# TissueImageAnalytics/cerberus

Measured on AMD Instinct MI355X. Metric: Mpx/sec WSI tiled inference (all heads), higher is better.
Workload: dtype f32

## Files before the change

### cerberus_amd/csrc/cerb_api.hip

```cpp
#include "cerb_net.h"

static thread_local std::string g_err;
int cerb_set_error(const std::string& m) {
    g_err = m;
    return 1;
}
extern "C" int cerb_version(void) { return 1; }
extern "C" const char* cerb_last_error(void) { return g_err.c_str(); }
std::atomic<long long> g_devbuf_bytes{0};
extern "C" size_t cerb_device_bytes_held(void) { const long long v = g_devbuf_bytes.load(); return v > 0 ? (size_t)v : 0; }
thread_local hipStream_t g_call_stream = nullptr;

static int alloc_dev(cerb_net* net, size_t bytes, void** out) {
    if (net->reusing) {
        if (net->reuse_cursor >= net->n_finalize_allocs || net->dev_alloc_bytes[net->reuse_cursor] != bytes)
            return fail("reload: the tensors do not have the shapes the handle was finalized with");
        *out = net->dev_allocs[net->reuse_cursor++];
        return 0;
    }
    void* d = nullptr;
    HIP_OK(hipMalloc(&d, bytes));
    net->dev_allocs.push_back(d);
    net->dev_alloc_bytes.push_back(bytes);
    *out = d;
    return 0;
}
static int upload(cerb_net* net, const std::vector<float>& v, float** out) {
    void* d = nullptr;
    if (alloc_dev(net, v.size() * sizeof(float), &d)) return 1;
    HIP_OK(hipMemcpy(d, v.data(), v.size() * sizeof(float), hipMemcpyHostToDevice));
    *out = reinterpret_cast<float*>(d);
    return 0;
}

extern "C" int cerb_net_create(const char* const* decoder_names, const char* const* head_names, const int* out_ch,
                               int n_decoders, cerb_net** out_net) {
    if (!decoder_names || !head_names || !out_ch || !out_net || n_decoders <= 0) return fail("cerb_net_create: bad arguments");
    cerb_net* net = new cerb_net();
    for (int i = 0; i < n_decoders; ++i) {
        DecoderCfg d;
        d.name = decoder_names[i];
        d.head = head_names[i];
        d.out_ch = out_ch[i];
        if (d.name == "Patch-Class") {
            d.kind = 2;
            if (d.out_ch < 1 || d.out_ch > 16) { delete net; return fail("Patch-Class: out_ch must be 1..16"); }
            net->pc_idx = i;
        } else {
            if (d.head == "INST") d.kind = 0;
            else if (d.head == "TYPE") d.kind = 1;
            else { delete net; return fail("decoder " + d.name + ": head must be INST or TYPE, got " + d.head); }
            if (d.kind == 0 && d.out_ch != 2 && d.out_ch != 3) { delete net; return fail("INST heads must have 2 or 3 channels (infer_step keeps channels 1..out_ch-1), got " + std::to_string(d.out_ch)); }
            if (d.out_ch < 2 || d.out_ch > 8) { delete net; return fail("head out_ch must be 2..8"); }
            int trunk = -1;
            for (size_t t = 0; t < net->trunk_idx.size(); ++t)
                if (net->dec[net->trunk_idx[t]].name == d.name) trunk = (int)t;
            if (trunk < 0) {
                trunk = (int)net->trunk_idx.size();
                net->trunk_idx.push_back(i);
            } else {
                for (int e : net->dense_idx)
                    if (net->dec[e].name == d.name && net->dec[e].head == d.head) { delete net; return fail("decoder " + d.name + ": head " + d.head + " listed twice"); }
            }
            net->dense_idx.push_back(i);
            net->trunk_of.push_back(trunk);
        }
        net->dec.push_back(d);
    }
    *out_net = net;
    return 0;
}

extern "C" void cerb_net_destroy(cerb_net* net) { delete net; }

extern "C" int cerb_net_load_tensor(cerb_net* net, const char* key, const float* data, const int64_t* shape, int ndim) {
    if (!net || !key) return fail("cerb_net_load_tensor: bad arguments");
    if (net->finalized) return fail("cerb_net_load_tensor: network already finalized");
    std::string k(key);
    if (k.size() > 19 && k.compare(k.size() - 19, 19, "num_batches_tracked") == 0) return 0;
    if (k.rfind("backbone.fc.", 0) == 0) return 0;
    if (!data && ndim > 0) return fail("cerb_net_load_tensor: null data for " + k);
    HostTensor t;
    size_t n = 1;
    for (int i = 0; i < ndim; ++i) {
        t.shape.push_back(shape[i]);
        n *= (size_t)shape[i];
    }
    t.data.assign(data, data + n);
    net->host[k] = std::move(t);
    return 0;
}

struct Fold {
    std::vector<float> scale, shift;
};
static int get(cerb_net* net, const std::string& k, std::vector<int64_t> shape, const HostTensor** out) {
    auto it = net->host.find(k);
    if (it == net->host.end()) return fail("missing key in state dict: " + k);
    if (it->second.shape != shape) {
        std::string s = "shape mismatch for " + k + ": got [";
        for (auto v : it->second.shape) s += std::to_string(v) + ",";
        s += "] expected [";
        for (auto v : shape) s += std::to_string(v) + ",";
        return fail(s + "]");
    }
    *out = &it->second;
    return 0;
}
static int bn_fold(cerb_net* net, const std::string& p, int ch, Fold* f) {
    const HostTensor *w, *b, *m, *v;
    if (get(net, p + ".weight", {ch}, &w) || get(net, p + ".bias", {ch}, &b) || get(net, p + ".running_mean", {ch}, &m) ||
        get(net, p + ".running_var", {ch}, &v))
        return 1;
    f->scale.resize(ch);
    f->shift.resize(ch);
    for (int c = 0; c < ch; ++c) {
        const float s = w->data[c] / std::sqrt(v->data[c] + 1e-5f);
        f->scale[c] = s;
        f->shift[c] = b->data[c] - m->data[c] * s;
    }
    return 0;
}

static void pack_conv(const float* w, const float* scale, int cout, int cin, int ks, int CB, std::vector<float>* out) {
    const int T = ks * ks, NG = CB / 8, nchunk = cin / CB, ncb = cout / 64;
    const size_t base = out->size();
    out->resize(base + (size_t)cout * cin * T);
    float* o = out->data() + base;
    size_t idx = 0;
    for (int cb = 0; cb < ncb; ++cb)
        for (int ch = 0; ch < nchunk; ++ch)
            for (int tap = 0; tap < T; ++tap)
                for (int G = 0; G < NG; ++G)
                    for (int s = 0; s < 2; ++s)
                        for (int lane = 0; lane < 64; ++lane)
                            for (int t = 0; t < 4; ++t) {
                                const int co = cb * 64 + s * 32 + (lane & 31);
                                const int ci = ch * CB + G * 8 + 4 * (lane >> 5) + t;
                                o[idx++] = w[((size_t)co * cin + ci) * T + tap] * (scale ? scale[co] : 1.f);
                            }
}

static void pack_wino(const float* w, const float* scale, int cout, int cin, std::vector<float>* out) {
    static const double Gm[4][3] = {{1, 0, 0}, {0.5, 0.5, 0.5}, {0.5, -0.5, 0.5}, {0, 0, 1}};
    const int nchunk = cin / 32, ncb = cout / 64;
    const size_t base = out->size();
    out->resize(base + (size_t)cout * cin * 16);
    float* o = out->data() + base;
    std::vector<float> U((size_t)cout * cin * 16);
    for (int co = 0; co < cout; ++co)
        for (int ci = 0; ci < cin; ++ci) {
            double g[3][3], t[4][3];
            for (int y = 0; y < 3; ++y)
                for (int x = 0; x < 3; ++x) g[y][x] = (double)(w[((size_t)co * cin + ci) * 9 + y * 3 + x] * (scale ? scale[co] : 1.f));
            for (int a = 0; a < 4; ++a)
                for (int x = 0; x < 3; ++x) t[a][x] = Gm[a][0] * g[0][x] + Gm[a][1] * g[1][x] + Gm[a][2] * g[2][x];
            for (int a = 0; a < 4; ++a)
                for (int b = 0; b < 4; ++b)
                    U[((size_t)co * cin + ci) * 16 + a * 4 + b] = (float)(t[a][0] * Gm[b][0] + t[a][1] * Gm[b][1] + t[a][2] * Gm[b][2]);
        }
    size_t idx = 0;
    for (int cb = 0; cb < ncb; ++cb)
        for (int ch = 0; ch < nchunk; ++ch)
            for (int a = 0; a < 4; ++a)
                for (int b = 0; b < 4; ++b)
                    for (int G = 0; G < 4; ++G)
                        for (int s = 0; s < 2; ++s)
                            for (int lane = 0; lane < 64; ++lane)
                                for (int t = 0; t < 4; ++t) {
                                    const int co = cb * 64 + s * 32 + (lane & 31);
                                    const int ci = ch * 32 + G * 8 + 4 * (lane >> 5) + t;
                                    o[idx++] = U[((size_t)co * cin + ci) * 16 + a * 4 + b];
                                }
}

static void pack_wino4(const float* w, int cout, int cin, std::vector<float>* out, int layout = 0) {
    const bool chunk32 = layout == 1;
    static const double Gm[6][3] = {{1.0 / 4, 0, 0},          {-1.0 / 6, -1.0 / 6, -1.0 / 6}, {-1.0 / 6, 1.0 / 6, -1.0 / 6},
                                    {1.0 / 24, 1.0 / 12, 1.0 / 6}, {1.0 / 24, -1.0 / 12, 1.0 / 6},  {0, 0, 1}};
    const int nchunk = cin / 16, ncb = cout / 64;
    std::vector<float> U((size_t)cout * cin * 36);
    for (int co = 0; co < cout; ++co)
        for (int ci = 0; ci < cin; ++ci) {
            const float* g = w + ((size_t)co * cin + ci) * 9;
            double t[6][3];
            for (int a = 0; a < 6; ++a)
                for (int x = 0; x < 3; ++x) t[a][x] = Gm[a][0] * (double)g[x] + Gm[a][1] * (double)g[3 + x] + Gm[a][2] * (double)g[6 + x];
            for (int a = 0; a < 6; ++a)
                for (int b = 0; b < 6; ++b)
                    U[((size_t)co * cin + ci) * 36 + a * 6 + b] = (float)(t[a][0] * Gm[b][0] + t[a][1] * Gm[b][1] + t[a][2] * Gm[b][2]);
        }
    const size_t base = out->size();
    out->resize(base + (size_t)cout * cin * 36);
    float* o = out->data() + base;
    size_t idx = 0;
    if (chunk32) {
        for (int cb = 0; cb < ncb; ++cb)
            for (int ch = 0; ch < cin / 32; ++ch)
                for (int a = 0; a < 4; ++a)
                    for (int xi = 0; xi < 36; ++xi)
                        for (int G = 0; G < 2; ++G)
                            for (int lane = 0; lane < 64; ++lane)
                                for (int t = 0; t < 4; ++t) {
                                    const int co = cb * 64 + 16 * a + (lane & 15);
                                    const int ci = ch * 32 + 16 * G + 4 * (lane >> 4) + t;
                                    o[idx++] = U[((size_t)co * cin + ci) * 36 + xi];
                                }
        return;
    }
    for (int cb = 0; cb < ncb; ++cb)
        for (int ch = 0; ch < nchunk; ++ch)
            for (int a = 0; a < 4; ++a)
                for (int xi = 0; xi < 36; ++xi)
                    for (int lane = 0; lane < 64; ++lane)
                        for (int t = 0; t < 4; ++t) {
                            const int co = cb * 64 + 16 * a + (lane & 15);
                            const int ci = ch * 16 + 4 * (lane >> 4) + t;
                            o[idx++] = U[((size_t)co * cin + ci) * 36 + xi];
                        }
}

static int store_bn(cerb_net* net, const std::string& name, const std::vector<std::string>& bnkeys, int ch) {
    std::vector<float> ga, be;
    for (const std::string& k : bnkeys) {
        const HostTensor *w, *b;
        if (get(net, k + ".weight", {ch}, &w) || get(net, k + ".bias", {ch}, &b)) return 1;
        ga.insert(ga.end(), w->data.begin(), w->data.end());
        be.insert(be.end(), b->data.begin(), b->data.end());
    }
    cerb_net::BnDev d;
    d.C = ch;
    d.groups = (int)bnkeys.size();
    if (upload(net, ga, &d.gamma) || upload(net, be, &d.beta)) return 1;
    for (size_t g = 0; g < bnkeys.size(); ++g) {
        net->param_slots[bnkeys[g] + ".weight"].push_back({d.gamma + g * ch, ch});
        net->param_slots[bnkeys[g] + ".bias"].push_back({d.beta + g * ch, ch});
    }
    net->bn[name] = d;
    net->bn_keys[name] = bnkeys;
    return 0;
}

static int make_conv(cerb_net* net, const std::string& name, const std::vector<std::string>& wkeys,
                     const std::vector<std::string>& bkeys, const std::vector<std::string>& bnkeys, int cout, int cin, int ks,
                     int stride) {
    const int CB = cerb_conv_chunk(ks, stride);
    if (cout % 64 || cin % CB) return fail("conv " + name + ": unsupported channel counts");
    std::vector<float> wp, bp, wwino, hw;
    const bool wino = (ks == 3 && stride == 1 && cin % 32 == 0);
    for (size_t g = 0; g < wkeys.size(); ++g) {
        const HostTensor* w;
        if (get(net, wkeys[g], {cout, cin, ks, ks}, &w)) return 1;
        Fold f;
        bool have_bn = !bnkeys.empty() && net->fold_bn;
        if (have_bn && bn_fold(net, bnkeys[g], cout, &f)) return 1;
        if (net->fold_bn) {
            pack_conv(w->data.data(), have_bn ? f.scale.data() : nullptr, cout, cin, ks, CB, &wp);
            if (wino) {
                pack_wino(w->data.data(), have_bn ? f.scale.data() : nullptr, cout, cin, &wwino);
                const size_t b0 = hw.size();
                hw.insert(hw.end(), w->data.begin(), w->data.end());
                if (have_bn)
                    for (int co = 0; co < cout; ++co)
                        for (size_t e = 0; e < (size_t)cin * 9; ++e) hw[b0 + (size_t)co * cin * 9 + e] *= f.scale[co];
            }
        }
        const HostTensor* b = nullptr;
        if (!bkeys.empty() && get(net, bkeys[g], {cout}, &b)) return 1;
        for (int c = 0; c < cout; ++c) {
            float v = b ? b->data[c] : 0.f;
            if (have_bn) v = v * f.scale[c] + f.shift[c];
            bp.push_back(v);
        }
    }
    if (!net->fold_bn && !bnkeys.empty() && store_bn(net, name, bnkeys, cout)) return 1;
    if (!net->fold_bn) {
        std::vector<float> rw, rb;
        for (size_t g = 0; g < wkeys.size(); ++g) {
            const HostTensor* w;
            if (get(net, wkeys[g], {cout, cin, ks, ks}, &w)) return 1;
            rw.insert(rw.end(), w->data.begin(), w->data.end());
            if (!bkeys.empty()) {
                const HostTensor* b;
                if (get(net, bkeys[g], {cout}, &b)) return 1;
                rb.insert(rb.end(), b->data.begin(), b->data.end());
            }
        }
        cerb_net::RawW r;
        r.wkeys = wkeys; r.bkeys = bkeys; r.bnkeys = bnkeys;
        if (upload(net, rw, &r.w) || (!rb.empty() && upload(net, rb, &r.b))) return 1;
        for (size_t g = 0; g < wkeys.size(); ++g) {
            const long long nwg = (long long)cout * cin * ks * ks;
            net->param_slots[wkeys[g]].push_back({r.w + g * nwg, nwg});
            if (r.b) net->param_slots[bkeys[g]].push_back({r.b + g * cout, cout});
        }
        net->raw[name] = r;
    }
    PackedConv pc;
    pc.cin = cin; pc.cout = cout; pc.ks = ks; pc.stride = stride; pc.groups = (int)wkeys.size();
    if (upload(net, bp, &pc.b)) return 1;
    if (!net->fold_bn)
        for (size_t g = 0; g < bkeys.size(); ++g) net->param_slots[bkeys[g]].push_back({pc.b + g * cout, cout});
    if (net->fold_bn) {
        if (upload(net, wp, &pc.w)) return 1;
        if (wino && upload(net, wwino, &pc.wino)) return 1;
        pc.host_w.swap(hw);
    } else {
        const float* rawd = net->raw[name].w;
        const size_t G = wkeys.size(), nw = (size_t)cout * cin * ks * ks, nu = (size_t)cout * cin * 16;
        const bool dgrad = ks == 3 && cin % 64 == 0 && cout % 32 == 0;
        void *dwp = nullptr, *dwi = nullptr, *ddg = nullptr;
        if (alloc_dev(net, G * nw * 4, &dwp) || (wino && alloc_dev(net, G * nu * 4, &dwi)) || (dgrad && alloc_dev(net, G * nu * 4, &ddg))) return 1;
        pc.w = reinterpret_cast<float*>(dwp);
        pc.wino = reinterpret_cast<float*>(dwi);
        pc.wino_dgrad = reinterpret_cast<float*>(ddg);
        for (size_t g = 0; g < G; ++g) {
            HIP_OK(cerb_launch_pack_conv(rawd + g * nw, pc.w + g * nw, cout, cin, ks, CB, 0));
            if (wino) HIP_OK(cerb_launch_pack_wino(rawd + g * nw, pc.wino + g * nu, cout, cin, 0, 0));
            if (dgrad) HIP_OK(cerb_launch_pack_wino(rawd + g * nw, pc.wino_dgrad + g * nu, cin, cout, 1, 0));
        }
    }
    net->conv[name] = pc;
    return 0;
}


extern "C" int cerb_net_finalize(cerb_net* net) {
    if (!net) return fail("cerb_net_finalize: null handle");
    if (net->finalized) return 0;
    if (!net->fold_bn && net->trunk_idx.size() != net->dense_idx.size())
        return fail("cerb_net_finalize: a decoder with several output heads runs in inference only (the training tape sums one head's gradient per decoder)");
    {
        const HostTensor* w;
        if (get(net, "backbone.conv1.weight", {64, 3, 7, 7}, &w)) return 1;
        Fold f;
        if (bn_fold(net, "backbone.bn1", 64, &f)) return 1;
        if (!net->fold_bn) {
            f.scale.assign(64, 1.f);
            f.shift.assign(64, 0.f);
            if (store_bn(net, "stem", {"backbone.bn1"}, 64)) return 1;
        }
        std::vector<float> wp(7 * 12 * 2 * 64, 0.f);
        for (int ky = 0; ky < 7; ++ky)
            for (int t = 0; t < 12; ++t)
                for (int s = 0; s < 2; ++s)
                    for (int lane = 0; lane < 64; ++lane) {
                        const int co = s * 32 + (lane & 31), kk = 2 * t + (lane >> 5);
                        float v = 0.f;
                        if (kk < 21) {
                            const int kx = kk / 3, c = kk % 3;
                            v = w->data[(((size_t)co * 3 + c) * 7 + ky) * 7 + kx] * f.scale[co];
                        }
                        wp[((ky * 12 + t) * 2 + s) * 64 + lane] = v;
                    }
        if (upload(net, wp, &net->stem_w) || upload(net, f.shift, &net->stem_b)) return 1;
        if (!net->fold_bn) {
            if (upload(net, w->data, &net->stem_raw)) return 1;
            net->param_slots["backbone.conv1.weight"].push_back({net->stem_raw, 64 * 147});
        }
    }
    int inpl = 64;
    for (int li = 0; li < 4; ++li) {
        const int planes = kFilters[li + 1];
        for (int b = 0; b < kLayers[li]; ++b) {
            const std::string p = "backbone.layer" + std::to_string(li + 1) + "." + std::to_string(b);
            const int stride = (b == 0 && li > 0) ? 2 : 1;
            if (make_conv(net, p + ".conv1", {p + ".conv1.weight"}, {}, {p + ".bn1"}, planes, inpl, 3, stride)) return 1;
            if (make_conv(net, p + ".conv2", {p + ".conv2.weight"}, {}, {p + ".bn2"}, planes, planes, 3, 1)) return 1;
            if (stride != 1 || inpl != planes)
                if (make_conv(net, p + ".downsample", {p + ".downsample.0.weight"}, {}, {p + ".downsample.1"}, planes, inpl, 1, stride)) return 1;
            inpl = planes;
        }
    }
    if (make_conv(net, "conv_map", {"conv_map.weight"}, {}, {}, 256, 512, 1, 1)) return 1;
    const int dec_in[4] = {256, 128, 64, 64};
    const int dec_u[4][2] = {{256, 128}, {128, 64}, {64, 64}, {64, 64}};
    if (!net->dense_idx.empty()) {
        for (int u = 0; u < 4; ++u) {
            int c = dec_in[u];
            for (int j = 0; j < 2; ++j) {
                std::vector<std::string> wk, bk, bnk;
                for (int di : net->trunk_idx) {
                    const std::string p = "decoder_head." + net->dec[di].name + "." + std::to_string(u) + ".block." + std::to_string(j);
                    wk.push_back(p + ".conv.weight");
                    bk.push_back(p + ".conv.bias");
                    bnk.push_back(p + ".bn");
                }
                if (make_conv(net, "dec." + std::to_string(u) + "." + std::to_string(j), wk, bk, bnk, dec_u[u][j], c, 3, 1)) return 1;
                c = dec_u[u][j];
            }
        }
        for (int di : net->dense_idx) {
            const DecoderCfg& d = net->dec[di];
            const std::string p = "output_head." + d.name + "." + d.head + ".x";
            const HostTensor *w1, *b1, *w2, *b2;
            Fold f;
            if (get(net, p + ".0.block.0.conv.weight", {96, 64, 1, 1}, &w1) || get(net, p + ".0.block.0.conv.bias", {96}, &b1) ||
                bn_fold(net, p + ".0.block.0.bn", 96, &f) || get(net, p + ".1.conv.weight", {d.out_ch, 96, 1, 1}, &w2) ||
                get(net, p + ".1.conv.bias", {d.out_ch}, &b2))
                return 1;
            std::vector<float> w1p(6 * 4 * 64 * 4), b1p(96), w2p(6 * 64 * 4, 0.f), b2p(32, 0.f);
            for (int blk = 0; blk < 6; ++blk)
                for (int G = 0; G < 4; ++G)
                    for (int lane = 0; lane < 64; ++lane)
                        for (int t = 0; t < 4; ++t) {
                            const int hid = blk * 16 + (lane & 15), ci = G * 16 + 4 * (lane >> 4) + t;
                            w1p[((blk * 4 + G) * 64 + lane) * 4 + t] = w1->data[(size_t)hid * 64 + ci] * f.scale[hid];
                        }
            for (int c = 0; c < 96; ++c) b1p[c] = b1->data[c] * f.scale[c] + f.shift[c];
            for (int blk = 0; blk < 6; ++blk)
                for (int lane = 0; lane < 64; ++lane)
                    for (int r = 0; r < 4; ++r) {
                        const int o = lane & 15, hid = blk * 16 + 4 * (lane >> 4) + r;
                        w2p[(blk * 64 + lane) * 4 + r] = (o < d.out_ch) ? w2->data[(size_t)o * 96 + hid] : 0.f;
                    }
            for (int c = 0; c < d.out_ch; ++c) b2p[c] = b2->data[c];
            std::vector<float> w2q(2 * 24 * 64, 0.f);
            for (int set = 0; set < 2; ++set)
                for (int blk = 0; blk < 6; ++blk)
                    for (int r = 0; r < 4; ++r)
                        for (int lane = 0; lane < 64; ++lane) {
                            const int o = 4 * set + (lane & 3), hid = blk * 16 + 4 * (lane >> 4) + r;
                            if (o < d.out_ch) w2q[((set * 6 + blk) * 64 + lane) * 4 + r] = w2->data[(size_t)o * 96 + hid];
                        }
            if (!net->fold_bn) {
                float *r1, *rb1, *r2, *rb2;
                if (upload(net, w1->data, &r1) || upload(net, b1->data, &rb1) || upload(net, w2->data, &r2) || upload(net, b2->data, &rb2)) return 1;
                net->head_rw1.push_back(r1); net->head_rb1.push_back(rb1); net->head_rw2.push_back(r2); net->head_rb2.push_back(rb2);
                net->param_slots[p + ".0.block.0.conv.weight"].push_back({r1, 96 * 64});
                net->param_slots[p + ".0.block.0.conv.bias"].push_back({rb1, 96});
                net->param_slots[p + ".1.conv.weight"].push_back({r2, (long long)d.out_ch * 96});
                net->param_slots[p + ".1.conv.bias"].push_back({rb2, d.out_ch});
                if (store_bn(net, "head." + std::to_string(net->head_rw1.size() - 1), {p + ".0.block.0.bn"}, 96)) return 1;
            }
            float *dw1, *db1, *dw2, *db2;
            float* dw2q;
            if (upload(net, w1p, &dw1) || upload(net, b1p, &db1) || upload(net, w2p, &dw2) || upload(net, b2p, &db2) || upload(net, w2q, &dw2q)) return 1;
            net->head_w1.push_back(dw1); net->head_b1.push_back(db1); net->head_w2.push_back(dw2); net->head_b2.push_back(db2); net->head_w2q.push_back(dw2q);
        }
    }
    if (net->pc_idx >= 0) {
        const int oc = net->dec[net->pc_idx].out_ch;
        const std::string p = "decoder_head.Patch-Class";
        Fold f1, f2;
        const HostTensor *w1, *b1, *w2, *b2;
        if (bn_fold(net, p + ".bn1", 512, &f1) || bn_fold(net, p + ".bn2", 256, &f2) || get(net, p + ".conv1.weight", {256, 512, 1, 1}, &w1) ||
            get(net, p + ".conv1.bias", {256}, &b1) || get(net, p + ".conv2.weight", {oc, 256, 1, 1}, &w2) || get(net, p + ".conv2.bias", {oc}, &b2))
            return 1;
        if (!net->fold_bn) {
            if (upload(net, w1->data, &net->pc_rw1) || upload(net, b1->data, &net->pc_rb1) || upload(net, w2->data, &net->pc_rw2) ||
                upload(net, b2->data, &net->pc_rb2) || store_bn(net, "pc.bn1", {p + ".bn1"}, 512) || store_bn(net, "pc.bn2", {p + ".bn2"}, 256))
                return 1;
            net->param_slots[p + ".conv1.weight"].push_back({net->pc_rw1, 256 * 512});
            net->param_slots[p + ".conv1.bias"].push_back({net->pc_rb1, 256});
            net->param_slots[p + ".conv2.weight"].push_back({net->pc_rw2, (long long)oc * 256});
            net->param_slots[p + ".conv2.bias"].push_back({net->pc_rb2, oc});
        }
        std::vector<float> w1t(512 * 256), b1f(256), w2t(256 * 16, 0.f), b2f(16, 0.f);
        for (int o = 0; o < 256; ++o) {
            for (int c = 0; c < 512; ++c) w1t[(size_t)c * 256 + o] = w1->data[(size_t)o * 512 + c] * f2.scale[o];
            b1f[o] = b1->data[o] * f2.scale[o] + f2.shift[o];
        }
        for (int o = 0; o < oc; ++o) {
            for (int c = 0; c < 256; ++c) w2t[(size_t)c * 16 + o] = w2->data[(size_t)o * 256 + c];
            b2f[o] = b2->data[o];
        }
        if (upload(net, f1.scale, &net->pc_bn1s) || upload(net, f1.shift, &net->pc_bn1b) || upload(net, w1t, &net->pc_w1t) ||
            upload(net, b1f, &net->pc_b1) || upload(net, w2t, &net->pc_w2t) || upload(net, b2f, &net->pc_b2))
            return 1;
    }
    if (!net->fold_bn) {
        std::vector<float> z(512, 0.f);
        if (upload(net, z, &net->zero_bias)) return 1;
    }
    if (!net->fold_bn) HIP_OK(hipDeviceSynchronize());
    if (net->reusing && net->reuse_cursor != net->n_finalize_allocs) return fail("reload: fewer tensors than the handle was finalized with");
    if (!net->reusing) net->n_finalize_allocs = net->dev_allocs.size();
    net->reusing = false;
    net->host.clear();
    net->finalized = true;
    return 0;
}

int prof_begin(cerb_net* net, const std::string& name, const std::string& kernel, double flops, hipStream_t st) {
    if (!net->profiling) return 0;
    if (net->prof_n == net->prof.size()) {
        cerb_net::ProfRec r;
        HIP_OK(hipEventCreate(&r.e0));
        HIP_OK(hipEventCreate(&r.e1));
        net->prof.push_back(r);
    }
    cerb_net::ProfRec& r = net->prof[net->prof_n];
    r.name = name; r.kernel = kernel; r.flops = flops;
    HIP_OK(hipEventRecord(r.e0, st));
    net->prof_open = true;
    return 0;
}
int prof_end(cerb_net* net, hipStream_t st) {
    if (!net->profiling) return 0;
    HIP_OK(hipEventRecord(net->prof[net->prof_n].e1, st));
    net->prof_n++;
    net->prof_open = false;
    return 0;
}

int train_wino2_fresh(cerb_net* net, const std::string& name, PackedConv& cm, int dgrad, hipStream_t st) {
    if (net->fold_bn) return 0;
    bool& used = dgrad ? cm.wino_dgrad_used : cm.wino_used;
    bool& stale = dgrad ? cm.wino_dgrad_stale : cm.wino_stale;
    used = true;
    if (!stale) return 0;
    auto rit = net->raw.find(name);
    if (rit == net->raw.end()) return fail("conv " + name + ": no raw weights to re-pack");
    const size_t nw = (size_t)cm.cout * cm.cin * 9, nu = (size_t)cm.cout * cm.cin * 16;
    for (int g = 0; g < cm.groups; ++g)
        HIP_OK(cerb_launch_pack_wino(rit->second.w + g * nw, (dgrad ? cm.wino_dgrad : cm.wino) + g * nu, dgrad ? cm.cin : cm.cout, dgrad ? cm.cout : cm.cin, dgrad, st));
    stale = false;
    return 0;
}

int train_wino4_slot(cerb_net* net, const std::string& name, PackedConv& cm, int w4b, int dgrad, hipStream_t st, float** out) {
    float*& slot = cm.wino4_t[w4b][dgrad];
    if (!slot) {
        auto rit = net->raw.find(name);
        if (rit == net->raw.end()) return fail("conv " + name + ": no raw weights for the F(4x4) transform");
        const size_t nw = (size_t)cm.cout * cm.cin * 9, nu = (size_t)cm.cout * cm.cin * 36;
        void* d = nullptr;
        HIP_OK(hipMalloc(&d, (size_t)cm.groups * nu * 4));
        net->dev_allocs.push_back(d);
        net->dev_alloc_bytes.push_back((size_t)cm.groups * nu * 4);
        slot = (float*)d;
        (void)nw;
        HIP_OK(cerb_launch_pack_wino4(rit->second.w, slot, dgrad ? cm.cin : cm.cout, dgrad ? cm.cout : cm.cin, dgrad, w4b, cm.groups, st));
    }
    *out = slot;
    return 0;
}

static constexpr int kPlanarLowest = 0;
static const char* const kPlanarFamily[4] = {"conv_wino4_planar<f4x4,16x16x2,eighth-res>", "conv_wino4_planar<f4x4,16x16x2,quarter-res>",
                                             "conv_wino4p<f4x4,16x16x2,planar,half-res>", "conv_wino4p<f4x4,16x16x2,planar>"};
static const char* const kPlanarEntryFamily[4] = {"upsample2_add_planar<eighth-res>", "upsample2_add_planar<quarter-res>", "upsample2_add_planar", "upsample2_add_planar"};

int run_conv(cerb_net* net, const std::string& name, const float* in, const float* prev, const float* resid, float* out, int N,
             int H, int W, int relu, int mode, long long in_gs, long long prev_gs, hipStream_t st, double* macs,
             const int* roi, long long planar_out_gs) {
    auto it = net->conv.find(name);
    if (it == net->conv.end()) return fail("internal: conv " + name + " not packed");
    const PackedConv& c = it->second;
    struct BnReq {
        cerb_net* n;
        ~BnReq() { n->conv_bn_part = nullptr; }
    } bn_req{net};
    net->conv_bn_bpg = 0;
    ConvParams p;
    memset(&p, 0, sizeof(p));
    p.in = in; p.prev = prev; p.wpack = c.w; p.bias = c.b; p.resid = resid; p.out = out;
    p.N = N; p.H = H; p.W = W; p.Cin = c.cin; p.Cout = c.cout;
    p.Ho = (c.stride == 2) ? H / 2 : H;
    p.Wo = (c.stride == 2) ? W / 2 : W;
    p.relu = relu;
    p.groups = c.groups;
    p.in_gs = in_gs; p.prev_gs = prev_gs;
    p.w_gs = (long long)c.cout * c.cin * c.ks * c.ks;
    p.bias_gs = c.cout;
    p.resid_gs = 0;
    p.out_gs = (long long)N * p.Ho * p.Wo * c.cout;
    p.pk_off = net->packed_items ? 0 : 1;
    if (macs) {
        *macs += (double)c.groups * N * p.Ho * p.Wo * (double)c.cout * c.cin * c.ks * c.ks;
        if (!out) return 0;
    }
    const double fl = 2.0 * (double)c.groups * N * p.Ho * p.Wo * (double)c.cout * c.cin * c.ks * c.ks;
    const long long map_px = (long long)p.Ho * p.Wo;
    const bool use_w4 = net->conv_algo == 5 || net->conv_algo == 7 || (net->conv_algo == 6 && map_px >= 256);
    const bool planar = planar_out_gs > 0;
    static const long long w4b_max_px = [] {
        const char* e = cerb_dev_getenv("CERB_W4B_MAX_PX");
        return e ? atoll(e) : 4096ll;
    }();
    const bool w4b = !planar && (net->conv_algo == 7 || (net->conv_algo == 6 && map_px <= w4b_max_px)) && c.cin % 64 == 0;
    if (planar && !(use_w4 && c.wino && mode == 0 && net->fold_bn && !resid)) return fail("internal: conv " + name + " cannot take the planar path");
    if (use_w4 && c.wino && mode == 0 && (!it->second.host_w.empty() || !net->fold_bn)) {
        PackedConv& cm = it->second;
        float* train_slot = nullptr;
        if (!net->fold_bn && train_wino4_slot(net, name, cm, w4b ? 1 : 0, 0, st, &train_slot)) return 1;
        float*& slot4 = !net->fold_bn ? train_slot : (w4b ? cm.wino4b : cm.wino4);
        if (!slot4) {
            std::vector<float> w4;
            for (int g = 0; g < cm.groups; ++g) pack_wino4(cm.host_w.data() + (size_t)g * cm.cout * cm.cin * 9, cm.cout, cm.cin, &w4, w4b ? 1 : 0);
            void* d = nullptr;
            HIP_OK(hipMalloc(&d, w4.size() * 4));
            net->dev_allocs.push_back(d);
            net->dev_alloc_bytes.push_back(w4.size() * 4);
            HIP_OK(hipMemcpy(d, w4.data(), w4.size() * 4, hipMemcpyHostToDevice));
            slot4 = (float*)d;
        }
        p.wpack = slot4;
        p.w_gs = (long long)c.cout * c.cin * 36;
        double fl_done = fl;
        if (roi && roi[1] > roi[0] && roi[3] > roi[2]) {
            p.roi_y0 = roi[0]; p.roi_y1 = roi[1]; p.roi_x0 = roi[2]; p.roi_x1 = roi[3];
            const double ty = (roi[1] + 15) / 16 - roi[0] / 16, tx = (roi[3] + 15) / 16 - roi[2] / 16;
            fl_done = fl * (ty * 16.0 * tx * 16.0) / ((double)p.Ho * p.Wo);
        }
        if (planar) {
            p.out_gs = planar_out_gs;
            p.level_tag = net->planar_level == 3 ? 1 : net->planar_level == 2 ? 0 : 2;
            p.pl_byp = cerb_planar_blocks(p.Ho);
            p.pl_bxp = cerb_planar_blocks(p.Wo);
        }
        if (prof_begin(net, name, planar ? kPlanarFamily[net->planar_level & 3] : w4b ? (cerb_wino4b_packed(p) ? (resid ? "conv_wino4b<f4x4,16t,res>" : "conv_wino4b<f4x4,16t>") : (resid ? "conv_wino4b<f4x4,16x16,res>" : "conv_wino4b<f4x4,16x16>")) : (resid ? "conv_wino4<f4x4,16x16x2,res>" : "conv_wino4<f4x4,16x16x2>"), fl_done, st)) return 1;
        if (net->conv_bn_part && !planar && !resid && !(roi && roi[1] > roi[0] && roi[3] > roi[2])) {
            p.bn_part = net->conv_bn_part;
            net->conv_bn_bpg = w4b ? cerb_wino4b_bn_blocks(p) : N * ((p.Ho + 15) / 16) * ((p.Wo + 15) / 16);
        }
        HIP_OK(planar ? cerb_launch_wino4p(p, st) : w4b ? cerb_launch_wino4b(p, st) : cerb_launch_wino4(p, st));
        if (prof_end(net, st)) return 1;
        return 0;
    }
    if (net->conv_algo && c.wino && mode == 0) {
        if (train_wino2_fresh(net, name, it->second, 0, st)) return 1;
        p.wpack = c.wino;
        p.w_gs = (long long)c.cout * c.cin * 16;
        double fl_done = fl;
        if (roi && roi[1] > roi[0] && roi[3] > roi[2]) {
            p.roi_y0 = roi[0]; p.roi_y1 = roi[1]; p.roi_x0 = roi[2]; p.roi_x1 = roi[3];
            const double ty = (roi[1] + 7) / 8 - roi[0] / 8, tx = (roi[3] + 15) / 16 - roi[2] / 16;
            fl_done = fl * (ty * 8.0 * tx * 16.0) / ((double)p.Ho * p.Wo);
        }
        if (prof_begin(net, name, resid ? "conv_wino<f2x2,8x16,res>" : "conv_wino<f2x2,8x16>", fl_done, st)) return 1;
        HIP_OK(cerb_launch_wino(p, st));
        if (prof_end(net, st)) return 1;
        return 0;
    }
    const std::string kn = "conv_igemm<ks" + std::to_string(c.ks) + ",s" + std::to_string(c.stride) + ",mode" + std::to_string(mode) +
                           (p.Wo < 32 ? ",16x16>" : ",8x32>");
    if (prof_begin(net, name, kn, fl, st)) return 1;
    HIP_OK(cerb_launch_conv(p, c.ks, c.stride, mode, st));
    if (prof_end(net, st)) return 1;
    return 0;
}

static int forward_impl(cerb_net* net, const cerb_forward_io* io, hipStream_t st, double* macs) {
    g_call_stream = st;
    const bool dry = (macs != nullptr) && (io->tiles == nullptr) && (io->tiles_f32 == nullptr);
    const int N = io->n, H = io->h, W = io->w;
    if (N <= 0 || H <= 0 || W <= 0 || (H % 16) || (W % 16)) return fail("cerb_net_forward: tile H,W must be positive multiples of 16");
    const int out_h = io->out_h > 0 ? io->out_h : H, out_w = io->out_w > 0 ? io->out_w : W;
    if (out_h > H || out_w > W) return fail("cerb_net_forward: crop larger than tile");
    const int hs[5] = {H, H / 2, H / 4, H / 8, H / 16}, ws[5] = {W, W / 2, W / 4, W / 8, W / 16};
    const size_t D = net->trunk_idx.size();
    const size_t guard = cerb_conv_guard_bytes(W);
    const int planar_lowest = [] {
        const char* e = cerb_dev_getenv("CERB_PLANAR_LOWEST");
        return e ? atoi(e) : kPlanarLowest;
    }();
    auto level_is_planar = [&](int u) {
        if (dry || !net->planar || !net->fold_bn || net->conv_algo != 6 || net->head_algo < 1) return false;
        for (int v = 3; v >= u; --v) {
            if (v < planar_lowest) return false;
            auto c0 = net->conv.find("dec." + std::to_string(v) + ".0"), c1 = net->conv.find("dec." + std::to_string(v) + ".1");
            if (c0 == net->conv.end() || c1 == net->conv.end() || !c0->second.wino || !c1->second.wino) return false;
            const long long px = (long long)hs[3 - v] * ws[3 - v];
            if ((hs[3 - v] & 3) || (ws[3 - v] & 3)) return false;
            const bool ok = v >= 2 ? px >= 4096 && c0->second.cin == 64 && c0->second.cout == 64 && c1->second.cout == 64
                                   : px >= 256 && c0->second.cin % 16 == 0 && c0->second.cout % 64 == 0 && c1->second.cin == c0->second.cout && c1->second.cout % 64 == 0;
            if (!ok) return false;
        }
        return true;
    };
    if (!dry) {
        if (net->x0.ensure((size_t)N * H * W * 64 * 4, guard) || net->pool.ensure((size_t)N * hs[1] * ws[1] * 64 * 4, guard)) return fail_alloc();
        for (int i = 1; i < 5; ++i)
            if (net->x[i].ensure((size_t)N * hs[i] * ws[i] * kFilters[i] * 4, guard)) return fail_alloc();
        if (net->ta.ensure((size_t)N * hs[1] * ws[1] * 64 * 4, guard) || net->tb.ensure((size_t)N * hs[1] * ws[1] * 64 * 4, guard) ||
            net->cm.ensure((size_t)N * hs[4] * ws[4] * 256 * 4, guard))
            return fail_alloc();
        if (D) {
            static const bool exact_ws = cerb_dev_getenv("CERB_LEGACY_WS") == nullptr;
            size_t need_sum = 0, need_mid = 0;
            const int oc[4] = {128, 64, 64, 64};
            for (int u = 0; u < 4; ++u) {
                if (exact_ws && level_is_planar(u)) continue;
                const std::string n0 = "dec." + std::to_string(u) + ".0";
                auto c0 = net->conv.find(n0);
                const size_t px = (size_t)D * N * hs[3 - u] * ws[3 - u];
                need_sum = std::max(need_sum, px * (size_t)(c0 != net->conv.end() ? c0->second.cin : 256) * 4);
                need_mid = std::max(need_mid, px * (size_t)(c0 != net->conv.end() ? c0->second.cout : 256) * 4);
            }
            if (!exact_ws) need_sum = need_mid = D * (size_t)N * H * W * 64 * 4;
            if (net->dmid.ensure(need_mid, guard)) return fail_alloc();
            if (net->conv_algo && net->dsum.ensure(need_sum, guard)) return fail_alloc();
            for (int u = 0; u < 4; ++u) {
                if (exact_ws && level_is_planar(u)) continue;
                if (net->dout[u].ensure(D * (size_t)N * hs[3 - u] * ws[3 - u] * oc[u] * 4, guard)) return fail_alloc();
            }
        }
    }
    if (macs) *macs += (double)N * H * W * 64.0 * 147.0;
    if (!dry) {
        StemParams sp;
        sp.tiles = io->tiles; sp.tiles_f32 = io->tiles ? nullptr : io->tiles_f32; sp.wpack = net->stem_w; sp.bias = net->stem_b; sp.out = net->x0.p; sp.N = N; sp.H = H; sp.W = W; sp.relu = 1;
        sp.tiles_x = sp.tiles_y = 0;
        if (prof_begin(net, "stem", "stem_conv7x7", 2.0 * N * H * W * 64.0 * 147.0, st)) return 1;
        HIP_OK(cerb_launch_stem(sp, st));
        if (prof_end(net, st)) return 1;
        if (prof_begin(net, "maxpool", "maxpool3x3s2", 0.0, st)) return 1;
        HIP_OK(cerb_launch_maxpool(net->x0.p, net->pool.p, N, H, W, 64, st));
        if (prof_end(net, st)) return 1;
    }
    float* cur = dry ? nullptr : net->pool.p;
    int inpl = 64;
    for (int li = 0; li < 4; ++li) {
        const int planes = kFilters[li + 1];
        const int Hi = (li == 0) ? hs[1] : hs[li], Wi = (li == 0) ? ws[1] : ws[li];
        for (int b = 0; b < kLayers[li]; ++b) {
            const std::string p = "backbone.layer" + std::to_string(li + 1) + "." + std::to_string(b);
            const int stride = (b == 0 && li > 0) ? 2 : 1;
            const int hin = (b == 0) ? Hi : hs[li + 1], win = (b == 0) ? Wi : ws[li + 1];
            float* t1 = dry ? nullptr : net->ta.p;
            const bool last = (b == kLayers[li] - 1);
            float* outb = dry ? nullptr : (((kLayers[li] - 1 - b) % 2 == 0) ? net->x[li + 1].p : net->tb.p);
            (void)last;
            const float* idt = cur;
            if (run_conv(net, p + ".conv1", cur, nullptr, nullptr, t1, N, hin, win, 1, 0, 0, 0, st, macs)) return 1;
            if (stride != 1 || inpl != planes) {
                float* ds = dry ? nullptr : net->pool.p;
                if (run_conv(net, p + ".downsample", cur, nullptr, nullptr, ds, N, hin, win, 0, 0, 0, 0, st, macs)) return 1;
                idt = ds;
            }
            if (run_conv(net, p + ".conv2", t1, nullptr, idt, outb, N, hs[li + 1], ws[li + 1], 1, 0, 0, 0, st, macs)) return 1;
            cur = outb;
            inpl = planes;
        }
    }
    if (run_conv(net, "conv_map", dry ? nullptr : net->x[4].p, nullptr, nullptr, dry ? nullptr : net->cm.p, N, hs[4], ws[4], 0, 0, 0, 0, st, macs)) return 1;

    const long long tile_stride = io->tile_stride ? io->tile_stride : (long long)out_h * out_w;
    const long long row_stride = io->row_stride ? io->row_stride : out_w;
    if (net->pc_idx >= 0) {
        if (macs) *macs += (double)N * (512.0 * 256 + 256.0 * net->dec[net->pc_idx].out_ch);
        const bool want = io->out && io->out[net->pc_idx];
        const bool wantl = io->logits && io->logits[net->pc_idx];
        if (!dry && (want || wantl)) {
            PatchClassParams pp;
            memset(&pp, 0, sizeof(pp));
            pp.x4 = net->x[4].p; pp.bn1_s = net->pc_bn1s; pp.bn1_b = net->pc_bn1b; pp.w1t = net->pc_w1t; pp.b1 = net->pc_b1;
            pp.w2t = net->pc_w2t; pp.b2 = net->pc_b2;
            pp.N = N; pp.Hf = hs[4]; pp.Wf = ws[4]; pp.out_ch = net->dec[net->pc_idx].out_ch;
            pp.out_h = out_h; pp.out_w = out_w;
            pp.logits = wantl ? io->logits[net->pc_idx] : nullptr;
            pp.out = want ? (float*)io->out[net->pc_idx] : nullptr;
            pp.tile_off = io->tile_off; pp.tile_stride = tile_stride; pp.row_stride = row_stride;
            if (prof_begin(net, "patch_class", "patch_class", 2.0 * N * (512.0 * 256 + 256.0 * pp.out_ch), st)) return 1;
            HIP_OK(cerb_launch_patch_class(pp, st));
            if (prof_end(net, st)) return 1;
        }
    }
    if (D) {
        const float* skips[4] = {dry ? nullptr : net->x[3].p, dry ? nullptr : net->x[2].p, dry ? nullptr : net->x[1].p, dry ? nullptr : net->x0.p};
        const float* prev = dry ? nullptr : net->cm.p;
        long long prev_gs = 0;
        const int oc[4] = {128, 64, 64, 64};
        int roi_out[4][4], roi_mid[4][4], roi_sum[4][4];
        const bool any_logits = [&] {
            if (!io->logits) return false;
            for (size_t k = 0; k < net->dec.size(); ++k)
                if (io->logits[k]) return true;
            return false;
        }();
        const bool use_roi = !dry && net->crop_roi && (net->conv_algo == 1 || net->conv_algo >= 5) && !any_logits && (out_h < H || out_w < W);
        if (use_roi) {
            int y0 = (int)((H - out_h) * 0.5), x0 = (int)((W - out_w) * 0.5), y1 = y0 + out_h, x1 = x0 + out_w;
            for (int u = 3; u >= 0; --u) {
                const int hh = hs[3 - u], ww = ws[3 - u];
                auto widen = [&](int* r, const int* in, int d) {
                    r[0] = std::max(0, (in[0] - d) & ~3); r[1] = std::min(hh, (in[1] + d + 3) & ~3);
                    r[2] = std::max(0, (in[2] - d) & ~3); r[3] = std::min(ww, (in[3] + d + 3) & ~3);
                };
                const int win[4] = {y0, y1, x0, x1};
                widen(roi_out[u], win, 0);
                widen(roi_mid[u], roi_out[u], 1);
                widen(roi_sum[u], roi_mid[u], 1);
                y0 = std::max(0, roi_sum[u][0] / 2 - 1); y1 = std::min(hh / 2, (roi_sum[u][1] - 1) / 2 + 2);
                x0 = std::max(0, roi_sum[u][2] / 2 - 1); x1 = std::min(ww / 2, (roi_sum[u][3] - 1) / 2 + 2);
            }
        }
        bool feat_planar = false, prev_planar = false;
        for (int u = 0; u < 4; ++u) {
            const int hh = hs[3 - u], ww = ws[3 - u];
            const std::string n0 = "dec." + std::to_string(u) + ".0", n1 = "dec." + std::to_string(u) + ".1";
            const int cmid = net->conv[n0].cout;
            const int cin0 = net->conv[n0].cin;
            const bool lvl_planar = level_is_planar(u);
            if (lvl_planar) {
                PlanarBuf &bs = u == 3 ? net->psum : u == 2 ? net->psum2 : u == 1 ? net->psum1 : net->psum0;
                PlanarBuf &bm = u == 3 ? net->pmid : u == 2 ? net->pmid2 : u == 1 ? net->pmid1 : net->pmid0;
                const int cout1 = net->conv[n1].cout;
                PlanarBuf& bo = cout1 == cin0 ? bs : u == 1 ? net->pout1 : net->pout0;
                if (bs.ensure((int)D, N, hh, ww, cin0, st) || bm.ensure((int)D, N, hh, ww, cmid, st) || (&bo != &bs && bo.ensure((int)D, N, hh, ww, cout1, st)))
                    return fail_alloc();
                if (prof_begin(net, n0 + ".up", kPlanarEntryFamily[u], 0.0, st)) return 1;
                HIP_OK(cerb_launch_upsample2_add_planar(skips[u], prev, bs.b.p, (int)D, N, hh, ww, cin0, prev_gs, bs.gs(), use_roi ? roi_sum[u] : nullptr, prev_planar ? 1 : 0, st));
                if (prof_end(net, st)) return 1;
                net->planar_level = u;
                if (run_conv(net, n0, bs.b.p, nullptr, nullptr, bm.b.p, N, hh, ww, 1, 0, bs.gs(), 0, st, macs, use_roi ? roi_mid[u] : nullptr, bm.gs()))
                    return 1;
                if (run_conv(net, n1, bm.b.p, nullptr, nullptr, bo.b.p, N, hh, ww, 1, 0, bm.gs(), 0, st, macs, use_roi ? roi_out[u] : nullptr, bo.gs()))
                    return 1;
                if (u == 3) feat_planar = true;
                prev = bo.b.p;
                prev_gs = bo.gs();
                prev_planar = true;
                continue;
            }
            if (prev_planar) return fail("internal: a tile-planar decoder level feeds an NHWC one");
            if (net->conv_algo && net->conv[n0].wino && !dry) {
                if (prof_begin(net, n0 + ".up", "upsample2_add", 0.0, st)) return 1;
                HIP_OK(cerb_launch_upsample2_add(skips[u], prev, net->dsum.p, (int)D, N, hh, ww, cin0, prev_gs, use_roi ? roi_sum[u] : nullptr, st));
                if (prof_end(net, st)) return 1;
                if (run_conv(net, n0, net->dsum.p, nullptr, nullptr, net->dmid.p, N, hh, ww, 1, 0, (long long)N * hh * ww * cin0, 0, st, macs,
                             use_roi ? roi_mid[u] : nullptr))
                    return 1;
            } else if (run_conv(net, n0, skips[u], prev, nullptr, dry ? nullptr : net->dmid.p, N, hh, ww, 1, 1, 0, prev_gs, st, macs)) return 1;
            if (run_conv(net, n1, dry ? nullptr : net->dmid.p, nullptr, nullptr, dry ? nullptr : net->dout[u].p, N, hh, ww, 1, 0,
                         (long long)N * hh * ww * cmid, 0, st, macs, use_roi ? roi_out[u] : nullptr))
                return 1;
            prev = dry ? nullptr : net->dout[u].p;
            prev_gs = (long long)N * hh * ww * oc[u];
        }
        HeadParams hps[8];
        int n_hp = 0;
        double head_flops = 0.0;
        for (size_t k = 0; k < net->dense_idx.size(); ++k) {
            const int di = net->dense_idx[k];
            const size_t tk = (size_t)net->trunk_of[k];
            const DecoderCfg& d = net->dec[di];
            if (macs) *macs += (double)N * H * W * (64.0 * 96 + 96.0 * d.out_ch);
            const bool want = io->out && io->out[di];
            const bool wantl = io->logits && io->logits[di];
            if (dry || !(want || wantl)) continue;
            HeadParams hp;
            memset(&hp, 0, sizeof(hp));
            hp.feat = feat_planar ? net->psum.b.p + tk * net->psum.gs() : net->dout[3].p + tk * (size_t)N * H * W * 64;
            hp.feat_planar = feat_planar ? 1 : 0;
            hp.pl_byp = cerb_planar_blocks(H);
            hp.pl_bxp = cerb_planar_blocks(W);
            hp.w1p = net->head_w1[k]; hp.b1 = net->head_b1[k]; hp.w2p = net->head_w2[k]; hp.b2 = net->head_b2[k]; hp.w2q = net->head_w2q[k];
            hp.N = N; hp.H = H; hp.W = W; hp.out_ch = d.out_ch; hp.kind = d.kind;
            hp.crop_y0 = (int)((H - out_h) * 0.5); hp.crop_x0 = (int)((W - out_w) * 0.5);
            hp.out_h = want ? out_h : 0; hp.out_w = want ? out_w : 0;
            hp.roi = use_roi ? 1 : 0;
            hp.logits = wantl ? io->logits[di] : nullptr;
            hp.absmax_bits = io->logit_absmax ? io->logit_absmax + di : nullptr;
            if (want) {
                if (d.kind == 0) hp.out_inst = (float*)io->out[di];
                else if (io->type_is_u8) hp.out_type_u8 = (unsigned char*)io->out[di];
                else hp.out_type_i64 = (long long*)io->out[di];
            }
            hp.tile_off = io->tile_off; hp.tile_stride = tile_stride; hp.row_stride = row_stride;
            const double head_px = hp.roi ? (double)out_h * (((hp.crop_x0 + out_w + 15) / 16 - hp.crop_x0 / 16) * 16.0) : (double)H * W;
            const double fl = 2.0 * N * head_px * (64.0 * 96 + 96.0 * d.out_ch);
            if (net->head_algo == 0) {
                if (prof_begin(net, "head." + d.name, "head", fl, st)) return 1;
                HIP_OK(cerb_launch_head(hp, st));
                if (prof_end(net, st)) return 1;
            } else {
                if (n_hp == 8) {
                    if (prof_begin(net, "heads", "head_group", head_flops, st)) return 1;
                    HIP_OK(cerb_launch_head_group(hps, n_hp, st, net->head_algo == 1 ? 1 : 0));
                    if (prof_end(net, st)) return 1;
                    n_hp = 0;
                    head_flops = 0.0;
                }
                hps[n_hp++] = hp;
                head_flops += fl;
            }
        }
        if (n_hp > 0) {
            if (prof_begin(net, "heads", "head_group", head_flops, st)) return 1;
            HIP_OK(cerb_launch_head_group(hps, n_hp, st, net->head_algo == 1 ? 1 : 0));
            if (prof_end(net, st)) return 1;
        }
    }
    if (!dry && io->feats) {
        const float* src[6] = {net->x0.p, net->x[1].p, net->x[2].p, net->x[3].p, net->cm.p, net->x[4].p};
        const size_t nb[6] = {(size_t)N * H * W * 64, (size_t)N * hs[1] * ws[1] * 64, (size_t)N * hs[2] * ws[2] * 128,
                              (size_t)N * hs[3] * ws[3] * 256, (size_t)N * hs[4] * ws[4] * 256, (size_t)N * hs[4] * ws[4] * 512};
        for (int i = 0; i < 6; ++i)
            if (io->feats[i]) HIP_OK(hipMemcpyAsync(io->feats[i], src[i], nb[i] * 4, hipMemcpyDeviceToDevice, st));
    }
    return 0;
}

extern "C" int cerb_net_begin_reload(cerb_net* net) {
    if (!net) return fail("cerb_net_begin_reload: null handle");
    HIP_OK(hipDeviceSynchronize());
    while (net->dev_allocs.size() > net->n_finalize_allocs) {
        (void)hipFree(net->dev_allocs.back());
        net->dev_allocs.pop_back();
        net->dev_alloc_bytes.pop_back();
    }
    net->reusing = true;
    net->reuse_cursor = 0;
    net->param_slots.clear();
    net->conv.clear();
    net->bn.clear();
    net->raw.clear();
    net->grads.clear();
    net->head_w1.clear(); net->head_b1.clear(); net->head_w2.clear(); net->head_b2.clear(); net->head_w2q.clear();
    net->head_rw1.clear(); net->head_rb1.clear(); net->head_rw2.clear(); net->head_rb2.clear();
    net->host.clear();
    net->finalized = false;
    return 0;
}
extern "C" int cerb_net_update_params(cerb_net* net, int count, const char* const* keys, const float* const* dev_src, void* hip_stream) {
    if (!net || count < 0 || (count && (!keys || !dev_src))) return fail("cerb_net_update_params: bad arguments");
    if (!net->finalized || net->fold_bn) return fail("cerb_net_update_params: needs a finalized handle packed for training (cerb_net_set_fold_bn(net, 0))");
    hipStream_t st = (hipStream_t)hip_stream;
    std::vector<float*> cd;
    std::vector<const float*> cs;
    std::vector<long long> cn;
    for (int i = 0; i < count; ++i) {
        auto it = net->param_slots.find(keys[i]);
        if (it == net->param_slots.end()) continue;
        if (!dev_src[i]) return fail(std::string("cerb_net_update_params: null source for ") + keys[i]);
        for (const cerb_net::ParamSlot& sl : it->second) {
            cd.push_back(sl.dst); cs.push_back(dev_src[i]); cn.push_back(sl.n);
        }
    }
    HIP_OK(cerb_launch_copy_multi((int)cd.size(), cd.data(), cs.data(), cn.data(), &net->copy_tab, &net->copy_tab_bytes, &net->copy_tab_host, st));
    HIP_OK(cerb_launch_pack_stem(net->stem_raw, net->stem_w, st));
    static const bool per_conv = cerb_dev_getenv("CERB_PACK_PER_CONV") != nullptr;
    std::vector<PackJob> jobs;
    auto job = [&](const float* w, float* out, long long total, int cout, int cin, int kind, int a, int b) { jobs.push_back(PackJob{w, out, total, cout, cin, kind, a, b, 0}); };
    for (auto& kv : net->conv) {
        PackedConv& pc = kv.second;
        const float* rawd = net->raw[kv.first].w;
        if (pc.wino && !pc.wino_used) pc.wino_stale = true;
        if (pc.wino_dgrad && !pc.wino_dgrad_used) pc.wino_dgrad_stale = true;
        const size_t nw = (size_t)pc.cout * pc.cin * pc.ks * pc.ks, nu = (size_t)pc.cout * pc.cin * 16, nu4 = (size_t)pc.cout * pc.cin * 36;
        for (int g = 0; g < pc.groups; ++g) {
            if (per_conv) {
                HIP_OK(cerb_launch_pack_conv(rawd + g * nw, pc.w + g * nw, pc.cout, pc.cin, pc.ks, cerb_conv_chunk(pc.ks, pc.stride), st));
                if (pc.wino && pc.wino_used) HIP_OK(cerb_launch_pack_wino(rawd + g * nw, pc.wino + g * nu, pc.cout, pc.cin, 0, st));
                if (pc.wino_dgrad && pc.wino_dgrad_used) HIP_OK(cerb_launch_pack_wino(rawd + g * nw, pc.wino_dgrad + g * nu, pc.cin, pc.cout, 1, st));
                continue;
            }
            job(rawd + g * nw, pc.w + g * nw, (long long)nw, pc.cout, pc.cin, 0, pc.ks * pc.ks, cerb_conv_chunk(pc.ks, pc.stride));
            if (pc.wino && pc.wino_used) job(rawd + g * nw, pc.wino + g * nu, (long long)nu, pc.cout, pc.cin, 1, 0, 0);
            if (pc.wino_dgrad && pc.wino_dgrad_used) job(rawd + g * nw, pc.wino_dgrad + g * nu, (long long)nu, pc.cin, pc.cout, 1, 1, 0);
        }
        for (int l = 0; l < 2; ++l)
            for (int dg = 0; dg < 2; ++dg)
                if (pc.wino4_t[l][dg]) {
                    if (per_conv) {
                        HIP_OK(cerb_launch_pack_wino4(rawd, pc.wino4_t[l][dg], dg ? pc.cin : pc.cout, dg ? pc.cout : pc.cin, dg, l, pc.groups, st));
                        continue;
                    }
                    for (int g = 0; g < pc.groups; ++g)
                        job(rawd + g * nw, pc.wino4_t[l][dg] + g * nu4, (long long)nu4, dg ? pc.cin : pc.cout, dg ? pc.cout : pc.cin, 2, dg, l);
                }
    }
    if (!jobs.empty()) HIP_OK(cerb_launch_pack_multi(jobs.data(), (int)jobs.size(), &net->pack_tab, &net->pack_tab_bytes, &net->pack_tab_host, st));
    return 0;
}
extern "C" int cerb_net_set_fold_bn(cerb_net* net, int fold) {
    if (!net) return fail("cerb_net_set_fold_bn: null handle");
    if (net->finalized) return fail("cerb_net_set_fold_bn: must be called before cerb_net_finalize");
    net->fold_bn = fold ? 1 : 0;
    return 0;
}

extern "C" int cerb_net_forward(cerb_net* net, const cerb_forward_io* io, void* hip_stream) {
    if (!net || !io) return fail("cerb_net_forward: null argument");
    if (!net->finalized) return fail("cerb_net_forward: call cerb_net_finalize first");
    if (!io->tiles && !io->tiles_f32) return fail("cerb_net_forward: null tiles pointer (neither tiles nor tiles_f32)");
    if (!net->fold_bn) return fail("cerb_net_forward: the network was packed for training (cerb_net_set_fold_bn(net, 0)); use cerb_net_forward_train");
    net->prof_n = 0;
    return forward_impl(net, io, (hipStream_t)hip_stream, nullptr);
}

extern "C" double cerb_net_flops(const cerb_net* net, int n, int h, int w) {
    if (!net || !net->finalized) return -1.0;
    cerb_forward_io io;
    memset(&io, 0, sizeof(io));
    io.n = n; io.h = h; io.w = w;
    double macs = 0.0;
    if (forward_impl(const_cast<cerb_net*>(net), &io, nullptr, &macs)) return -1.0;
    return 2.0 * macs;
}

extern "C" int cerb_net_set_crop_roi(cerb_net* net, int enable) {
    if (!net) return fail("cerb_net_set_crop_roi: null handle");
    net->crop_roi = enable ? 1 : 0;
    return 0;
}
extern "C" int cerb_net_set_conv_algo(cerb_net* net, int algo) {
    if (!net) return fail("cerb_net_set_conv_algo: null handle");
    if (algo < 0 || algo > 7 || (algo >= 2 && algo <= 4))
        return fail("cerb_net_set_conv_algo: algo must be 0 (direct), 1 (Winograd F(2x2) fp32), 5 (Winograd F(4x4) fp32), 7 (F(4x4), one-block items with 32-channel chunks) or 6 (F(4x4) for maps of 16 x 16 pixels and more -- 7's kernel up to 64 x 64, 5's above --, else F(2x2): the default); 2-4 were experiments (scripts/experiments/)");
    net->conv_algo = algo;
    return 0;
}

extern "C" int cerb_net_set_bn_eval(cerb_net* net, const char* bn_prefix, const float* running_mean, const float* running_var, int channels) {
    if (!net || !bn_prefix) return fail("cerb_net_set_bn_eval: null argument");
    if (!net->finalized || net->fold_bn) return fail("cerb_net_set_bn_eval: needs a finalized network packed with cerb_net_set_fold_bn(net, 0)");
    for (auto& kv : net->bn_keys) {
        const std::vector<std::string>& keys = kv.second;
        for (size_t g = 0; g < keys.size(); ++g) {
            if (keys[g] != bn_prefix) continue;
            auto it = net->bn.find(kv.first);
            if (it == net->bn.end()) return fail(std::string("cerb_net_set_bn_eval: internal: no BatchNorm ") + kv.first);
            cerb_net::BnDev& b = it->second;
            if (!running_mean || !running_var) {
                if (g < b.eval.size()) b.eval[g] = 0;
                return 0;
// ... 81 lines not shown
```

### cerberus_amd/csrc/cerb_net.h

```cpp
#ifndef CERB_NET_H
#define CERB_NET_H
#include <hip/hip_runtime.h>

#include <algorithm>
#include <cmath>
#include <cstdio>
#include <cstdlib>
#include <cstring>
#include <map>
#include <atomic>
#include <string>
#include <vector>

#include "../../include/cerberus_hip.h"
#include "cerb_common.h"

hipError_t cerb_launch_conv(const ConvParams& p, int ks, int stride, int mode, hipStream_t st);
hipError_t cerb_launch_wino(ConvParams p, hipStream_t st);
hipError_t cerb_launch_wino4(ConvParams p, hipStream_t st);
hipError_t cerb_launch_wino4b(ConvParams p, hipStream_t st);
int cerb_wino4b_bn_blocks(const ConvParams& p);
bool cerb_wino4b_packed(const ConvParams& p);
hipError_t cerb_launch_wino4p(ConvParams p, hipStream_t st);
hipError_t cerb_launch_upsample2_add_planar(const float* skip, const float* prev, float* out, int groups, int N, int H, int W, int C, long long prev_gs,
                                            long long out_gs, const int* roi, int prev_planar, hipStream_t st);
hipError_t cerb_launch_upsample2_add(const float* skip, const float* prev, float* out, int groups, int N, int H, int W, int C,
                                     long long prev_gs, const int* roi, hipStream_t st);
extern "C" int cerb_conv_chunk(int ks, int stride);
struct StemParams {
    const unsigned char* tiles;
    const float* tiles_f32;
    const float* wpack;
    const float* bias;
    float* out;
    int N, H, W, tiles_x, tiles_y;
    int relu;
};
hipError_t cerb_launch_stem(StemParams p, hipStream_t st);
size_t cerb_bn_workspace_bytes(int groups, long long rows, int C);
hipError_t cerb_launch_bn_stats(const float* x, long long group_stride, long long rows, int C, int groups, float eps, float* mean, float* rstd,
                                float* var_unbiased, void* ws, hipStream_t st);
hipError_t cerb_launch_bn_apply(float* x, const float* src, const float* resid, long long group_stride, long long rows, int C, int groups, const float* mean,
                                const float* rstd, const float* gamma, const float* beta, int relu, hipStream_t st);
hipError_t cerb_launch_bn_finalize(const double* partial, int blocks, long long rows, int C, float eps, float* mean, float* rstd, float* var_unbiased, hipStream_t st,
                                   int groups = 1, void* fold_ws = nullptr);
size_t cerb_bn_fold_workspace_bytes(int groups, int C);
hipError_t cerb_launch_pointwise(const float* in, const float* w, const float* bias, float* out, long long rows, int cin, int cout, const float* in_scale,
                                 hipStream_t st, double* bn_part = nullptr, int* bn_blocks = nullptr);
hipError_t cerb_launch_crop_gap(const float* x, int N, int H, int W, int C, int y0, int ch, int x0, int cw, float* out, hipStream_t st);
hipError_t cerb_launch_copy_multi(int count, float* const* dst, const float* const* src, const long long* n, void** dev_tab, size_t* dev_bytes,
                                  std::vector<char>* host_prev, hipStream_t st);
hipError_t cerb_launch_bn_bwd(const float* dz, const float* z, const float* y, float* dy, float* dresid, long long group_stride, long long rows, int C, int groups,
                              const float* mean, const float* rstd, const float* gamma, const float* beta, float* dgamma, float* dbeta, int relu, int dy_assign, void* ws, hipStream_t st, unsigned long long eval_mask = 0, int dresid_assign = 0,
                              const double* pre_part = nullptr, int pre_bpg = 0);
int cerb_head_bwd2_blocks();
hipError_t cerb_launch_conv_bwd(const float* x, const float* dy, const float* w, float* dx, float* dw, float* db, int G, int N, int H, int W, int Cin, int Cout,
                                int ks, int stride, long long x_gs, hipStream_t st);
hipError_t cerb_launch_stem_wgrad(const unsigned char* tiles, const float* dy, float* dw, int N, int H, int W, hipStream_t st);
hipError_t cerb_launch_maxpool_bwd(const float* x, const float* ypool, const float* dy, float* dx, int N, int H, int W, int C, hipStream_t st);
hipError_t cerb_launch_maxpool_idx(const float* in, float* out, unsigned* idx, int N, int H, int W, int C, hipStream_t st);
hipError_t cerb_launch_maxpool_bwd_idx(const unsigned* idx, const float* dy, float* dx, int N, int H, int W, int C, hipStream_t st);
bool cerb_upadd_bwd_fused_ok(int H, int W, int C, int G);
hipError_t cerb_launch_upadd_bwd(const float* dout, float* dskip, float* dprev, int G, int N, int H, int W, int C, long long prev_gs, int shared_prev, hipStream_t st,
                                 unsigned group_mask = 0xffffffffu, int skip_assign = 0, int prev_assign = 0);
hipError_t cerb_launch_pointwise_bwd(const float* x, const float* dy, const float* w, float* dx, float* dw, float* db, long long rows, int cin, int cout,
                                     const float* in_scale, int dx_assign, hipStream_t st);
hipError_t cerb_launch_crop_gap_bwd(const float* dg, float* dx, int N, int H, int W, int C, int y0, int ch, int x0, int cw, hipStream_t st);
hipError_t cerb_launch_adam(float* p, const float* g, float* m, float* v, long long n, float lr, float b1, float b2, float eps, int step, hipStream_t st);
size_t cerb_wgrad_workspace_bytes(int G, int N, int Ho, int Wo, int Cin, int Cout, int ks, int* slices_out);
size_t cerb_stem_wgrad_workspace_bytes();
hipError_t cerb_launch_pack_stem(const float* w_raw, float* out, hipStream_t st);
struct PackJob {
    const float* w;
    float* out;
    long long total;
    int cout, cin, kind, a, b, pad;
};
hipError_t cerb_launch_pack_multi(const PackJob* jobs, int count, void** dev_tab, size_t* dev_bytes, std::vector<char>* host_prev, hipStream_t st);
hipError_t cerb_launch_adam_multi(int count, float* const* p, const float* const* g, float* const* m, float* const* v, const long long* n, float lr, float b1,
                                  float b2, float eps, int step, hipStream_t st);
hipError_t cerb_launch_pack_conv(const float* w_raw, float* out, int cout, int cin, int ks, int chunk, hipStream_t st);
hipError_t cerb_launch_pack_wino(const float* w_raw, float* out, int cout, int cin, int dgrad, hipStream_t st);
hipError_t cerb_launch_pack_wino4(const float* w_raw, float* out, int cout, int cin, int dgrad, int chunk32, int groups, hipStream_t st);
hipError_t cerb_launch_dilate2(const float* dy, float* d, long long n, int H, int W, int C, hipStream_t st);
size_t cerb_pw_wgrad_small_workspace_bytes(long long rows, int cin, int cout);
hipError_t cerb_launch_pw_wgrad_small(const float* x, const float* dy, float* dw, long long rows, int cin, int cout, void* ws, hipStream_t st);
size_t cerb_pw_bwd_small_workspace_bytes(long long rows, int cin, int cout);
hipError_t cerb_launch_pw_bwd_small(const float* x, const float* dy, const float* w, float* dx, float* dw, float* db, long long rows, int cin, int cout,
                                    int dx_assign, void* ws, hipStream_t st);
hipError_t cerb_launch_stem_wgrad_mfma(const unsigned char* tiles, const float* dy, float* dw, int N, int H, int W, void* ws, hipStream_t st);
hipError_t cerb_launch_colsum(const float* d, long long group_stride, long long rows, int C, int G, float* out, void* ws, hipStream_t st);
bool cerb_wgrad_wino_supported(int H, int W, int Cin, int Cout);
size_t cerb_wgrad_wino_workspace_bytes(int G, int N, int H, int W, int Cin, int Cout);
hipError_t cerb_launch_wgrad_wino(const float* x, const float* dy, float* dw, int G, int N, int H, int W, int Cin, int Cout, long long x_gs, void* ws, hipStream_t st,
                                  float* db);
hipError_t cerb_launch_wgrad(const float* x, const float* dy, float* dw, int G, int N, int H, int W, int Cin, int Cout, int ks, int stride, long long x_gs, void* ws,
                             hipStream_t st, float* db = nullptr);
bool cerb_head_train_supported(long long rows, int cin, int chid, int out);
hipError_t cerb_launch_head_fwd1(const float* prev, const float* w1, const float* b1, float* hid, long long rows, double* bn_part, int* bn_blocks, hipStream_t st,
                                 const float* const* in_bn = nullptr);
hipError_t cerb_launch_head_fwd2(const float* hid, const float* mean, const float* rstd, const float* gamma, const float* beta, const float* w2, const float* b2,
                                 float* logits, long long rows, int out, hipStream_t st);
size_t cerb_head_bwd_workspace_bytes(long long rows, int out);
hipError_t cerb_launch_head_bwd1(const float* hid, const float* dlog, const float* mean, const float* rstd, const float* gamma, const float* beta, const float* w2,
                                 float* dw2, float* db2, float* dgamma, float* dbeta, long long rows, int out, void* ws, hipStream_t st);
hipError_t cerb_launch_head_bwd2(const float* hid, const float* dlog, const float* prev, const float* mean, const float* rstd, const float* gamma, const float* beta,
                                 const float* dgamma, const float* dbeta, const float* w1, const float* w2, float* dprev, float* dw1, float* db1, long long rows, int out,
                                 int eval_mode, int assign, void* ws, hipStream_t st, const float* const* in_bn = nullptr, double* in_part = nullptr);
hipError_t cerb_launch_maxpool(const float* in, float* out, int N, int H, int W, int C, hipStream_t st);
hipError_t cerb_launch_head(const HeadParams& p, hipStream_t st);
hipError_t cerb_launch_head_group(const HeadParams* heads, int n_heads, hipStream_t st, int w2_44);
struct PatchClassParams {
    const float* x4;
    const float* bn1_s;
    const float* bn1_b;
    const float* w1t;
    const float* b1;
    const float* w2t;
    const float* b2;
    int N, Hf, Wf, out_ch;
    int out_h, out_w;
    float* logits;
    float* out;
    const long long* tile_off;
    long long tile_stride, row_stride;
};
hipError_t cerb_launch_patch_class(const PatchClassParams& p, hipStream_t st);

int cerb_set_error(const std::string& m);
static inline int fail(const std::string& m) { return cerb_set_error(m); }
static inline int fail_alloc() { return cerb_set_error("workspace allocation failed") + 1; }
#define HIP_OK(expr)                                                                              \
    do {                                                                                          \
        hipError_t e_ = (expr);                                                                   \
        if (e_ != hipSuccess) return fail(std::string(#expr) + ": " + hipGetErrorString(e_));     \
    } while (0)

struct HostTensor {
    std::vector<int64_t> shape;
    std::vector<float> data;
};

extern "C" size_t cerb_conv_guard_bytes(int tile_w);
extern thread_local hipStream_t g_call_stream;
extern std::atomic<long long> g_devbuf_bytes;
struct DevBuf {
    float* p = nullptr;
    char* raw = nullptr;
    size_t bytes = 0, guard = 0, held = 0;
    int ensure(size_t need, size_t g) {
        if (need <= bytes && g <= guard) return 0;
        release();
        if (hipMalloc(&raw, need + 2 * g) != hipSuccess) {
            raw = nullptr;
            return 1;
        }
        g_devbuf_bytes += (long long)(need + 2 * g);
        held = need + 2 * g;
        if (hipMemsetAsync(raw, 0, need + 2 * g, g_call_stream) != hipSuccess) return 1;
        p = reinterpret_cast<float*>(raw + g);
        bytes = need;
        guard = g;
        return 0;
    }
    void release() {
        if (raw) {
            (void)hipFree(raw);
            g_devbuf_bytes -= (long long)held;
        }
        held = 0;
        raw = nullptr;
        p = nullptr;
        bytes = guard = 0;
    }
};

struct PlanarBuf {
    DevBuf b;
    int h = 0, w = 0, c = 0, groups = 0;
    long long cap_n = 0;
    long long per_image() const { return cerb_planar_elems(1, h, w, c); }
    long long gs() const { return cap_n * per_image(); }
    int ensure(int G, int N, int H, int W, int C, hipStream_t st) {
        if (H == h && W == w && C == c && G == groups && N <= cap_n) return 0;
        const size_t need = (size_t)G * (size_t)N * (size_t)cerb_planar_elems(1, H, W, C) * 4;
        if (need > b.bytes) {
            if (b.ensure(need, 0)) return 1;
        } else if (hipMemsetAsync(b.raw, 0, b.bytes + 2 * b.guard, st) != hipSuccess) {
            return 1;
        }
        h = H; w = W; c = C; groups = G;
        cap_n = (long long)(b.bytes / ((size_t)G * (size_t)cerb_planar_elems(1, H, W, C) * 4));
        return 0;
    }
    void release() { b.release(); h = w = c = groups = 0; cap_n = 0; }
};

struct PackedConv {
    int cin = 0, cout = 0, ks = 0, stride = 1, groups = 1;
    float* w = nullptr;
    float* wino = nullptr;
    float* wino_dgrad = nullptr;
    bool wino_used = false, wino_dgrad_used = false, wino_stale = false, wino_dgrad_stale = false;
    float* wino4_t[2][2] = {{nullptr, nullptr}, {nullptr, nullptr}};
    float* wino4b = nullptr;
    float* wino4 = nullptr;
    std::vector<float> host_w;
    float* b = nullptr;
};

struct DecoderCfg {
    std::string name, head;
    int out_ch = 0;
    int kind = 0;
};

struct cerb_net {
    std::vector<DecoderCfg> dec;
    std::vector<int> dense_idx;
    std::vector<int> trunk_idx;
    std::vector<int> trunk_of;
    int pc_idx = -1;
    std::map<std::string, HostTensor> host;
    bool finalized = false;
    float *stem_w = nullptr, *stem_b = nullptr;
    std::map<std::string, PackedConv> conv;
    std::vector<float*> head_w1, head_b1, head_w2, head_b2, head_w2q;
    float *pc_bn1s = nullptr, *pc_bn1b = nullptr, *pc_w1t = nullptr, *pc_b1 = nullptr, *pc_w2t = nullptr, *pc_b2 = nullptr;
    std::vector<void*> dev_allocs;
    std::vector<size_t> dev_alloc_bytes;
    size_t n_finalize_allocs = 0, reuse_cursor = 0;
    bool reusing = false;
    int fold_bn = 1;
    struct BnDev {
        float *gamma = nullptr, *beta = nullptr;
        int C = 0, groups = 1;
        float *run_mean = nullptr, *run_rstd = nullptr;
        std::vector<char> eval;
    };
    std::map<std::string, BnDev> bn;
    std::vector<float*> head_rw1, head_rb1, head_rw2, head_rb2;
    float *pc_rw1 = nullptr, *pc_rb1 = nullptr, *pc_rw2 = nullptr, *pc_rb2 = nullptr;
    DevBuf t_mean, t_rstd, t_ws, t_hid, t_gap, t_pc1, t_idn, t_dil;
    struct RawW { float* w = nullptr; float* b = nullptr; std::vector<std::string> wkeys, bkeys, bnkeys; };
    std::map<std::string, RawW> raw;
    struct ParamSlot { float* dst; long long n; };
    std::map<std::string, std::vector<ParamSlot>> param_slots;
    float* stem_raw = nullptr;
    std::vector<DevBuf> tape;
    size_t tape_pos = 0;
    void* copy_tab = nullptr;
    size_t copy_tab_bytes = 0;
    std::vector<char> copy_tab_host;
    void* pack_tab = nullptr;
    size_t pack_tab_bytes = 0;
    std::vector<char> pack_tab_host;
    float* zero_bias = nullptr;
    std::map<std::string, std::pair<float*, long long>> grads;
    std::map<std::string, std::vector<std::string>> bn_keys;
    DevBuf x0, pool, x[5], ta, tb, cm, dmid, dsum, dout[4];
    PlanarBuf psum, pmid, pout;
    int planar_level = 3;
    PlanarBuf psum2, pmid2, pout2;
    PlanarBuf psum1, pmid1, pout1, psum0, pmid0, pout0;
    int packed_items = 1;
    int planar = 1;
    bool profiling = false;
    int crop_roi = 1;
    int head_algo = 1;
    int conv_algo = 6;
    struct ProfRec { std::string name, kernel; double flops; hipEvent_t e0, e1; };
    std::vector<ProfRec> prof;
    size_t prof_n = 0;
    bool prof_open = false;
    double* conv_bn_part = nullptr;
    int conv_bn_bpg = 0;
    hipStream_t side = nullptr;
    hipEvent_t ev_fork = nullptr, ev_join = nullptr;
    DevBuf t_ws2;
    ~cerb_net() {
        if (side) { (void)hipStreamSynchronize(side); (void)hipStreamDestroy(side); }
        if (ev_fork) (void)hipEventDestroy(ev_fork);
        if (ev_join) (void)hipEventDestroy(ev_join);
        t_ws2.release();
        for (auto& r : prof) { (void)hipEventDestroy(r.e0); (void)hipEventDestroy(r.e1); }
        for (void* p : dev_allocs) (void)hipFree(p);
        if (copy_tab) (void)hipFree(copy_tab);
        if (pack_tab) (void)hipFree(pack_tab);
        x0.release(); pool.release(); ta.release(); tb.release(); cm.release(); dmid.release(); dsum.release(); psum.release(); pmid.release(); pout.release(); psum2.release(); pmid2.release(); pout2.release(); psum1.release(); pmid1.release(); pout1.release(); psum0.release(); pmid0.release(); pout0.release();
        t_mean.release(); t_rstd.release(); t_ws.release(); t_hid.release(); t_gap.release(); t_pc1.release(); t_idn.release(); t_dil.release();
        for (auto& b : tape) b.release();
        for (auto& b : x) b.release();
        for (auto& b : dout) b.release();
    }
};


static const int kLayers[4] = {3, 4, 6, 3};
static const int kFilters[5] = {64, 64, 128, 256, 512};
int prof_begin(cerb_net* net, const std::string& name, const std::string& kernel, double flops, hipStream_t st);
int prof_end(cerb_net* net, hipStream_t st);
int train_wino2_fresh(cerb_net* net, const std::string& name, PackedConv& cm, int dgrad, hipStream_t st);
int train_wino4_slot(cerb_net* net, const std::string& name, PackedConv& cm, int w4b, int dgrad, hipStream_t st, float** out);
int run_conv(cerb_net* net, const std::string& name, const float* in, const float* prev, const float* resid, float* out, int N, int H, int W, int relu, int mode,
             long long in_gs, long long prev_gs, hipStream_t st, double* macs, const int* roi = nullptr, long long planar_out_gs = 0);
#endif
```

### cerberus_amd/csrc/conv_igemm.hip

```cpp
#include "wino_common.h"

__device__ __forceinline__ f32x4 splat4(float x) {
    f32x4 r = {x, x, x, x};
    return r;
}

template <int KS, int STRIDE, int TH, int TW, int CB, int MODE>
struct ConvCfg {
    static constexpr int PAD = KS / 2;
    static constexpr int GSTEP = (KS == 1) ? STRIDE : 1;
    static constexpr int LSTEP = (KS == 1) ? 1 : STRIDE;
    static constexpr int IH = (KS == 1) ? TH : (TH - 1) * STRIDE + KS;
    static constexpr int IW = (KS == 1) ? TW : (TW - 1) * STRIDE + KS;
    static constexpr int PS = CB + 4;
    static constexpr int NG = CB / 8;
    static constexpr int T = KS * KS;
    static constexpr int NQ = T * NG;
    static constexpr int PARTS = CB / 4;
    static constexpr int PPS = 256 / PARTS;
    static constexpr int NF = IH * IW * PARTS;
    static constexpr int RPS = 32 / TW;
    static constexpr int NM = (IH + RPS - 1) / RPS;
    static constexpr int NE = (2 * IH * 8 + 255) / 256;
    static constexpr int ITER = (MODE == 1) ? NM + NE : (NF + 255) / 256;
    static constexpr int MAIN_FLOATS = IH * IW * PS;
    static constexpr int AR = TH / 2 + 2, AC = TW / 2 + 2;
    static constexpr int NA = AR * AC * PARTS;
    static constexpr int AITER = (NA + 255) / 256;
    static constexpr int AUX_FLOATS = (MODE == 1) ? AR * AC * PS : 0;
    static constexpr int LDS_FLOATS = MAIN_FLOATS + AUX_FLOATS;
    static constexpr int LDS_BYTES = LDS_FLOATS * 4;
    static constexpr int S_PREV = ITER;
    static constexpr int S_BAR = ITER + AITER + 6;
    static constexpr int S_COMB = S_BAR + 1;
    static constexpr int WD = (MODE == 0 && STRIDE == 1) ? 3 : 2;
};

struct Item {
    int g, cb, n, oy0, ox0, tx, ty;
};

template <int KS, int STRIDE, int TH, int TW, int CB, int MODE>
__global__ __launch_bounds__(256, 2) void conv_igemm_kernel(ConvParams p) {
    using C = ConvCfg<KS, STRIDE, TH, TW, CB, MODE>;
    constexpr int WD = C::WD;
    static_assert(TH * TW == 256, "tile must hold 256 pixels (4 waves x 2 x 32)");
    static_assert(MODE == 0 || (KS == 3 && STRIDE == 1 && CB == 32 && C::IH % C::RPS == 0 && C::S_COMB + C::ITER <= C::NQ),
                  "MODE 1 schedule must fit in one chunk");
    static_assert(C::ITER <= 2 * C::NQ || KS == 1, "every staging slice needs a step");
    extern __shared__ __attribute__((aligned(16))) float lds[];

    const int tid = threadIdx.x;
    const int lane = tid & 63;
    const int wave = tid >> 6;
    const int j = lane & 31;
    const int h = lane >> 5;

    const int ncb = p.Cout >> 6;
    const int ntile = p.N * p.tiles_y * p.tiles_x;
    const int per_group = ntile * ncb;
    const int total = per_group * p.groups;
    const int nchunk = p.Cin / CB;
    const int lb = xcd_remap(blockIdx.x, gridDim.x);
    const int base_cnt = total / (int)gridDim.x, rem_cnt = total % (int)gridDim.x;
    int item = lb * base_cnt + min(lb, rem_cnt);
    const int item_end = item + base_cnt + (lb < rem_cnt ? 1 : 0);
    if (item >= item_end) return;

    auto decode = [&](int it) {
        Item w;
        w.g = it / per_group;
        int L = it - w.g * per_group;
        w.cb = L % ncb;
        int t_ = L / ncb;
        w.tx = t_ % p.tiles_x;
        t_ /= p.tiles_x;
        w.ty = t_ % p.tiles_y;
        w.n = t_ / p.tiles_y;
        w.oy0 = w.ty * TH;
        w.ox0 = w.tx * TW;
        return w;
    };
    auto advance = [&](Item w) {
        if (++w.cb == ncb) {
            w.cb = 0;
            if (++w.tx == p.tiles_x) {
                w.tx = 0;
                if (++w.ty == p.tiles_y) {
                    w.ty = 0;
                    if (++w.n == p.N) {
                        w.n = 0;
                        ++w.g;
                    }
                }
            }
        }
        w.oy0 = w.ty * TH;
        w.ox0 = w.tx * TW;
        return w;
    };
    auto in_base = [&](const Item& w) {
        return reinterpret_cast<const char*>(p.in + w.g * p.in_gs) +
               ((((long long)w.n * p.H + (w.oy0 * STRIDE - C::PAD)) * p.W + (w.ox0 * STRIDE - C::PAD)) * p.Cin) * 4;
    };
    auto w_base = [&](const Item& w) {
        return reinterpret_cast<const char*>(p.wpack + w.g * p.w_gs + (long long)w.cb * nchunk * C::NQ * 2 * 256);
    };
    auto touches_border = [&](const Item& w) {
        const int y0 = w.oy0 * STRIDE - C::PAD, x0 = w.ox0 * STRIDE - C::PAD;
        return y0 < 0 || x0 < 0 || y0 + (C::IH - 1) * C::GSTEP + 1 > p.H || x0 + (C::IW - 1) * C::GSTEP + 1 > p.W;
    };

    constexpr int RPS = C::RPS, NM = C::NM, NE = C::NE;
    unsigned soff[MODE == 1 ? 1 + NE : C::ITER];
    int ldsw0, ldswE = 0;
    bool e_last_ok = true;
    const int rowb = p.W * p.Cin * 4;
    if (MODE == 1) {
        const int mrow = (tid >> 3) / TW, mcol = (tid >> 3) % TW, part = tid & 7;
        soff[0] = (unsigned)(((mrow * p.W + mcol) * p.Cin + part * 4) * 4);
        ldsw0 = (mrow * C::IW + mcol) * C::PS + part * 4;
        const int e_iy = tid >> 4, e_ix = TW + ((tid >> 3) & 1);
#pragma unroll
        for (int k = 0; k < NE; ++k) {
            const int iy = min(e_iy + 16 * k, C::IH - 1);
            soff[1 + k] = (unsigned)(((iy * p.W + e_ix) * p.Cin + part * 4) * 4);
        }
        ldswE = (e_iy * C::IW + e_ix) * C::PS + part * 4;
        e_last_ok = e_iy + 16 * (NE - 1) < C::IH;
    } else {
#pragma unroll
        for (int s = 0; s < C::ITER; ++s) {
            const int f = min(tid + s * 256, C::NF - 1);
            const int pix = f / C::PARTS, part = f % C::PARTS;
            soff[s] = (unsigned)((((pix / C::IW) * C::GSTEP * p.W + (pix % C::IW) * C::GSTEP) * p.Cin + part * 4) * 4);
        }
        ldsw0 = (tid / C::PARTS) * C::PS + (tid % C::PARTS) * 4;
    }
    const unsigned wlane = (unsigned)lane * 16u;
    int ldsb[2];
    unsigned ooff[2];
#pragma unroll
    for (int q = 0; q < 2; ++q) {
        const int pl = (wave * 2 + q) * 32 + j;
        const int py = pl / TW, px = pl % TW;
        ldsb[q] = ((py * C::LSTEP) * C::IW + px * C::LSTEP) * C::PS + 4 * h;
        ooff[q] = (unsigned)(((py * p.Wo + px) * p.Cout + 4 * h) * 4);
    }
    float* aux = lds + C::MAIN_FLOATS;
    int aoffM = 0, aoffE[NE];
    float wM[4] = {0.f, 0.f, 0.f, 0.f}, wE[4] = {0.f, 0.f, 0.f, 0.f};
    int auxw0 = 0;
    if (MODE == 1) {
        const int mrow = (tid >> 3) / TW, mcol = (tid >> 3) % TW, part = tid & 7;
        aoffM = (mcol >> 1) * C::PS + part * 4;
        const float lxM = (mcol & 1) ? 0.75f : 0.25f;
        const float lyM = (RPS == 2 && (mrow & 1)) ? 0.75f : 0.25f;
        wM[0] = (1.f - lyM) * (1.f - lxM), wM[1] = (1.f - lyM) * lxM, wM[2] = lyM * (1.f - lxM), wM[3] = lyM * lxM;
        const int e_iy = tid >> 4, e_b = (tid >> 3) & 1;
#pragma unroll
        for (int k = 0; k < NE; ++k) aoffE[k] = ((min(e_iy + 16 * k, C::IH - 1) >> 1) * C::AC + TW / 2) * C::PS + part * 4;
        const float lxE = e_b ? 0.75f : 0.25f, lyE = (e_iy & 1) ? 0.75f : 0.25f;
        wE[0] = (1.f - lyE) * (1.f - lxE), wE[1] = (1.f - lyE) * lxE, wE[2] = lyE * (1.f - lxE), wE[3] = lyE * lxE;
        auxw0 = (tid / C::PARTS) * C::PS + (tid % C::PARTS) * 4;
    }

    f32x4 v[C::ITER];
    f32x4 pvv[C::AITER > 0 ? C::AITER : 1];
    unsigned poff[MODE == 1 ? C::AITER : 1];

    auto issue = [&](__amdgpu_buffer_rsrc_t r, int chunk_off, int s) {
        if (MODE == 1) {
            if (s < NM) v[s] = buf_load(r, soff[0], chunk_off + s * RPS * rowb);
            else v[s] = buf_load(r, soff[1 + s - NM], chunk_off);
        } else {
            v[s] = buf_load(r, soff[s], chunk_off);
        }
    };
    auto prev_offsets = [&](const Item& w) {
        const int Hp = p.H >> 1, Wp = p.W >> 1;
#pragma unroll
        for (int k = 0; k < C::AITER; ++k) {
            const int f = min(tid + k * 256, C::NA - 1);
            const int apix = f / C::PARTS, part = f % C::PARTS;
            const int py = min(max((w.oy0 >> 1) - 1 + apix / C::AC, 0), Hp - 1), px = min(max((w.ox0 >> 1) - 1 + apix % C::AC, 0), Wp - 1);
            poff[k] = (unsigned)(((py * Wp + px) * p.Cin + part * 4) * 4);
        }
    };
    auto prev_base = [&](const Item& w) {
        return reinterpret_cast<const char*>(p.prev + w.g * p.prev_gs + (long long)w.n * (p.H >> 1) * (p.W >> 1) * p.Cin);
    };
    auto write_prev = [&]() {
#pragma unroll
        for (int k = 0; k < C::AITER; ++k)
            if (tid + k * 256 < C::NA) *reinterpret_cast<f32x4*>(aux + auxw0 + k * C::PPS * C::PS) = pvv[k];
    };
    auto combine = [&](int s) {
        const bool main = s < NM;
        const float* a = main ? aux + aoffM + ((s * RPS) >> 1) * C::AC * C::PS : aux + aoffE[main ? 0 : s - NM];
        const f32x4 p00 = *reinterpret_cast<const f32x4*>(a);
        const f32x4 p01 = *reinterpret_cast<const f32x4*>(a + C::PS);
        const f32x4 p10 = *reinterpret_cast<const f32x4*>(a + C::AC * C::PS);
        const f32x4 p11 = *reinterpret_cast<const f32x4*>(a + C::AC * C::PS + C::PS);
        const bool swap = main && RPS == 1 && (s & 1);
        const float* wt = main ? wM : wE;
        f32x4 r = v[s];
        r = __builtin_elementwise_fma(splat4(wt[swap ? 2 : 0]), p00, r);
        r = __builtin_elementwise_fma(splat4(wt[swap ? 3 : 1]), p01, r);
        r = __builtin_elementwise_fma(splat4(wt[swap ? 0 : 2]), p10, r);
        r = __builtin_elementwise_fma(splat4(wt[swap ? 1 : 3]), p11, r);
        v[s] = r;
    };
    auto slice_iy = [&](int s) { return MODE == 1 ? (s < NM ? s * RPS + (tid >> 3) / TW : (tid >> 4) + 16 * (s - NM)) : ((tid + s * 256) / C::PARTS) / C::IW; };
    auto slice_ix = [&](int s) { return MODE == 1 ? (s < NM ? (tid >> 3) % TW : TW + ((tid >> 3) & 1)) : ((tid + s * 256) / C::PARTS) % C::IW; };
    auto slice_ptr = [&](int s) { return MODE == 1 ? (s < NM ? lds + ldsw0 + s * RPS * C::IW * C::PS : lds + ldswE + (s - NM) * 16 * C::IW * C::PS) : lds + ldsw0 + s * C::PPS * C::PS; };
    auto slice_live = [&](int s) { return MODE == 1 ? (s < C::ITER - 1 || e_last_ok) : (tid + s * 256 < C::NF); };
    auto write_tile = [&](const Item& w, bool masked) {
        if (!masked) {
#pragma unroll
            for (int s = 0; s < C::ITER; ++s)
                if (slice_live(s)) *reinterpret_cast<f32x4*>(slice_ptr(s)) = v[s];
        } else {
#pragma unroll
            for (int s = 0; s < C::ITER; ++s) {
                const int gy = w.oy0 * STRIDE - C::PAD + slice_iy(s) * C::GSTEP, gx = w.ox0 * STRIDE - C::PAD + slice_ix(s) * C::GSTEP;
                const bool ok = gy >= 0 && gy < p.H && gx >= 0 && gx < p.W;
                const f32x4 z = {0.f, 0.f, 0.f, 0.f};
                if (slice_live(s)) *reinterpret_cast<f32x4*>(slice_ptr(s)) = ok ? v[s] : z;
            }
        }
    };

    Item w = decode(item);
    {
        const __amdgpu_buffer_rsrc_t r0 = make_rsrc(in_base(w));
#pragma unroll
        for (int s = 0; s < C::ITER; ++s) issue(r0, 0, s);
    }
    if (MODE == 1) {
        prev_offsets(w);
        const __amdgpu_buffer_rsrc_t rp = make_rsrc(prev_base(w));
#pragma unroll
        for (int k = 0; k < C::AITER; ++k) pvv[k] = buf_load(rp, poff[k], 0);
        write_prev();
        __syncthreads();
#pragma unroll
        for (int s = 0; s < C::ITER; ++s) combine(s);
    }
    __amdgpu_buffer_rsrc_t rw = make_rsrc(w_base(w));
    f32x4 wq[WD + 1][2];
#pragma unroll
    for (int d = 0; d < WD; ++d)
#pragma unroll
        for (int s = 0; s < 2; ++s) wq[d][s] = buf_load(rw, wlane, (d * 2 + s) * 1024);

    for (;;) {
        f32x16 acc[2][2];
#pragma unroll
        for (int s = 0; s < 2; ++s)
#pragma unroll
            for (int q = 0; q < 2; ++q)
#pragma unroll
                for (int r = 0; r < 16; ++r) acc[s][q][r] = 0.f;

        const bool more_items = item + 1 < item_end;
        const Item wnx = more_items ? advance(w) : w;
        const __amdgpu_buffer_rsrc_t rw_nx = more_items ? make_rsrc(w_base(wnx)) : rw;
        const bool mask_cur = touches_border(w);

        for (int ch = 0; ch < nchunk; ++ch) {
            __syncthreads();
            write_tile(w, mask_cur);
            __syncthreads();

            const bool last_ch = (ch == nchunk - 1);
            const Item wp_ = last_ch ? wnx : w;
            const int chp = last_ch ? 0 : ch + 1;
            const __amdgpu_buffer_rsrc_t r_stage = make_rsrc(in_base(wp_));
            const int stage_off = chp * (CB * 4);
            __amdgpu_buffer_rsrc_t r_prev = r_stage;
            if (MODE == 1) {
                r_prev = make_rsrc(prev_base(wp_));
                if (last_ch) prev_offsets(wp_);
            }
            const int wcur_off = ch * (C::NQ * 2048);
            const __amdgpu_buffer_rsrc_t rw_over = last_ch ? rw_nx : rw;
            const int wover_off = last_ch ? 0 : (ch + 1) * (C::NQ * 2048);

            f32x4 b0 = *reinterpret_cast<const f32x4*>(lds + ldsb[0]), b1 = *reinterpret_cast<const f32x4*>(lds + ldsb[1]);
            f32x4 bn0 = b0, bn1 = b1;
#pragma unroll
            for (int tap = 0; tap < C::T; ++tap) {
#pragma unroll
                for (int G = 0; G < C::NG; ++G) {
                    const int q = tap * C::NG + G;
                    {
                        if (q + WD < C::NQ) {
                            wq[WD][0] = buf_load(rw, wlane, wcur_off + ((q + WD) * 2 + 0) * 1024);
                            wq[WD][1] = buf_load(rw, wlane, wcur_off + ((q + WD) * 2 + 1) * 1024);
                        } else {
                            wq[WD][0] = buf_load(rw_over, wlane, wover_off + ((q + WD - C::NQ) * 2 + 0) * 1024);
                            wq[WD][1] = buf_load(rw_over, wlane, wover_off + ((q + WD - C::NQ) * 2 + 1) * 1024);
                        }
                        if (q + 1 < C::NQ) {
                            const int tap1 = (q + 1) / C::NG, G1 = (q + 1) % C::NG;
                            const int toff1 = ((tap1 / KS) * C::IW + (tap1 % KS)) * C::PS + G1 * 8;
                            bn0 = *reinterpret_cast<const f32x4*>(lds + ldsb[0] + toff1);
                            bn1 = *reinterpret_cast<const f32x4*>(lds + ldsb[1] + toff1);
                        }
                    }
#pragma unroll
                    for (int s = q; s < C::ITER; s += C::NQ) issue(r_stage, stage_off, s);
                    if (MODE == 1) {
                        if (q >= C::S_PREV && q < C::S_PREV + C::AITER) pvv[q - C::S_PREV] = buf_load(r_prev, poff[q - C::S_PREV], stage_off);
                        if (q == C::S_BAR) {
                            write_prev();
                            __syncthreads();
                        }
                        if (q >= C::S_COMB && q - C::S_COMB < C::ITER) combine(q - C::S_COMB);
                    }
                    __builtin_amdgcn_sched_barrier(0);
#pragma unroll
                    for (int t = 0; t < 4; ++t) {
                        acc[0][0] = __builtin_amdgcn_mfma_f32_32x32x2f32(wq[0][0][t], b0[t], acc[0][0], 0, 0, 0);
                        acc[1][0] = __builtin_amdgcn_mfma_f32_32x32x2f32(wq[0][1][t], b0[t], acc[1][0], 0, 0, 0);
                        acc[0][1] = __builtin_amdgcn_mfma_f32_32x32x2f32(wq[0][0][t], b1[t], acc[0][1], 0, 0, 0);
                        acc[1][1] = __builtin_amdgcn_mfma_f32_32x32x2f32(wq[0][1][t], b1[t], acc[1][1], 0, 0, 0);
                    }
#pragma unroll
                    for (int d = 0; d < WD; ++d) {
                        wq[d][0] = wq[d + 1][0];
                        wq[d][1] = wq[d + 1][1];
                    }
                    b0 = bn0;
                    b1 = bn1;
                }
            }
        }

        {
            const float* bias = p.bias + w.g * p.bias_gs + w.cb * 64 + h * 4;
            const long long origin = (((long long)w.n * p.Ho + w.oy0) * p.Wo + w.ox0) * p.Cout + w.cb * 64;
            const __amdgpu_buffer_rsrc_t r_out = make_rsrc(p.out + w.g * p.out_gs + origin);
            const __amdgpu_buffer_rsrc_t r_res = make_rsrc(p.resid ? p.resid + w.g * p.resid_gs + origin : p.out);
            const bool has_res = p.resid != nullptr;
            const bool partial = (w.oy0 + TH > p.Ho) || (w.ox0 + TW > p.Wo);
#pragma unroll
            for (int q = 0; q < 2; ++q) {
                if (partial) {
                    const int pl = (wave * 2 + q) * 32 + j;
                    if (w.oy0 + pl / TW >= p.Ho || w.ox0 + pl % TW >= p.Wo) continue;
                }
#pragma unroll
                for (int s = 0; s < 2; ++s) {
#pragma unroll
                    for (int rq = 0; rq < 4; ++rq) {
                        const int co = s * 32 + rq * 8;
                        f32x4 o = {acc[s][q][rq * 4 + 0], acc[s][q][rq * 4 + 1], acc[s][q][rq * 4 + 2], acc[s][q][rq * 4 + 3]};
                        o = o + *reinterpret_cast<const f32x4*>(bias + co);
                        if (has_res) o = o + buf_load(r_res, ooff[q], co * 4);
                        if (p.relu) {
                            o[0] = fmaxf(o[0], 0.f);
                            o[1] = fmaxf(o[1], 0.f);
                            o[2] = fmaxf(o[2], 0.f);
                            o[3] = fmaxf(o[3], 0.f);
                        }
                        buf_store(o, r_out, ooff[q], co * 4);
                    }
                }
            }
        }
        if (!more_items) break;
        ++item;
        w = wnx;
        rw = rw_nx;
    }
}

template <int KS, int STRIDE, int TH, int TW, int CB, int MODE>
static hipError_t launch_cfg(ConvParams p, hipStream_t st) {
    using C = ConvCfg<KS, STRIDE, TH, TW, CB, MODE>;
    p.tiles_x = (p.Wo + TW - 1) / TW;
    p.tiles_y = (p.Ho + TH - 1) / TH;
    const long long items = (long long)p.groups * p.N * p.tiles_x * p.tiles_y * (p.Cout / 64);
    auto kern = conv_igemm_kernel<KS, STRIDE, TH, TW, CB, MODE>;
    static bool attr_done[64] = {};
    if (cerb_attr_needed(attr_done)) {
        hipError_t e = hipFuncSetAttribute(reinterpret_cast<const void*>(kern), hipFuncAttributeMaxDynamicSharedMemorySize, C::LDS_BYTES);
        if (e != hipSuccess) return e;
    }
    const int blocks_per_cu = (C::LDS_BYTES * 2 <= 160 * 1024) ? 2 : 1;
    long long grid = 256ll * blocks_per_cu;
    if (grid > items) grid = items;
    hipLaunchKernelGGL(kern, dim3((unsigned)grid), dim3(256), C::LDS_BYTES, st, p);
    return hipGetLastError();
}

extern "C" int cerb_conv_chunk(int ks, int stride) { return (stride == 2) ? 16 : 32; }

extern "C" size_t cerb_conv_guard_bytes(int tile_w) { return (size_t)17 * (size_t)tile_w * 64 * 4 + (64u << 10); }

hipError_t cerb_launch_conv(const ConvParams& p, int ks, int stride, int mode, hipStream_t st) {
    const bool small = p.Wo < 32;
    if (ks == 3 && stride == 1 && mode == 0) return small ? launch_cfg<3, 1, 16, 16, 32, 0>(p, st) : launch_cfg<3, 1, 8, 32, 32, 0>(p, st);
    if (ks == 3 && stride == 1 && mode == 1) return small ? launch_cfg<3, 1, 16, 16, 32, 1>(p, st) : launch_cfg<3, 1, 8, 32, 32, 1>(p, st);
    if (ks == 3 && stride == 2 && mode == 0) return small ? launch_cfg<3, 2, 16, 16, 16, 0>(p, st) : launch_cfg<3, 2, 8, 32, 16, 0>(p, st);
    if (ks == 1 && stride == 1 && mode == 0) return small ? launch_cfg<1, 1, 16, 16, 32, 0>(p, st) : launch_cfg<1, 1, 8, 32, 32, 0>(p, st);
    if (ks == 1 && stride == 2 && mode == 0) return small ? launch_cfg<1, 2, 16, 16, 16, 0>(p, st) : launch_cfg<1, 2, 8, 32, 16, 0>(p, st);
    return hipErrorInvalidValue;
}
```

### cerberus_amd/csrc/conv_wino4p.hip

```cpp
#include <type_traits>

#include "wino_common.h"

namespace {
constexpr int NPOS = 36;
constexpr int NT = 32;
constexpr int CB = 16;
constexpr int V_FLOATS = NPOS * NT * CB;
constexpr int LDS_BYTES = 2 * V_FLOATS * 4;
constexpr int PLANE_BYTES = 16 * 16 * 16 * 4;
constexpr int NS = NPOS;
constexpr int NPOS_A = 32;
#ifndef P4_RING
#define P4_RING 12
#endif
constexpr int RING = P4_RING;
#ifndef P4_WD
#define P4_WD 8
#endif
constexpr int WD = P4_WD;
#ifndef P4_PRE
#define P4_PRE P4_WD
#endif
constexpr int PRE = P4_PRE;
#ifndef P4_WB
#define P4_WB 1
#endif
constexpr int WB = P4_WB;
#ifndef P4_TQ
#define P4_TQ 22
#endif
constexpr int TQ = P4_TQ;
#ifndef P4_HQ
#define P4_HQ 8
#endif
constexpr int HQ = P4_HQ;
constexpr int halo_r(int k) { return k < 6 ? k : k < 14 ? ((k - 6) & 1 ? 5 : 0) : k - 14; }
constexpr int halo_q(int k) { return k < 6 ? 0 : k < 14 ? 1 + (k - 6) / 2 : 5; }
static_assert(NS % RING == 0 && WD + WB <= RING && NS % WB == 0 && PRE == WD && PRE <= RING, "weight ring");
static_assert(HQ + 10 <= TQ && TQ + 13 < NS && TQ + 8 + 4 <= NS, "the halo must be requested before the transform starts, the interior after its registers are free");
constexpr int BIAS_XI = 7;
constexpr int CHUNK_W_BYTES = NPOS * 4 * 1024;
constexpr int WAVE_W_BYTES = NPOS * 1024;

#ifdef P4_PROF
constexpr int PROF_BYTES = 16 * 40 * 8;
__device__ unsigned long long p4_prof_buf[16 * 40];
#ifndef P4_PROF_WAVE
#define P4_PROF_WAVE 0
#endif
#else
#ifdef P4_ABL_LDSPATCH
constexpr int PROF_BYTES = 16 * 1024;
#else
constexpr int PROF_BYTES = 0;
#endif
#endif

template <int I>
using IC = std::integral_constant<int, I>;
template <int B, int E, class F>
__device__ __forceinline__ void static_for(F&& f) {
    if constexpr (B < E) {
        f(IC<B>{});
        static_for<B + 1, E>(f);
    }
}

#ifndef P4_WAUX
#define P4_WAUX 0
#endif
#ifndef P4_PAUX
#define P4_PAUX 0
#endif

template <bool AGPR, bool ZERO>
__device__ __forceinline__ void mfma_step(f32x4& c0, f32x4& c1, const f32x4& av, const f32x4& b0, const f32x4& b1) {
#define P4_STEP_BODY(FIRST0, FIRST1)                               \
    "v_mfma_f32_16x16x4_f32 %0, %2, %6, " FIRST0 "\n\t"             \
    "v_mfma_f32_16x16x4_f32 %1, %2, %10, " FIRST1 "\n\t"            \
    "v_mfma_f32_16x16x4_f32 %0, %3, %7, %0\n\t"                     \
    "v_mfma_f32_16x16x4_f32 %1, %3, %11, %1\n\t"                    \
    "v_mfma_f32_16x16x4_f32 %0, %4, %8, %0\n\t"                     \
    "v_mfma_f32_16x16x4_f32 %1, %4, %12, %1\n\t"                    \
    "v_mfma_f32_16x16x4_f32 %0, %5, %9, %0\n\t"                     \
    "v_mfma_f32_16x16x4_f32 %1, %5, %13, %1"
#define P4_STEP_IN "v"(av[0]), "v"(av[1]), "v"(av[2]), "v"(av[3]), "v"(b0[0]), "v"(b0[1]), "v"(b0[2]), "v"(b0[3]), "v"(b1[0]), "v"(b1[1]), "v"(b1[2]), "v"(b1[3])
    if constexpr (ZERO) {
        if constexpr (AGPR) asm volatile(P4_STEP_BODY("0", "0") : "=&a"(c0), "=&a"(c1) : P4_STEP_IN);
        else asm volatile(P4_STEP_BODY("0", "0") : "=&v"(c0), "=&v"(c1) : P4_STEP_IN);
    } else {
        if constexpr (AGPR) asm volatile(P4_STEP_BODY("%0", "%1") : "+a"(c0), "+a"(c1) : P4_STEP_IN);
        else asm volatile(P4_STEP_BODY("%0", "%1") : "+v"(c0), "+v"(c1) : P4_STEP_IN);
    }
#undef P4_STEP_BODY
#undef P4_STEP_IN
}
#ifndef P4_ILV
#define P4_ILV 0
#endif
template <bool AGPR, bool ZERO>
__device__ __forceinline__ void mfma_pair(f32x4& c0, f32x4& c1, float a, float b0, float b1) {
    if constexpr (ZERO) {
        if constexpr (AGPR) asm volatile("v_mfma_f32_16x16x4_f32 %0, %2, %3, 0\n\tv_mfma_f32_16x16x4_f32 %1, %2, %4, 0" : "=&a"(c0), "=&a"(c1) : "v"(a), "v"(b0), "v"(b1));
        else asm volatile("v_mfma_f32_16x16x4_f32 %0, %2, %3, 0\n\tv_mfma_f32_16x16x4_f32 %1, %2, %4, 0" : "=&v"(c0), "=&v"(c1) : "v"(a), "v"(b0), "v"(b1));
    } else {
        if constexpr (AGPR) asm volatile("v_mfma_f32_16x16x4_f32 %0, %2, %3, %0\n\tv_mfma_f32_16x16x4_f32 %1, %2, %4, %1" : "+a"(c0), "+a"(c1) : "v"(a), "v"(b0), "v"(b1));
        else asm volatile("v_mfma_f32_16x16x4_f32 %0, %2, %3, %0\n\tv_mfma_f32_16x16x4_f32 %1, %2, %4, %1" : "+v"(c0), "+v"(c1) : "v"(a), "v"(b0), "v"(b1));
    }
}
__device__ __forceinline__ void wait_mfma_results() { asm volatile("s_nop 15\n\ts_nop 3"); }

__device__ __forceinline__ int fresh_lane() {
    int l;
    asm volatile("v_mbcnt_lo_u32_b32 %0, -1, 0\n\tv_mbcnt_hi_u32_b32 %0, -1, %0" : "=v"(l));
    return l;
}

__device__ __forceinline__ f32x4 sub4(const f32x4& x, const f32x4& y) {
    f32x2 lo, hi;
    const f32x2 xl = {x[0], x[1]}, xh = {x[2], x[3]}, yl = {y[0], y[1]}, yh = {y[2], y[3]};
    asm("v_pk_add_f32 %0, %1, %2 neg_lo:[0,1] neg_hi:[0,1]" : "=v"(lo) : "v"(xl), "v"(yl));
    asm("v_pk_add_f32 %0, %1, %2 neg_lo:[0,1] neg_hi:[0,1]" : "=v"(hi) : "v"(xh), "v"(yh));
    return f32x4{lo[0], lo[1], hi[0], hi[1]};
}

struct Blk {
    int n, by, bx;
};
struct Item {
    int g, cb;
    Blk b0, b1;
    int nvalid;
};
}

template <int LEVEL>
__global__ __launch_bounds__(256) __attribute__((amdgpu_waves_per_eu(1, 1))) void conv_wino4p_kernel(ConvParams p) {
    extern __shared__ __attribute__((aligned(16))) float lds[];
    const int tid = threadIdx.x;
    const int lane = tid & 63;
    const int a = __builtin_amdgcn_readfirstlane(tid >> 6);
    const int m = lane & 15;
    const int ks = lane >> 4;

    const int ncb = p.Cout >> 6;
    const int nblk = p.N * p.tiles_y * p.tiles_x;
    const int npair = (nblk + 1) >> 1;
    const int per_group = npair * ncb;
    const int total = per_group * p.groups;
    const int nchunk = p.Cin / CB;
    const int nplane_o = p.Cout / CB;
    const int lb = xcd_remap(blockIdx.x, gridDim.x);
    const int ISTEP = (int)gridDim.x;
    int item = lb;
    const int item_end = total;
    if (item >= item_end) return;
#ifdef P4_PROF
    const int prof_item = item + 2 * ISTEP;
#endif

    auto decode_blk = [&](int id) {
        Blk b;
        b.bx = id % p.tiles_x;
        const int r = id / p.tiles_x;
        b.by = r % p.tiles_y;
        b.n = r / p.tiles_y;
        return b;
    };
    auto decode = [&](int it) {
        Item w;
        w.g = it / per_group;
        const int L = it - w.g * per_group;
        w.cb = L % ncb;
        const int pr = L / ncb;
        w.nvalid = (2 * pr + 1 < nblk) ? 2 : 1;
        w.b0 = decode_blk(2 * pr);
        w.b1 = w.nvalid == 2 ? decode_blk(2 * pr + 1) : w.b0;
        return w;
    };
    auto in_base = [&](int g, const Blk& b) {
#ifdef P4_ABL_PATCHL2
        return reinterpret_cast<const char*>(p.in) + (((long long)(b.by & 1)) * p.pl_bxp + (b.bx & 3)) * (long long)nchunk * PLANE_BYTES;
#endif
        return reinterpret_cast<const char*>(p.in + g * p.in_gs) +
               (((long long)b.n * p.pl_byp + (b.by + p.ty_off)) * p.pl_bxp + (b.bx + p.tx_off)) * (long long)nchunk * PLANE_BYTES;
    };
    auto w_base = [&](const Item& w) {
        return reinterpret_cast<const char*>(p.wpack + w.g * p.w_gs) + (long long)w.cb * nchunk * CHUNK_W_BYTES + a * WAVE_W_BYTES;
    };

    const int t = tid >> 3, c = tid & 7, tm = t & 15, tty = tm >> 2, ttx = tm & 3;
    const bool second = (a >> 1) != 0;
    auto mine = [&](const Item& wi) {
        Blk b;
        b.n = second ? wi.b1.n : wi.b0.n;
        b.by = second ? wi.b1.by : wi.b0.by;
        b.bx = second ? wi.b1.bx : wi.b0.bx;
        return b;
    };
    unsigned poff[3][3];
    {
        const unsigned rowblk = (unsigned)p.pl_bxp * (unsigned)nchunk * PLANE_BYTES, colblk = (unsigned)nchunk * PLANE_BYTES;
#pragma unroll
        for (int rc = 0; rc < 3; ++rc)
#pragma unroll
            for (int qc = 0; qc < 3; ++qc) {
                const int dby = (rc == 0 && tty == 0) ? 0 : (rc == 2 && tty == 3) ? 2 : 1;
                const int dbx = (qc == 0 && ttx == 0) ? 0 : (qc == 2 && ttx == 3) ? 2 : 1;
                const int ty2 = rc == 0 ? ((tty + 3) & 3) : rc == 2 ? ((tty + 1) & 3) : tty;
                const int tx2 = qc == 0 ? ((ttx + 3) & 3) : qc == 2 ? ((ttx + 1) & 3) : ttx;
                poff[rc][qc] = (unsigned)dby * rowblk + (unsigned)dbx * colblk + (unsigned)((4 * ty2 + tx2) * 64 + c * 8);
                asm volatile("" : "+v"(poff[rc][qc]));
            }
    }
    const int vw = t * CB + (((c >> 1) ^ ((tm & 8) ? 3 : 0)) << 2) + 2 * (c & 1);
    const int vr = m * CB + ((ks ^ ((m & 8) ? 3 : 0)) << 2);
    const unsigned wlane = (unsigned)lane * 16u;

    f32x2 d[6][6];
#ifdef P4_ABL_PREVADD
    f32x2 pv[4][4];
#endif
    auto issue = [&](__amdgpu_buffer_rsrc_t r, int chunk_off, int rr, int qq) __attribute__((always_inline)) {
        const int ii = rr == 0 ? 3 : rr == 5 ? 0 : rr - 1, jj = qq == 0 ? 3 : qq == 5 ? 0 : qq - 1;
#ifdef P4_ABL_PREVADD
        if ((rr == 0 || rr == 1 || rr == 3 || rr == 5) && (qq == 0 || qq == 1 || qq == 3 || qq == 5))
            pv[rr == 0 ? 0 : rr == 1 ? 1 : rr == 3 ? 2 : 3][qq == 0 ? 0 : qq == 1 ? 1 : qq == 3 ? 2 : 3] =
                buf_load2<P4_PAUX>(r, poff[rr == 0 ? 0 : rr == 5 ? 2 : 1][qq == 0 ? 0 : qq == 5 ? 2 : 1], chunk_off + ((ii ^ 1) * 4 + (jj ^ 2)) * 1024);
#endif
#ifdef P4_ABL_LDSPATCH
        d[rr][qq] = *reinterpret_cast<const f32x2*>(lds + (rr * 6 + qq) * NT * CB + vw);
        return;
#endif
#ifdef P4_ABL_NOCORNER
        if ((rr == 0 || rr == 5) && (qq == 0 || qq == 5)) return;
#endif
#ifdef P4_ABL_NOEDGE
        if (rr == 0 || rr == 5 || qq == 0 || qq == 5) return;
#endif
#ifdef P4_ABL_HALOOWN
        d[rr][qq] = buf_load2<P4_PAUX>(r, poff[1][1], chunk_off + (ii * 4 + jj) * 1024);
        return;
#endif
#ifdef P4_ABL_CORNEROWN
        if ((rr == 0 || rr == 5) && (qq == 0 || qq == 5)) { d[rr][qq] = buf_load2<P4_PAUX>(r, poff[1][1], chunk_off + (ii * 4 + jj) * 1024); return; }
#endif
        d[rr][qq] = buf_load2<P4_PAUX>(r, poff[rr == 0 ? 0 : rr == 5 ? 2 : 1][qq == 0 ? 0 : qq == 5 ? 2 : 1], chunk_off + (ii * 4 + jj) * 1024);
    };
    f32x2 k2 = {2.f, 2.f}, k4 = {4.f, 4.f}, k5 = {5.f, 5.f};
    asm volatile("" : "+v"(k2), "+v"(k4), "+v"(k5));
#if defined(P4_ABL_PREVADD) && P4_ABL_PREVADD + 0 == 2
    f32x2 k75 = {0.75f, 0.75f}, k25 = {0.25f, 0.25f};
    asm volatile("" : "+v"(k75), "+v"(k25));
    auto blend = [&](const f32x2& wa, const f32x2& x, const f32x2& wb, const f32x2& y) __attribute__((always_inline)) {
        f32x2 t, r;
        asm("v_pk_mul_f32 %0, %1, %2" : "=v"(t) : "v"(wb), "v"(y));
        asm("v_pk_fma_f32 %0, %1, %2, %3" : "=v"(r) : "v"(wa), "v"(x), "v"(t));
        return r;
    };
    auto pass_v = [&](int q) __attribute__((always_inline)) {
        const int qa = q <= 1 ? 0 : q <= 3 ? 1 : 2, qb = qa + 1;
        const bool odd = (q & 1) != 0;
        f32x2 h[4];
#pragma unroll
        for (int r = 0; r < 4; ++r) h[r] = odd ? blend(k75, pv[r][qa], k25, pv[r][qb]) : blend(k25, pv[r][qa], k75, pv[r][qb]);
        const f32x2 v0 = blend(k25, h[0], k75, h[1]), v1 = blend(k75, h[1], k25, h[2]), v2 = blend(k25, h[1], k75, h[2]);
        const f32x2 v3 = blend(k75, h[2], k25, h[3]), v4 = blend(k25, h[2], k75, h[3]), v5 = blend(k75, h[2], k25, h[3]);
        asm("v_pk_add_f32 %0, %0, %1" : "+v"(d[0][q]) : "v"(v0));
        asm("v_pk_add_f32 %0, %0, %1" : "+v"(d[1][q]) : "v"(v1));
        asm("v_pk_add_f32 %0, %0, %1" : "+v"(d[2][q]) : "v"(v2));
        asm("v_pk_add_f32 %0, %0, %1" : "+v"(d[3][q]) : "v"(v3));
        asm("v_pk_add_f32 %0, %0, %1" : "+v"(d[4][q]) : "v"(v4));
        asm("v_pk_add_f32 %0, %0, %1" : "+v"(d[5][q]) : "v"(v5));
        wino4_bt6(d[0][q], d[1][q], d[2][q], d[3][q], d[4][q], d[5][q], k2, k4, k5);
    };
#elif defined(P4_ABL_PREVADD)
    auto pass_v = [&](int q) __attribute__((always_inline)) {
        const int qi = q == 0 ? 0 : q <= 2 ? 1 : q <= 4 ? 2 : 3;
        asm("v_pk_add_f32 %0, %0, %1" : "+v"(d[0][q]) : "v"(pv[0][qi]));
        asm("v_pk_add_f32 %0, %0, %1" : "+v"(d[1][q]) : "v"(pv[1][qi]));
        asm("v_pk_add_f32 %0, %0, %1" : "+v"(d[2][q]) : "v"(pv[1][qi]));
        asm("v_pk_add_f32 %0, %0, %1" : "+v"(d[3][q]) : "v"(pv[2][qi]));
        asm("v_pk_add_f32 %0, %0, %1" : "+v"(d[4][q]) : "v"(pv[2][qi]));
        asm("v_pk_add_f32 %0, %0, %1" : "+v"(d[5][q]) : "v"(pv[3][qi]));
        wino4_bt6(d[0][q], d[1][q], d[2][q], d[3][q], d[4][q], d[5][q], k2, k4, k5);
    };
#else
    auto pass_v = [&](int q) __attribute__((always_inline)) { wino4_bt6(d[0][q], d[1][q], d[2][q], d[3][q], d[4][q], d[5][q], k2, k4, k5); };
#endif
    auto pass_h = [&](int r) __attribute__((always_inline)) { wino4_bt6(d[r][0], d[r][1], d[r][2], d[r][3], d[r][4], d[r][5], k2, k4, k5); };
    auto write_row = [&](int buf, int r) __attribute__((always_inline)) {
#pragma unroll
        for (int b = 0; b < 6; ++b) *reinterpret_cast<f32x2*>(lds + buf * V_FLOATS + (r * 6 + b) * NT * CB + vw) = d[r][b];
    };

    Item w = decode(item);
    {
        const __amdgpu_buffer_rsrc_t r0 = make_rsrc(in_base(w.g, mine(w)));
#pragma unroll
        for (int k = 0; k < 36; ++k) issue(r0, 0, k / 6, k % 6);
    }
#pragma unroll
    for (int q = 0; q < 6; ++q) pass_v(q);
#pragma unroll
    for (int r = 0; r < 6; ++r) {
        pass_h(r);
        write_row(0, r);
    }
    {
        const bool one = (nchunk == 1);
        const Item w1 = (one && item + ISTEP < item_end) ? decode(item + ISTEP) : w;
        const __amdgpu_buffer_rsrc_t r1 = make_rsrc(in_base(w1.g, mine(w1)));
#pragma unroll
        for (int k = 0; k < 16; ++k) issue(r1, one ? 0 : PLANE_BYTES, 1 + k / 4, 1 + k % 4);
    }
    int vbuf = 0;
    __syncthreads();
    __amdgpu_buffer_rsrc_t rw = make_rsrc(w_base(w));
    f32x4 wq[RING];
#pragma unroll
    for (int dd = 0; dd < PRE; ++dd) wq[dd] = buf_load<P4_WAUX>(rw, wlane, dd * 1024);
    f32x4 bnext;
    auto load_bias = [&](const Item& wi) {
        const float* bias = p.bias + wi.g * p.bias_gs + wi.cb * 64 + 16 * a;
        const __amdgpu_buffer_rsrc_t rb = __builtin_amdgcn_make_buffer_rsrc(const_cast<float*>(bias), 0, 64, 0x00020000);
        bnext = buf_load<P4_WAUX>(rb, (unsigned)(fresh_lane() >> 4) * 16u, 0);
    };
    load_bias(w);

    for (;;) {
        f32x4 acc[NPOS][2];
        const bool more_items = item + ISTEP < item_end;
        const Item wnx = more_items ? decode(item + ISTEP) : w;
        const __amdgpu_buffer_rsrc_t rw_nx = more_items ? make_rsrc(w_base(wnx)) : rw;
        const char* in_cur = in_base(w.g, mine(w));
        const char* in_nx = in_base(wnx.g, mine(wnx));
        const bool more2 = item + 2 * ISTEP < item_end;
        const Item wn2 = (nchunk == 1 && more2) ? decode(item + 2 * ISTEP) : wnx;
        const char* in_n2 = in_base(wn2.g, mine(wn2));
        auto in_nx2 = [&](int over) { return (nchunk == 1 && over >= 1) ? in_n2 : in_nx; };
        acc[BIAS_XI][0] = bnext;
        acc[BIAS_XI][1] = bnext;
#ifdef P4_PROF
        const bool prof_on = (blockIdx.x == P4_PROF) && a == P4_PROF_WAVE && (item == prof_item);
#define P4_STAMP(row, col) do { if (prof_on && lane == 0) reinterpret_cast<unsigned long long*>(lds + 2 * V_FLOATS)[(row) * 40 + (col)] = __builtin_readcyclecounter(); } while (0)
#else
#define P4_STAMP(row, col) do { } while (0)
#endif

        auto chunk = [&](auto first_tag, int ch) __attribute__((always_inline)) {
            constexpr bool FIRST = decltype(first_tag)::value;
            const bool last_ch = (ch == nchunk - 1);
            const __amdgpu_buffer_rsrc_t r_stage = make_rsrc(last_ch ? in_nx : in_cur);
            const int stage_off = (last_ch ? 0 : ch + 1) * PLANE_BYTES;
            const bool wrap2 = ch + 2 >= nchunk;
            const __amdgpu_buffer_rsrc_t r_stage2 = make_rsrc(wrap2 ? in_nx2(ch + 2 - nchunk) : in_cur);
            const int stage_off2 = (wrap2 ? (ch + 2 - nchunk) % nchunk : ch + 2) * PLANE_BYTES;
            const int wcur_off = ch * CHUNK_W_BYTES;
            const __amdgpu_buffer_rsrc_t rw_over = last_ch ? rw_nx : rw;
            const int wover_off = last_ch ? 0 : (ch + 1) * CHUNK_W_BYTES;
            const float* vsrc = lds + vbuf * V_FLOATS + vr;
            const int wbuf = vbuf ^ 1;

            f32x4 bb[2][2];
            bb[0][0] = *reinterpret_cast<const f32x4*>(vsrc);
            bb[0][1] = *reinterpret_cast<const f32x4*>(vsrc + 16 * CB);
            static_for<0, NS>([&](auto Q) __attribute__((always_inline)) {
                constexpr int q = decltype(Q)::value;
                constexpr int xi = q;
                constexpr bool AG = xi < NPOS_A;
#ifdef P4_PROF
                if (ch < 15) P4_STAMP(ch, q);
#endif
#if P4_ILV
                {
                    const f32x4 av = wq[q % RING];
                    const f32x4 b0 = bb[q & 1][0], b1 = bb[q & 1][1];
                    constexpr bool ZR = FIRST && xi != BIAS_XI;
                    __builtin_amdgcn_sched_barrier(0);
                    mfma_pair<AG, ZR>(acc[xi][0], acc[xi][1], av[0], b0[0], b1[0]);
                    __builtin_amdgcn_sched_barrier(0);
#ifndef P4_ABL_NOWLOAD
                if constexpr (q % WB == 0) {
#pragma unroll
                    for (int dd = q + WD; dd < q + WD + WB; ++dd) {
                        if (FIRST && dd < PRE) continue;
                        if (dd < NS) wq[dd % RING] = buf_load<P4_WAUX>(rw, wlane, wcur_off + dd * 1024);
                        else wq[(dd - NS) % RING] = buf_load<P4_WAUX>(rw_over, wlane, wover_off + (dd - NS) * 1024);
                    }
                }
#endif
                    __builtin_amdgcn_sched_barrier(0);
                    mfma_pair<AG, false>(acc[xi][0], acc[xi][1], av[1], b0[1], b1[1]);
                    __builtin_amdgcn_sched_barrier(0);
                if constexpr (q + 1 < NS) {
                    bb[(q + 1) & 1][0] = *reinterpret_cast<const f32x4*>(vsrc + (q + 1) * NT * CB);
                    bb[(q + 1) & 1][1] = *reinterpret_cast<const f32x4*>(vsrc + (q + 1) * NT * CB + 16 * CB);
                }
                    __builtin_amdgcn_sched_barrier(0);
                    mfma_pair<AG, false>(acc[xi][0], acc[xi][1], av[2], b0[2], b1[2]);
                    __builtin_amdgcn_sched_barrier(0);
#if P4_ILV == 3
                if constexpr (q > TQ + 7 && q <= TQ + 13) write_row(wbuf, q - TQ - 8);
#endif
#ifndef P4_ABL_NOPATCH
                if constexpr (q >= HQ && q < HQ + 10) {
                    issue(r_stage, stage_off, halo_r(2 * (q - HQ)), halo_q(2 * (q - HQ)));
                    issue(r_stage, stage_off, halo_r(2 * (q - HQ) + 1), halo_q(2 * (q - HQ) + 1));
                }
#endif
#ifndef P4_ABL_NOPATCH
                if constexpr (q >= TQ + 9 && q <= TQ + 12) {
#pragma unroll
                    for (int u = 1; u <= 4; ++u) issue(r_stage2, stage_off2, q - TQ - 8, u);
                }
#endif
                    __builtin_amdgcn_sched_barrier(0);
                    mfma_pair<AG, false>(acc[xi][0], acc[xi][1], av[3], b0[3], b1[3]);
                    __builtin_amdgcn_sched_barrier(0);
#ifndef P4_ABL_NOXF
                if constexpr (q > TQ && q <= TQ + 6) pass_v(q - TQ - 1);
                if constexpr (q > TQ + 6 && q <= TQ + 12) pass_h(q - TQ - 7);
#endif
#if defined(P4_ABL_VWRITE_FAKE)
                if constexpr (q > TQ + 6 && q <= TQ + 12) { if (p.N < 0) write_row(wbuf, q - TQ - 7); }
#elif !defined(P4_ABL_NOVWRITE)
                if constexpr (P4_ILV != 3 && q > TQ + 6 && q <= TQ + 12) write_row(wbuf, q - TQ - 7);
#endif
                }
#else
#ifndef P4_ABL_NOWLOAD
                if constexpr (q % WB == 0) {
#pragma unroll
                    for (int dd = q + WD; dd < q + WD + WB; ++dd) {
                        if (FIRST && dd < PRE) continue;
                        if (dd < NS) wq[dd % RING] = buf_load<P4_WAUX>(rw, wlane, wcur_off + dd * 1024);
                        else wq[(dd - NS) % RING] = buf_load<P4_WAUX>(rw_over, wlane, wover_off + (dd - NS) * 1024);
                    }
                }
#endif
                if constexpr (q + 1 < NS) {
                    bb[(q + 1) & 1][0] = *reinterpret_cast<const f32x4*>(vsrc + (q + 1) * NT * CB);
                    bb[(q + 1) & 1][1] = *reinterpret_cast<const f32x4*>(vsrc + (q + 1) * NT * CB + 16 * CB);
                }
#ifdef P4_ABL_LDSPATCH
                if constexpr (q < P4_ABL_LDSPATCH) {
                    const unsigned voff = (unsigned)(q * 4096 + tid * 16);
                    asm volatile("s_mov_b32 m0, %2\n\tbuffer_load_dwordx4 %0, %1, 0 offen lds" ::"v"(voff), "s"(r_stage), "s"((unsigned)(LDS_BYTES + ((q & 3) * 4 + a) * 1024)) : "memory");
                }
#endif
#ifndef P4_ABL_NOPATCH
                if constexpr (q >= HQ && q < HQ + 10) {
                    issue(r_stage, stage_off, halo_r(2 * (q - HQ)), halo_q(2 * (q - HQ)));
                    issue(r_stage, stage_off, halo_r(2 * (q - HQ) + 1), halo_q(2 * (q - HQ) + 1));
                }
#endif
#ifndef P4_ABL_NOXF
                if constexpr (q > TQ && q <= TQ + 6) pass_v(q - TQ - 1);
                if constexpr (q > TQ + 6 && q <= TQ + 12) pass_h(q - TQ - 7);
#endif
#if defined(P4_ABL_VWRITE_FAKE)
                if constexpr (q > TQ + 6 && q <= TQ + 12) { if (p.N < 0) write_row(wbuf, q - TQ - 7); }
#elif !defined(P4_ABL_NOVWRITE)
                if constexpr (q > TQ + 6 && q <= TQ + 12) write_row(wbuf, q - TQ - 7);
#endif
#ifndef P4_ABL_NOPATCH
                if constexpr (q >= TQ + 9 && q <= TQ + 12) {
#pragma unroll
                    for (int u = 1; u <= 4; ++u) issue(r_stage2, stage_off2, q - TQ - 8, u);
                }
#endif
                __builtin_amdgcn_sched_barrier(0);
                const f32x4 av = wq[q % RING];
                const f32x4 b0 = bb[q & 1][0], b1 = bb[q & 1][1];
                mfma_step<AG, FIRST && xi != BIAS_XI>(acc[xi][0], acc[xi][1], av, b0, b1);
#endif
                __builtin_amdgcn_sched_barrier(0);
            });
#ifndef P4_ABL_NOBAR
            __syncthreads();
#endif
            vbuf ^= 1;
        };
        chunk(std::true_type{}, 0);
        for (int ch = 1; ch < nchunk; ++ch) chunk(std::false_type{}, ch);

#pragma unroll
        for (int dd = WD; dd < PRE; ++dd) wq[dd % RING] = buf_load<P4_WAUX>(rw_nx, wlane, dd * 1024);
        load_bias(wnx);
        P4_STAMP(15, 0);
        wait_mfma_results();
#ifdef P4_ABL_NOOUT
        if (acc[0][0][0] == 1.2345e-30f)
#endif
        {
            int relu_s = p.relu;
            asm volatile("" : "+s"(relu_s));
            const float floor_ = __builtin_bit_cast(float, __builtin_amdgcn_readfirstlane(relu_s ? 0 : (int)0xff7fffff));
            const int lane_o = fresh_lane();
            const int m_o = lane_o & 15;
            const unsigned olane = (unsigned)(m_o * 64 + (lane_o >> 4) * 16);
#pragma unroll
            for (int tb = 0; tb < 2; ++tb) {
                const Blk bo = tb ? w.b1 : w.b0;
                if (tb == 1 && w.nvalid == 1) continue;
                const int by_abs = bo.by + p.ty_off, bx_abs = bo.bx + p.tx_off;
                const long long origin = p.out_gs * w.g + ((((long long)bo.n * p.pl_byp + by_abs + 1) * p.pl_bxp + bx_abs + 1) * nplane_o + w.cb * 4 + a) * (long long)(PLANE_BYTES / 4);
                const __amdgpu_buffer_rsrc_t r_out = __builtin_amdgcn_make_buffer_rsrc(p.out + origin, 0, PLANE_BYTES, 0x00020000);
                const bool partial = (by_abs * BLK + BLK > p.Ho) || (bx_abs * BLK + BLK > p.Wo);
                f32x4 T[4][6];
#pragma unroll
                for (int b = 0; b < 6; ++b) {
                    const f32x4 m0 = acc[0 * 6 + b][tb], m1 = acc[1 * 6 + b][tb], m2 = acc[2 * 6 + b][tb], m3 = acc[3 * 6 + b][tb],
                                m4 = acc[4 * 6 + b][tb], m5 = acc[5 * 6 + b][tb];
#ifdef P4_ABL_NOVPASS
                    T[0][b] = m0; T[1][b] = m1 + m5; T[2][b] = m2 + m3; T[3][b] = m4;
#else
                    const f32x4 s1 = m1 + m2, d1 = sub4(m1, m2), s2 = m3 + m4, d2 = sub4(m3, m4);
                    T[0][b] = m0 + s1 + s2;
                    T[1][b] = d1 + 2.f * d2;
                    T[2][b] = s1 + 4.f * s2;
                    T[3][b] = (d1 + 8.f * d2) + m5;
#endif
                }
                const int rem_y = p.Ho - by_abs * BLK - 4 * (m_o >> 2), rem_x = p.Wo - bx_abs * BLK - 4 * (m_o & 3);
#pragma unroll
                for (int i = 0; i < 4; ++i) {
                    const f32x4 s1 = T[i][1] + T[i][2], d1 = sub4(T[i][1], T[i][2]), s2 = T[i][3] + T[i][4], d2 = sub4(T[i][3], T[i][4]);
                    f32x4 y[4];
                    y[0] = T[i][0] + s1 + s2;
                    y[1] = d1 + 2.f * d2;
                    y[2] = s1 + 4.f * s2;
                    y[3] = (d1 + 8.f * d2) + T[i][5];
#pragma unroll
                    for (int j = 0; j < 4; ++j) {
                        f32x4 o = y[j];
                        o[0] = fmaxf(o[0], floor_);
                        o[1] = fmaxf(o[1], floor_);
                        o[2] = fmaxf(o[2], floor_);
                        o[3] = fmaxf(o[3], floor_);
#ifdef P4_ABL_STOREOOB
                        const unsigned vo = 0x80000000u | olane;
#else
                        const unsigned vo = (!partial || (i < rem_y && j < rem_x)) ? olane : 0x80000000u;
#endif
#ifndef P4_ABL_NOSTORE
                        buf_store(o, r_out, vo, (i * 4 + j) * 1024);
#else
                        if (o[0] == 1.2345e-30f) buf_store(o, r_out, vo, (i * 4 + j) * 1024);
#endif
                    }
                }
            }
        }
#ifdef P4_PROF
        P4_STAMP(15, 1);
        if (prof_on) {
            __builtin_amdgcn_s_waitcnt(0);
            P4_STAMP(15, 2);
            __builtin_amdgcn_s_waitcnt(0);
            for (int i = lane; i < 16 * 40; i += 64) p4_prof_buf[i] = reinterpret_cast<unsigned long long*>(lds + 2 * V_FLOATS)[i];
        }
#endif
        if (!more_items) break;
        item += ISTEP;
        w = wnx;
        rw = rw_nx;
    }
}

hipError_t cerb_launch_wino4p(ConvParams p, hipStream_t st) {
    if (p.Cin % CB || p.Cout % 64 || p.resid || p.pl_byp < 3 || p.pl_bxp < 3 || p.H != p.Ho || p.W != p.Wo) return hipErrorInvalidValue;
    const long long nblk = wino4_block_grid(p);
    if (p.pl_byp != (p.Ho + BLK - 1) / BLK + 2 || p.pl_bxp != (p.Wo + BLK - 1) / BLK + 2) return hipErrorInvalidValue;
    const long long items = (long long)p.groups * ((nblk + 1) / 2) * (p.Cout / 64);
    const int tag = p.level_tag == 2 ? 2 : p.level_tag ? 1 : 0;
    auto kern = tag == 2 ? conv_wino4p_kernel<2> : tag ? conv_wino4p_kernel<1> : conv_wino4p_kernel<0>;
    static bool attr_done[3][64] = {};
    return wino4_launch(kern, attr_done[tag], items, LDS_BYTES + PROF_BYTES, p, st);
}

#ifdef P4_PROF
extern "C" int cerb_w4p_prof_read(unsigned long long* dst) { return (int)hipMemcpyFromSymbol(dst, HIP_SYMBOL(p4_prof_buf), sizeof(unsigned long long) * 16 * 40); }
#endif
```

### cerberus_amd/csrc/dev_entry.hip

```cpp
#include "cerb_net.h"

#define DEV_NEED(cond) \
    do {               \
        if (!(cond)) return (int)hipErrorInvalidValue; \
    } while (0)

extern "C" {

int cerb_dev_wgrad_wino_supported(int H, int W, int Cin, int Cout) { return cerb_wgrad_wino_supported(H, W, Cin, Cout) ? 1 : 0; }
size_t cerb_dev_wgrad_wino_workspace_bytes(int G, int N, int H, int W, int Cin, int Cout) {
    return cerb_wgrad_wino_supported(H, W, Cin, Cout) ? cerb_wgrad_wino_workspace_bytes(G, N, H, W, Cin, Cout) : 0;
}
int cerb_dev_wgrad_wino(const float* x, const float* dy, float* dw, float* db, int G, int N, int H, int W, int Cin, int Cout, long long x_gs, void* ws, void* st) {
    DEV_NEED(x && dy && dw && ws && G > 0 && N > 0);
    return (int)cerb_launch_wgrad_wino(x, dy, dw, G, N, H, W, Cin, Cout, x_gs, ws, (hipStream_t)st, db);
}

size_t cerb_dev_wgrad_workspace_bytes(int G, int N, int Ho, int Wo, int Cin, int Cout, int ks, int* slices_out) {
    return cerb_wgrad_workspace_bytes(G, N, Ho, Wo, Cin, Cout, ks, slices_out);
}
int cerb_dev_wgrad(const float* x, const float* dy, float* dw, float* db, int G, int N, int H, int W, int Cin, int Cout, int ks, int stride, long long x_gs, void* ws,
                   void* st) {
    DEV_NEED(x && dy && dw && ws && G > 0 && N > 0 && H > 0 && W > 0);
    return (int)cerb_launch_wgrad(x, dy, dw, G, N, H, W, Cin, Cout, ks, stride, x_gs, ws, (hipStream_t)st, db);
}

size_t cerb_dev_stem_wgrad_mfma_workspace_bytes() { return cerb_stem_wgrad_workspace_bytes(); }
int cerb_dev_stem_wgrad_mfma(const unsigned char* tiles, const float* dy, float* dw, int N, int H, int W, void* ws, void* st) {
    DEV_NEED(tiles && dy && dw && ws && N > 0 && H > 0 && W > 0);
    return (int)cerb_launch_stem_wgrad_mfma(tiles, dy, dw, N, H, W, ws, (hipStream_t)st);
}
int cerb_dev_stem_wgrad(const unsigned char* tiles, const float* dy, float* dw, int N, int H, int W, void* st) {
    DEV_NEED(tiles && dy && dw && N > 0 && H > 0 && W > 0);
    return (int)cerb_launch_stem_wgrad(tiles, dy, dw, N, H, W, (hipStream_t)st);
}

int cerb_dev_conv_bwd(const float* x, const float* dy, const float* w, float* dx, float* dw, float* db, int G, int N, int H, int W, int Cin, int Cout, int ks, int stride,
                      long long x_gs, void* st) {
    DEV_NEED(dy && (dx || dw || db) && (!dx || w) && (!dw || x) && G > 0 && N > 0 && (ks == 1 || ks == 3) && (stride == 1 || stride == 2));
    return (int)cerb_launch_conv_bwd(x, dy, w, dx, dw, db, G, N, H, W, Cin, Cout, ks, stride, x_gs, (hipStream_t)st);
}

size_t cerb_dev_bn_workspace_bytes(int groups, long long rows, int C) { return cerb_bn_workspace_bytes(groups, rows, C); }
size_t cerb_dev_bn_fold_workspace_bytes(int groups, int C) { return cerb_bn_fold_workspace_bytes(groups, C); }
int cerb_dev_bn_stats(const float* x, long long group_stride, long long rows, int C, int groups, float eps, float* mean, float* rstd, float* var_unbiased, void* ws,
                      void* st) {
    DEV_NEED(x && mean && rstd && ws && rows > 0 && groups > 0);
    return (int)cerb_launch_bn_stats(x, group_stride, rows, C, groups, eps, mean, rstd, var_unbiased, ws, (hipStream_t)st);
}
int cerb_dev_bn_finalize(const double* partial, int blocks, long long rows, int C, float eps, float* mean, float* rstd, float* var_unbiased, int groups, void* fold_ws,
                         void* st) {
    DEV_NEED(partial && mean && rstd && blocks > 0 && rows > 0 && groups > 0);
    return (int)cerb_launch_bn_finalize(partial, blocks, rows, C, eps, mean, rstd, var_unbiased, (hipStream_t)st, groups, fold_ws);
}
int cerb_dev_bn_bwd(const float* dz, const float* z, const float* y, float* dy, float* dresid, long long group_stride, long long rows, int C, int groups, const float* mean,
                    const float* rstd, const float* gamma, const float* beta, float* dgamma, float* dbeta, int relu, int dy_assign, int dresid_assign,
                    unsigned long long eval_mask, void* ws, void* st) {
    DEV_NEED(dz && y && dy && mean && rstd && gamma && dgamma && dbeta && ws && rows > 0 && groups > 0 && (!relu || z || (beta && !dresid)));
    return (int)cerb_launch_bn_bwd(dz, z, y, dy, dresid, group_stride, rows, C, groups, mean, rstd, gamma, beta, dgamma, dbeta, relu, dy_assign, ws, (hipStream_t)st, eval_mask,
                                   dresid_assign);
}

int cerb_dev_upadd_bwd_fused_ok(int H, int W, int C, int G) { return cerb_upadd_bwd_fused_ok(H, W, C, G) ? 1 : 0; }
int cerb_dev_upadd_bwd(const float* dout, float* dskip, float* dprev, int G, int N, int H, int W, int C, long long prev_gs, int shared_prev, unsigned group_mask,
                       int skip_assign, int prev_assign, void* st) {
    DEV_NEED(dout && dskip && dprev && G > 0 && N > 0 && H > 0 && W > 0 && H % 2 == 0 && W % 2 == 0 && C % 4 == 0);
    return (int)cerb_launch_upadd_bwd(dout, dskip, dprev, G, N, H, W, C, prev_gs, shared_prev, (hipStream_t)st, group_mask, skip_assign, prev_assign);
}

int cerb_dev_maxpool_idx(const float* in, float* out, unsigned* idx, int N, int H, int W, int C, void* st) {
    DEV_NEED(in && out && idx && N > 0 && H > 0 && W > 0 && C % 4 == 0);
    return (int)cerb_launch_maxpool_idx(in, out, idx, N, H, W, C, (hipStream_t)st);
}
int cerb_dev_maxpool_bwd_idx(const unsigned* idx, const float* dy, float* dx, int N, int H, int W, int C, void* st) {
    DEV_NEED(idx && dy && dx && N > 0 && H > 0 && W > 0 && H % 2 == 0 && W % 2 == 0 && C % 4 == 0);
    return (int)cerb_launch_maxpool_bwd_idx(idx, dy, dx, N, H, W, C, (hipStream_t)st);
}
int cerb_dev_maxpool_bwd(const float* x, const float* ypool, const float* dy, float* dx, int N, int H, int W, int C, void* st) {
    DEV_NEED(x && ypool && dy && dx && N > 0 && H > 0 && W > 0 && H % 2 == 0 && W % 2 == 0 && C % 4 == 0);
    return (int)cerb_launch_maxpool_bwd(x, ypool, dy, dx, N, H, W, C, (hipStream_t)st);
}

int cerb_dev_pointwise_bwd(const float* x, const float* dy, const float* w, float* dx, float* dw, float* db, long long rows, int cin, int cout, const float* in_scale,
                           int dx_assign, void* st) {
    DEV_NEED(dy && (dx || dw || db) && (!dx || w) && (!dw || x) && rows > 0 && cin > 0 && cout > 0);
    return (int)cerb_launch_pointwise_bwd(x, dy, w, dx, dw, db, rows, cin, cout, in_scale, dx_assign, (hipStream_t)st);
}
size_t cerb_dev_pw_bwd_small_workspace_bytes(long long rows, int cin, int cout) { return cerb_pw_bwd_small_workspace_bytes(rows, cin, cout); }
int cerb_dev_pw_bwd_small(const float* x, const float* dy, const float* w, float* dx, float* dw, float* db, long long rows, int cin, int cout, int dx_assign, void* ws,
                          void* st) {
    DEV_NEED(x && dy && w && ws && rows > 0 && cin > 0 && cout > 0);
    return (int)cerb_launch_pw_bwd_small(x, dy, w, dx, dw, db, rows, cin, cout, dx_assign, ws, (hipStream_t)st);
}
size_t cerb_dev_pw_wgrad_small_workspace_bytes(long long rows, int cin, int cout) { return cerb_pw_wgrad_small_workspace_bytes(rows, cin, cout); }
int cerb_dev_pw_wgrad_small(const float* x, const float* dy, float* dw, long long rows, int cin, int cout, void* ws, void* st) {
    DEV_NEED(x && dy && dw && ws && rows > 0 && cin > 0 && cout > 0);
    return (int)cerb_launch_pw_wgrad_small(x, dy, dw, rows, cin, cout, ws, (hipStream_t)st);
}

size_t cerb_dev_colsum_workspace_bytes(int C, int G) { return (size_t)G * 2048 * C * 4; }
int cerb_dev_colsum(const float* d, long long group_stride, long long rows, int C, int G, float* out, void* ws, void* st) {
    DEV_NEED(d && out && ws && rows > 0 && C > 0 && G > 0);
    return (int)cerb_launch_colsum(d, group_stride, rows, C, G, out, ws, (hipStream_t)st);
}
int cerb_dev_crop_gap(const float* x, int N, int H, int W, int C, int y0, int ch, int x0, int cw, float* out, void* st) {
    DEV_NEED(x && out && N > 0 && C > 0 && y0 >= 0 && x0 >= 0 && ch > 0 && cw > 0 && y0 + ch <= H && x0 + cw <= W);
    return (int)cerb_launch_crop_gap(x, N, H, W, C, y0, ch, x0, cw, out, (hipStream_t)st);
}
int cerb_dev_crop_gap_bwd(const float* dg, float* dx, int N, int H, int W, int C, int y0, int ch, int x0, int cw, void* st) {
    DEV_NEED(dg && dx && N > 0 && C > 0 && y0 >= 0 && x0 >= 0 && ch > 0 && cw > 0 && y0 + ch <= H && x0 + cw <= W);
    return (int)cerb_launch_crop_gap_bwd(dg, dx, N, H, W, C, y0, ch, x0, cw, (hipStream_t)st);
}
int cerb_dev_dilate2(const float* dy, float* d, long long n, int H, int W, int C, void* st) {
    DEV_NEED(dy && d && n > 0 && H > 0 && W > 0);
    return (int)cerb_launch_dilate2(dy, d, n, H, W, C, (hipStream_t)st);
}

long long cerb_devfwd_planar_elems(int N, int H, int W, int C) { return cerb_planar_elems(N, H, W, C); }
int cerb_devfwd_upsample2_add(const float* skip, const float* prev, float* out, int G, int N, int H, int W, int C, long long prev_gs, void* st) {
    DEV_NEED(skip && prev && out && G > 0 && N > 0 && H > 0 && W > 0 && H % 2 == 0 && W % 2 == 0 && C % 4 == 0);
    return (int)cerb_launch_upsample2_add(skip, prev, out, G, N, H, W, C, prev_gs, nullptr, (hipStream_t)st);
}
int cerb_devfwd_upsample2_add_planar(const float* skip, const float* prev, float* out, int G, int N, int H, int W, int C, long long prev_gs, long long out_gs,
                                     int prev_planar, void* st) {
    DEV_NEED(skip && prev && out && G > 0 && N > 0 && H > 0 && W > 0 && out_gs >= cerb_planar_elems(N, H, W, C));
    return (int)cerb_launch_upsample2_add_planar(skip, prev, out, G, N, H, W, C, prev_gs, out_gs, nullptr, prev_planar, (hipStream_t)st);
}

}
```

### cerberus_amd/csrc/net_kernels.hip

```cpp
#include "cerb_common.h"

struct StemParams {
    const unsigned char* tiles;
    const float* tiles_f32;
    const float* wpack;
    const float* bias;
    float* out;
    int N, H, W, tiles_x, tiles_y;
    int relu;
};

template <bool F32IN>
__global__ __launch_bounds__(256, 2) void stem_conv7x7_kernel(StemParams p) {
    constexpr int TH = 8, TW = 32, IH = TH + 6, IW = TW + 6, ROW = 120;
    __shared__ __attribute__((aligned(16))) float wl[7 * 12 * 2 * 64];
    __shared__ __attribute__((aligned(16))) float xl[IH * ROW];
    const int tid = threadIdx.x, lane = tid & 63, wave = tid >> 6, j = lane & 31, h = lane >> 5;
    for (int i = tid; i < 7 * 12 * 2 * 64; i += 256) wl[i] = p.wpack[i];
    const int ntile = p.N * p.tiles_y * p.tiles_x;
    for (int tile = blockIdx.x; tile < ntile; tile += gridDim.x) {
        int t_ = tile;
        const int tx = t_ % p.tiles_x;
        t_ /= p.tiles_x;
        const int ty = t_ % p.tiles_y;
        const int n = t_ / p.tiles_y;
        const int oy0 = ty * TH, ox0 = tx * TW;
        __syncthreads();
        const unsigned char* img = F32IN ? nullptr : p.tiles + (long long)n * p.H * p.W * 3;
        const float* imgf = F32IN ? p.tiles_f32 + (long long)n * p.H * p.W * 3 : nullptr;
        for (int i = tid; i < IH * ROW; i += 256) {
            const int iy = i / ROW, c = i % ROW;
            const int gy = oy0 - 3 + iy, gx = ox0 - 3 + c / 3;
            float v = 0.f;
            if (c < IW * 3 && gy >= 0 && gy < p.H && gx >= 0 && gx < p.W) {
                const long long at = ((long long)gy * p.W + gx) * 3 + c % 3;
                v = (F32IN ? imgf[at] : (float)img[at]) / 255.0f;
            }
            xl[i] = v;
        }
        __syncthreads();
        f32x16 acc[2][2];
#pragma unroll
        for (int s = 0; s < 2; ++s)
#pragma unroll
            for (int q = 0; q < 2; ++q)
#pragma unroll
                for (int r = 0; r < 16; ++r) acc[s][q][r] = 0.f;
        const int b0 = (wave * 2 + 0) * ROW + j * 3 + h;
        const int b1 = (wave * 2 + 1) * ROW + j * 3 + h;
#pragma unroll
        for (int ky = 0; ky < 7; ++ky) {
#pragma unroll
            for (int t = 0; t < 12; ++t) {
                const float a0 = wl[((ky * 12 + t) * 2 + 0) * 64 + lane];
                const float a1 = wl[((ky * 12 + t) * 2 + 1) * 64 + lane];
                const float x0 = xl[b0 + ky * ROW + 2 * t];
                const float x1 = xl[b1 + ky * ROW + 2 * t];
                acc[0][0] = __builtin_amdgcn_mfma_f32_32x32x2f32(a0, x0, acc[0][0], 0, 0, 0);
                acc[1][0] = __builtin_amdgcn_mfma_f32_32x32x2f32(a1, x0, acc[1][0], 0, 0, 0);
                acc[0][1] = __builtin_amdgcn_mfma_f32_32x32x2f32(a0, x1, acc[0][1], 0, 0, 0);
                acc[1][1] = __builtin_amdgcn_mfma_f32_32x32x2f32(a1, x1, acc[1][1], 0, 0, 0);
            }
        }
#pragma unroll
        for (int q = 0; q < 2; ++q) {
            const int oy = oy0 + wave * 2 + q, ox = ox0 + j;
            if (oy >= p.H || ox >= p.W) continue;
            float* o = p.out + (((long long)n * p.H + oy) * p.W + ox) * 64;
#pragma unroll
            for (int s = 0; s < 2; ++s)
#pragma unroll
                for (int rq = 0; rq < 4; ++rq) {
                    const int co = s * 32 + rq * 8 + h * 4;
                    f32x4 v = {acc[s][q][rq * 4 + 0], acc[s][q][rq * 4 + 1], acc[s][q][rq * 4 + 2], acc[s][q][rq * 4 + 3]};
                    v = v + *reinterpret_cast<const f32x4*>(p.bias + co);
                    const float floor_ = p.relu ? 0.f : -3.402823466e38f;
                    v[0] = fmaxf(v[0], floor_);
                    v[1] = fmaxf(v[1], floor_);
                    v[2] = fmaxf(v[2], floor_);
                    v[3] = fmaxf(v[3], floor_);
                    *reinterpret_cast<f32x4*>(o + co) = v;
                }
        }
    }
}

hipError_t cerb_launch_stem(StemParams p, hipStream_t st) {
    p.tiles_x = (p.W + 31) / 32;
    p.tiles_y = (p.H + 7) / 8;
    const long long ntile = (long long)p.N * p.tiles_x * p.tiles_y;
    const unsigned grid = (unsigned)(ntile < 256 * 6 ? ntile : 256 * 6);
    if (p.tiles) hipLaunchKernelGGL(stem_conv7x7_kernel<false>, dim3(grid), dim3(256), 0, st, p);
    else hipLaunchKernelGGL(stem_conv7x7_kernel<true>, dim3(grid), dim3(256), 0, st, p);
    return hipGetLastError();
}

__global__ void maxpool3x3s2_kernel(const float* __restrict__ in, float* __restrict__ out, int N, int H, int W, int C, int Ho, int Wo) {
    const long long total = (long long)N * Ho * Wo * (C / 4);
    const long long per_xcd = gridDim.x / 8, vb = (long long)(blockIdx.x & 7) * per_xcd + (blockIdx.x >> 3);
    for (long long i = vb * (long long)blockDim.x + threadIdx.x; i < total; i += (long long)gridDim.x * blockDim.x) {
        const int c4 = (int)(i % (C / 4));
        long long r = i / (C / 4);
        const int ox = (int)(r % Wo);
        r /= Wo;
        const int oy = (int)(r % Ho);
        const int n = (int)(r / Ho);
        f32x4 m = {-INFINITY, -INFINITY, -INFINITY, -INFINITY};
#pragma unroll
        for (int ky = 0; ky < 3; ++ky) {
            const int y = oy * 2 - 1 + ky;
            if (y < 0 || y >= H) continue;
#pragma unroll
            for (int kx = 0; kx < 3; ++kx) {
                const int x = ox * 2 - 1 + kx;
                if (x < 0 || x >= W) continue;
                const f32x4 v = *reinterpret_cast<const f32x4*>(in + (((long long)n * H + y) * W + x) * C + c4 * 4);
                m[0] = fmaxf(m[0], v[0]);
                m[1] = fmaxf(m[1], v[1]);
                m[2] = fmaxf(m[2], v[2]);
                m[3] = fmaxf(m[3], v[3]);
            }
        }
        *reinterpret_cast<f32x4*>(out + i * 4) = m;
    }
}

__global__ void maxpool3x3s2_idx_kernel(const float* __restrict__ in, float* __restrict__ out, unsigned* __restrict__ idx, int N, int H, int W, int C, int Ho, int Wo) {
    const long long total = (long long)N * Ho * Wo * (C / 4);
    const long long per_xcd = gridDim.x / 8, vb = (long long)(blockIdx.x & 7) * per_xcd + (blockIdx.x >> 3);
    for (long long i = vb * (long long)blockDim.x + threadIdx.x; i < total; i += (long long)gridDim.x * blockDim.x) {
        const int c4 = (int)(i % (C / 4));
        long long r = i / (C / 4);
        const int ox = (int)(r % Wo);
        r /= Wo;
        const int oy = (int)(r % Ho);
        const int n = (int)(r / Ho);
        f32x4 m = {-INFINITY, -INFINITY, -INFINITY, -INFINITY};
        unsigned w0 = 0, w1 = 0, w2 = 0, w3 = 0;
        bool first = true;
#pragma unroll
        for (int ky = 0; ky < 3; ++ky) {
            const int y = oy * 2 - 1 + ky;
            if (y < 0 || y >= H) continue;
#pragma unroll
            for (int kx = 0; kx < 3; ++kx) {
                const int x = ox * 2 - 1 + kx;
                if (x < 0 || x >= W) continue;
                const f32x4 v = *reinterpret_cast<const f32x4*>(in + (((long long)n * H + y) * W + x) * C + c4 * 4);
                const unsigned k = (unsigned)(ky * 3 + kx);
                if (first || v[0] > m[0]) w0 = k;
                if (first || v[1] > m[1]) w1 = k;
                if (first || v[2] > m[2]) w2 = k;
                if (first || v[3] > m[3]) w3 = k;
                first = false;
                m[0] = fmaxf(m[0], v[0]);
                m[1] = fmaxf(m[1], v[1]);
                m[2] = fmaxf(m[2], v[2]);
                m[3] = fmaxf(m[3], v[3]);
            }
        }
        *reinterpret_cast<f32x4*>(out + i * 4) = m;
        idx[i] = w0 | (w1 << 8) | (w2 << 16) | (w3 << 24);
    }
}

hipError_t cerb_launch_maxpool_idx(const float* in, float* out, unsigned* idx, int N, int H, int W, int C, hipStream_t st) {
    const int Ho = (H + 2 - 3) / 2 + 1, Wo = (W + 2 - 3) / 2 + 1;
    const long long total = (long long)N * Ho * Wo * (C / 4);
    long long blocks = ((total + 255) / 256 + 7) / 8 * 8;
    if (blocks > 256 * 64) blocks = 256 * 64;
    hipLaunchKernelGGL(maxpool3x3s2_idx_kernel, dim3((unsigned)blocks), dim3(256), 0, st, in, out, idx, N, H, W, C, Ho, Wo);
    return hipGetLastError();
}

hipError_t cerb_launch_maxpool(const float* in, float* out, int N, int H, int W, int C, hipStream_t st) {
    const int Ho = (H + 2 - 3) / 2 + 1, Wo = (W + 2 - 3) / 2 + 1;
    const long long total = (long long)N * Ho * Wo * (C / 4);
    long long blocks = ((total + 255) / 256 + 7) / 8 * 8;
    if (blocks > 256 * 64) blocks = 256 * 64;
    hipLaunchKernelGGL(maxpool3x3s2_kernel, dim3((unsigned)blocks), dim3(256), 0, st, in, out, N, H, W, C, Ho, Wo);
    return hipGetLastError();
}

__device__ __forceinline__ f32x4 blend2(float a, const f32x4& x, float b, const f32x4& y) {
    f32x4 r;
#pragma unroll
    for (int e = 0; e < 4; ++e) r[e] = __builtin_fmaf(a, x[e], b * y[e]);
    return r;
}
__global__ void upsample2_add_kernel(const float* __restrict__ skip, const float* __restrict__ prev, float* __restrict__ out, int groups,
                                     int N, int H, int W, int C, long long prev_gs, int bm_lo, int bm_cnt, int bn_lo, int bn_cnt) {
    const int Hp = H >> 1, Wp = W >> 1, C4 = C >> 2;
    const long long total = (long long)N * bm_cnt * bn_cnt * C4;
    const long long out_gs = (long long)N * H * W * C;
    for (long long i = blockIdx.x * (long long)blockDim.x + threadIdx.x; i < total; i += (long long)gridDim.x * blockDim.x) {
        const int c4 = (int)(i % C4);
        long long r = i / C4;
        const int bn = (int)(r % bn_cnt) + bn_lo;
        r /= bn_cnt;
        const int bm = (int)(r % bm_cnt) + bm_lo;
        const int n = (int)(r / bm_cnt);
        const int m0 = max(bm, 0), m1 = min(bm + 1, Hp - 1), n0 = max(bn, 0), n1 = min(bn + 1, Wp - 1);
        f32x4 sk[2][2];
        bool ok[2][2];
        long long o[2][2];
#pragma unroll
        for (int dy = 0; dy < 2; ++dy)
#pragma unroll
            for (int dx = 0; dx < 2; ++dx) {
                const int y = 2 * bm + 1 + dy, x = 2 * bn + 1 + dx;
                ok[dy][dx] = y >= 0 && y < H && x >= 0 && x < W;
                o[dy][dx] = (((long long)n * H + y) * W + x) * C + c4 * 4;
                if (ok[dy][dx]) sk[dy][dx] = *reinterpret_cast<const f32x4*>(skip + o[dy][dx]);
            }
        const long long pb = (long long)n * Hp * Wp * C + c4 * 4;
        for (int g = 0; g < groups; ++g) {
            const float* pg = prev + g * prev_gs + pb;
            const f32x4 p00 = *reinterpret_cast<const f32x4*>(pg + ((long long)m0 * Wp + n0) * C);
            const f32x4 p01 = *reinterpret_cast<const f32x4*>(pg + ((long long)m0 * Wp + n1) * C);
            const f32x4 p10 = *reinterpret_cast<const f32x4*>(pg + ((long long)m1 * Wp + n0) * C);
            const f32x4 p11 = *reinterpret_cast<const f32x4*>(pg + ((long long)m1 * Wp + n1) * C);
            const f32x4 top_l = blend2(0.75f, p00, 0.25f, p01), top_r = blend2(0.25f, p00, 0.75f, p01);
            const f32x4 bot_l = blend2(0.75f, p10, 0.25f, p11), bot_r = blend2(0.25f, p10, 0.75f, p11);
            const f32x4 u[2][2] = {{blend2(0.75f, top_l, 0.25f, bot_l), blend2(0.75f, top_r, 0.25f, bot_r)},
                                   {blend2(0.25f, top_l, 0.75f, bot_l), blend2(0.25f, top_r, 0.75f, bot_r)}};
#pragma unroll
            for (int dy = 0; dy < 2; ++dy)
#pragma unroll
                for (int dx = 0; dx < 2; ++dx)
                    if (ok[dy][dx]) __builtin_nontemporal_store(sk[dy][dx] + u[dy][dx], reinterpret_cast<f32x4*>(out + g * out_gs + o[dy][dx]));
        }
    }
}

hipError_t cerb_launch_upsample2_add(const float* skip, const float* prev, float* out, int groups, int N, int H, int W, int C,
                                     long long prev_gs, const int* roi, hipStream_t st) {
    int bm_lo = -1, bm_hi = H / 2 - 1, bn_lo = -1, bn_hi = W / 2 - 1;
    if (roi && roi[1] > roi[0] && roi[3] > roi[2]) {
        auto lo = [](int v) { return (v - 2 >= 0 ? (v - 2) / 2 : -1); };
        bm_lo = lo(roi[0]);
        bn_lo = lo(roi[2]);
        if ((roi[1] - 1) / 2 < bm_hi) bm_hi = (roi[1] - 1) / 2;
        if ((roi[3] - 1) / 2 < bn_hi) bn_hi = (roi[3] - 1) / 2;
    }
    const int bm_cnt = bm_hi - bm_lo + 1, bn_cnt = bn_hi - bn_lo + 1;
    const long long total = (long long)N * bm_cnt * bn_cnt * (C / 4);
    long long blocks = (total + 255) / 256;
    if (blocks > 256 * 32) blocks = 256 * 32;
    if (blocks < 1) blocks = 1;
    hipLaunchKernelGGL(upsample2_add_kernel, dim3((unsigned)blocks), dim3(256), 0, st, skip, prev, out, groups, N, H, W, C, prev_gs, bm_lo, bm_cnt, bn_lo,
                       bn_cnt);
    return hipGetLastError();
}

template <bool PREV_PLANAR, int C>
__global__ __launch_bounds__(256) void upsample2_add_planar_kernel(const float* __restrict__ skip, const float* __restrict__ prev, float* __restrict__ out,
                                                                   int groups, int N, int H, int W, long long prev_gs, long long out_gs, int byp, int bxp,
                                                                   int by_lo, int by_cnt, int bx_lo, int bx_cnt) {
    static_assert(C % 64 == 0, "four 16-channel planes per pass");
    constexpr int NCC = C / 16, NPASS = NCC / 4;
    const int Hp = H >> 1, Wp = W >> 1;
    const int lane = threadIdx.x & 63, m = lane >> 2, cq = lane & 3, ty = m >> 2, tx = m & 3;
    const int nwork = N * by_cnt * bx_cnt * NPASS;
    for (int wk = blockIdx.x; wk < nwork; wk += gridDim.x) {
        const int blk = wk / NPASS, cc = (wk % NPASS) * 4 + (int)(threadIdx.x >> 6);
        const int bx = blk % bx_cnt + bx_lo;
        const int r_ = blk / bx_cnt;
        const int by = r_ % by_cnt + by_lo, n = r_ / by_cnt;
        const int y0 = 16 * by + 4 * ty, x0 = 16 * bx + 4 * tx;
        if (y0 >= H || x0 >= W) continue;
        const int ch = cc * 16 + cq * 4;
        f32x4 sk[4][4];
#pragma unroll
        for (int i = 0; i < 4; ++i)
#pragma unroll
            for (int j = 0; j < 4; ++j) sk[i][j] = *reinterpret_cast<const f32x4*>(skip + (((long long)n * H + y0 + i) * W + x0 + j) * C + ch);
        int rr[4], qq[4];
#pragma unroll
        for (int k = 0; k < 4; ++k) {
            rr[k] = min(max((y0 >> 1) - 1 + k, 0), Hp - 1);
            qq[k] = min(max((x0 >> 1) - 1 + k, 0), Wp - 1);
        }
        float* ob = out + ((((long long)n * byp + by + 1) * bxp + bx + 1) * NCC + cc) * 4096 + lane * 4;
        long long pcol[4];
        if constexpr (PREV_PLANAR) {
#pragma unroll
            for (int k = 0; k < 4; ++k) pcol[k] = (long long)((qq[k] >> 4) + 1) * NCC * 4096 + ((qq[k] & 3) * 16 + ((qq[k] >> 2) & 3)) * 16;
        }
        const int pbyp = cerb_planar_blocks(Hp), pbxp = cerb_planar_blocks(Wp);
        for (int g = 0; g < groups; ++g) {
            const float* pg = PREV_PLANAR ? prev + g * prev_gs + (long long)cc * 4096 + cq * 4 : prev + g * prev_gs + (long long)n * Hp * Wp * C + ch;
            f32x4 h[4][4];
#pragma unroll
            for (int k = 0; k < 4; ++k) {
                f32x4 p0, p1, p2, p3;
                if constexpr (PREV_PLANAR) {
                    const float* pr = pg + (((long long)n * pbyp + (rr[k] >> 4) + 1) * pbxp) * NCC * 4096 + (((rr[k] & 3) << 2) * 16 + (((rr[k] >> 2) & 3) << 2)) * 16;
                    p0 = *reinterpret_cast<const f32x4*>(pr + pcol[0]); p1 = *reinterpret_cast<const f32x4*>(pr + pcol[1]);
                    p2 = *reinterpret_cast<const f32x4*>(pr + pcol[2]); p3 = *reinterpret_cast<const f32x4*>(pr + pcol[3]);
                } else {
                    const float* pr = pg + (long long)rr[k] * Wp * C;
                    p0 = *reinterpret_cast<const f32x4*>(pr + (long long)qq[0] * C); p1 = *reinterpret_cast<const f32x4*>(pr + (long long)qq[1] * C);
                    p2 = *reinterpret_cast<const f32x4*>(pr + (long long)qq[2] * C); p3 = *reinterpret_cast<const f32x4*>(pr + (long long)qq[3] * C);
                }
                h[k][0] = blend2(0.25f, p0, 0.75f, p1);
                h[k][1] = blend2(0.75f, p1, 0.25f, p2);
                h[k][2] = blend2(0.25f, p1, 0.75f, p2);
                h[k][3] = blend2(0.75f, p2, 0.25f, p3);
            }
            float* og = ob + g * out_gs;
#pragma unroll
            for (int j = 0; j < 4; ++j) {
                const f32x4 u0 = blend2(0.25f, h[0][j], 0.75f, h[1][j]), u1 = blend2(0.75f, h[1][j], 0.25f, h[2][j]), u2 = blend2(0.25f, h[1][j], 0.75f, h[2][j]),
                            u3 = blend2(0.75f, h[2][j], 0.25f, h[3][j]);
#ifndef UPP_PLAIN_STORE
                __builtin_nontemporal_store(sk[0][j] + u0, reinterpret_cast<f32x4*>(og + (0 * 4 + j) * 256));
                __builtin_nontemporal_store(sk[1][j] + u1, reinterpret_cast<f32x4*>(og + (1 * 4 + j) * 256));
                __builtin_nontemporal_store(sk[2][j] + u2, reinterpret_cast<f32x4*>(og + (2 * 4 + j) * 256));
                __builtin_nontemporal_store(sk[3][j] + u3, reinterpret_cast<f32x4*>(og + (3 * 4 + j) * 256));
#else
                *reinterpret_cast<f32x4*>(og + (0 * 4 + j) * 256) = sk[0][j] + u0;
                *reinterpret_cast<f32x4*>(og + (1 * 4 + j) * 256) = sk[1][j] + u1;
                *reinterpret_cast<f32x4*>(og + (2 * 4 + j) * 256) = sk[2][j] + u2;
                *reinterpret_cast<f32x4*>(og + (3 * 4 + j) * 256) = sk[3][j] + u3;
#endif
            }
        }
    }
}

hipError_t cerb_launch_upsample2_add_planar(const float* skip, const float* prev, float* out, int groups, int N, int H, int W, int C, long long prev_gs,
                                            long long out_gs, const int* roi, int prev_planar, hipStream_t st) {
    if ((C != 64 && C != 128 && C != 256) || (H & 3) || (W & 3)) return hipErrorInvalidValue;
    int by_lo = 0, by_hi = (H + 15) / 16, bx_lo = 0, bx_hi = (W + 15) / 16;
    if (roi && roi[1] > roi[0] && roi[3] > roi[2]) {
        by_lo = roi[0] / 16; by_hi = (roi[1] + 15) / 16;
        bx_lo = roi[2] / 16; bx_hi = (roi[3] + 15) / 16;
    }
    const long long nblk = (long long)N * (by_hi - by_lo) * (bx_hi - bx_lo);
    if (nblk <= 0 || nblk >= (1ll << 31)) return hipErrorInvalidValue;
#ifndef UPP_GRID
#define UPP_GRID 16
#endif
    const long long nwork = nblk * (C / 64);
    if (nwork >= (1ll << 31)) return hipErrorInvalidValue;
    long long blocks = nwork < 256 * UPP_GRID ? nwork : 256 * UPP_GRID;
    auto kern = C == 64    ? (prev_planar ? upsample2_add_planar_kernel<true, 64> : upsample2_add_planar_kernel<false, 64>)
                : C == 128 ? (prev_planar ? upsample2_add_planar_kernel<true, 128> : upsample2_add_planar_kernel<false, 128>)
                           : (prev_planar ? upsample2_add_planar_kernel<true, 256> : upsample2_add_planar_kernel<false, 256>);
    hipLaunchKernelGGL(kern, dim3((unsigned)blocks), dim3(256), 0, st, skip, prev, out, groups, N, H, W, prev_gs, out_gs,
                       cerb_planar_blocks(H), cerb_planar_blocks(W), by_lo, by_hi - by_lo, bx_lo, bx_hi - bx_lo);
    return hipGetLastError();
}

#ifndef HEAD_TPW
#define HEAD_TPW 2
#endif
typedef float f32x4h __attribute__((ext_vector_type(4)));
__device__ __forceinline__ void head_absmax_commit(unsigned int* word, float m) {
#pragma unroll
    for (int o = 32; o >= 1; o >>= 1) m = fmaxf(m, __shfl_xor(m, o));
    if ((threadIdx.x & 63) == 0) {
        const unsigned int b = __float_as_uint(m);
        if (b > __atomic_load_n(word, __ATOMIC_RELAXED)) atomicMax(word, b);
    }
}

template <bool ROI>
__global__ __launch_bounds__(256, 2) void head_kernel(HeadParams p) {
    const int tid = threadIdx.x, lane = tid & 63, px = lane & 15, ks = lane >> 4;
    const f32x4h* w1v = reinterpret_cast<const f32x4h*>(p.w1p) + lane;
    const f32x4h* w2v = reinterpret_cast<const f32x4h*>(p.w2p) + lane;
    struct BPos {
        int n, row, xb;
    };
    auto inc = [&](BPos b) {
        if (++b.xb == p.nxb) {
            b.xb = 0;
            if (++b.row == p.rows) {
                b.row = 0;
                ++b.n;
            }
        }
        return b;
    };
    const long long npix = (long long)p.N * p.H * p.W;
    long long pbase = ((long long)blockIdx.x * 4 + (tid >> 6)) * (64 * HEAD_TPW);
    BPos cur[4], nxt[4];
    if constexpr (ROI) {
        const int wave = __builtin_amdgcn_readfirstlane(tid >> 6);
        const unsigned nblk = (unsigned)p.N * (unsigned)p.rows * (unsigned)p.nxb;
        const unsigned b0 = ((unsigned)blockIdx.x * 4u + (unsigned)wave) * (4u * HEAD_TPW);
        const unsigned bc = b0 < nblk ? b0 : nblk;
        const unsigned r = bc / (unsigned)p.nxb;
        cur[0].xb = (int)(bc - r * (unsigned)p.nxb);
        cur[0].n = (int)(r / (unsigned)p.rows);
        cur[0].row = (int)(r - (unsigned)cur[0].n * (unsigned)p.rows);
#pragma unroll
        for (int pb = 1; pb < 4; ++pb) cur[pb] = inc(cur[pb - 1]);
        nxt[0] = inc(cur[3]);
#pragma unroll
        for (int pb = 1; pb < 4; ++pb) nxt[pb] = inc(nxt[pb - 1]);
    }
    auto ptr_of = [&](const BPos& b) {
        const int n = min(b.n, p.N - 1), x = min(p.xa0 + 16 * b.xb + px, p.W - 1);
        return p.feat + (((long long)n * p.H + p.row0 + b.row) * p.W + x) * 64 + 4 * ks;
    };
    auto feat_ptr = [&](int pb, bool next) {
        if constexpr (ROI) return ptr_of(next ? nxt[pb] : cur[pb]);
        const long long P = pbase + (next ? 64 : 0) + pb * 16 + px;
        return p.feat + (P < npix ? P : npix - 1) * 64 + 4 * ks;
    };
    f32x4h x[4];
#pragma unroll
    for (int pb = 0; pb < 4; ++pb) x[pb] = *reinterpret_cast<const f32x4h*>(feat_ptr(pb, false));
    float amax = 0.f;
#pragma unroll 1
    for (int task = 0; task < HEAD_TPW; ++task, pbase += 64) {
    f32x4h acc1[6][4];
#pragma unroll
    for (int blk = 0; blk < 6; ++blk) {
        const f32x4h bb = *reinterpret_cast<const f32x4h*>(p.b1 + blk * 16 + ks * 4);
#pragma unroll
        for (int pb = 0; pb < 4; ++pb) acc1[blk][pb] = bb;
    }
    const float* xp[4];
#pragma unroll
    for (int pb = 0; pb < 4; ++pb) xp[pb] = feat_ptr(pb, false);
#pragma unroll
    for (int g = 0; g < 4; ++g) {
        f32x4h xn[4];
        if (g + 1 < 4) {
#pragma unroll
            for (int pb = 0; pb < 4; ++pb) xn[pb] = *reinterpret_cast<const f32x4h*>(xp[pb] + (g + 1) * 16);
        } else if (task + 1 < HEAD_TPW) {
#pragma unroll
            for (int pb = 0; pb < 4; ++pb) xn[pb] = *reinterpret_cast<const f32x4h*>(feat_ptr(pb, true));
        }
#pragma unroll
        for (int blk = 0; blk < 6; ++blk) {
            const f32x4h a = w1v[(blk * 4 + g) * 64];
#pragma unroll
            for (int t = 0; t < 4; ++t)
#pragma unroll
                for (int pb = 0; pb < 4; ++pb) acc1[blk][pb] = __builtin_amdgcn_mfma_f32_16x16x4f32(a[t], x[pb][t], acc1[blk][pb], 0, 0, 0);
        }
        if (g + 1 < 4 || task + 1 < HEAD_TPW) {
#pragma unroll
            for (int pb = 0; pb < 4; ++pb) x[pb] = xn[pb];
        }
    }
#pragma unroll
    for (int blk = 0; blk < 6; ++blk)
#pragma unroll
        for (int pb = 0; pb < 4; ++pb)
#pragma unroll
            for (int r = 0; r < 4; ++r) acc1[blk][pb][r] = fmaxf(acc1[blk][pb][r], 0.f);
    f32x4h acc2[4];
    {
        const f32x4h b2 = *reinterpret_cast<const f32x4h*>(p.b2 + 4 * ks);
#pragma unroll
        for (int pb = 0; pb < 4; ++pb) acc2[pb] = b2;
    }
#pragma unroll
    for (int blk = 0; blk < 6; ++blk) {
        const f32x4h a = w2v[blk * 64];
#pragma unroll
        for (int r = 0; r < 4; ++r)
#pragma unroll
            for (int pb = 0; pb < 4; ++pb) acc2[pb] = __builtin_amdgcn_mfma_f32_16x16x4f32(a[r], acc1[blk][pb][r], acc2[pb], 0, 0, 0);
    }
    float lg[8];
#pragma unroll
    for (int e = 0; e < 4; ++e) {
        float lo = 0.f, hi = 0.f;
#pragma unroll
        for (int pb = 0; pb < 4; ++pb) {
            const float t0 = __shfl(acc2[pb][e], px), t1 = __shfl(acc2[pb][e], 16 + px);
            lo = (ks == pb) ? t0 : lo;
            hi = (ks == pb) ? t1 : hi;
        }
        lg[e] = lo;
        lg[4 + e] = hi;
// ... 506 lines not shown
```

Baseline: 151.0.

## Run ResNet encoder stages in tile-planar layout with planar Winograd residual convs

Encoder stages of the backbone now keep activations in a tile-planar layout. This covers a planar maxpool entry, stride-2 implicit-GEMM convs that write planar output, and a new residual variant (LEVEL 4) of the planar Winograd F(4x4) kernel. Each stage then converts back to NHWC for the decoder skip connections. The aim is to let the faster planar Winograd kernels handle the encoder's stride-1 3x3 convs and to avoid layout shuffles inside blocks. The cost is an extra planar-to-NHWC pass per stage, extra planar buffers, and new device test entry points. It is enabled by default for stages 1-3 through an env mask.

```diff
diff --git a/cerberus_amd/csrc/cerb_api.hip b/cerberus_amd/csrc/cerb_api.hip
--- a/cerberus_amd/csrc/cerb_api.hip
+++ b/cerberus_amd/csrc/cerb_api.hip
@@ -219,6 +219,9 @@
                             o[idx++] = U[((size_t)co * cin + ci) * 36 + xi];
                         }
 }
+
+void cerb_host_pack_conv(const float* w, int cout, int cin, int ks, int chunk, std::vector<float>* out) { pack_conv(w, nullptr, cout, cin, ks, chunk, out); }
+void cerb_host_pack_wino4(const float* w, int cout, int cin, int layout, std::vector<float>* out) { pack_wino4(w, cout, cin, out, layout); }
 
 static int store_bn(cerb_net* net, const std::string& name, const std::vector<std::string>& bnkeys, int ch) {
     std::vector<float> ga, be;
@@ -538,8 +541,11 @@
 }
 
 static constexpr int kPlanarLowest = 0;
+static constexpr int kEncPlanarStages = 0x7;
 static const char* const kPlanarFamily[4] = {"conv_wino4_planar<f4x4,16x16x2,eighth-res>", "conv_wino4_planar<f4x4,16x16x2,quarter-res>",
                                              "conv_wino4p<f4x4,16x16x2,planar,half-res>", "conv_wino4p<f4x4,16x16x2,planar>"};
+static const char* const kEncPlanarFamily = "conv_wino4_enc<f4x4,16x16x2>";
+static const char* const kEncPlanarFamilyRes = "conv_wino4_enc<f4x4,16x16x2,res>";
 static const char* const kPlanarEntryFamily[4] = {"upsample2_add_planar<eighth-res>", "upsample2_add_planar<quarter-res>", "upsample2_add_planar", "upsample2_add_planar"};
 
 int run_conv(cerb_net* net, const std::string& name, const float* in, const float* prev, const float* resid, float* out, int N,
@@ -580,7 +586,19 @@
         return e ? atoll(e) : 4096ll;
     }();
     const bool w4b = !planar && (net->conv_algo == 7 || (net->conv_algo == 6 && map_px <= w4b_max_px)) && c.cin % 64 == 0;
-    if (planar && !(use_w4 && c.wino && mode == 0 && net->fold_bn && !resid)) return fail("internal: conv " + name + " cannot take the planar path");
+    const bool enc_planar = planar && net->planar_level == 4;
+    if (enc_planar && c.stride == 2) {
+        if (resid || mode != 0 || !net->fold_bn) return fail("internal: conv " + name + " cannot store tile-planar");
+        p.out_gs = planar_out_gs;
+        p.pl_byp = cerb_planar_blocks(p.Ho);
+        p.pl_bxp = cerb_planar_blocks(p.Wo);
+        const std::string kn = "conv_igemm_planar<ks" + std::to_string(c.ks) + ",s2" + (p.Wo < 32 ? ",16x16>" : ",8x32>");
+        if (prof_begin(net, name, kn, fl, st)) return 1;
+        HIP_OK(cerb_launch_conv(p, c.ks, c.stride, mode, st));
+        if (prof_end(net, st)) return 1;
+        return 0;
+    }
+    if (planar && !(use_w4 && c.wino && mode == 0 && net->fold_bn && (!resid || enc_planar))) return fail("internal: conv " + name + " cannot take the planar path");
     if (use_w4 && c.wino && mode == 0 && (!it->second.host_w.empty() || !net->fold_bn)) {
         PackedConv& cm = it->second;
         float* train_slot = nullptr;
@@ -606,11 +624,11 @@
         }
         if (planar) {
             p.out_gs = planar_out_gs;
-            p.level_tag = net->planar_level == 3 ? 1 : net->planar_level == 2 ? 0 : 2;
+            p.level_tag = enc_planar ? (resid ? 4 : 3) : net->planar_level == 3 ? 1 : net->planar_level == 2 ? 0 : 2;
             p.pl_byp = cerb_planar_blocks(p.Ho);
             p.pl_bxp = cerb_planar_blocks(p.Wo);
         }
-        if (prof_begin(net, name, planar ? kPlanarFamily[net->planar_level & 3] : w4b ? (cerb_wino4b_packed(p) ? (resid ? "conv_wino4b<f4x4,16t,res>" : "conv_wino4b<f4x4,16t>") : (resid ? "conv_wino4b<f4x4,16x16,res>" : "conv_wino4b<f4x4,16x16>")) : (resid ? "conv_wino4<f4x4,16x16x2,res>" : "conv_wino4<f4x4,16x16x2>"), fl_done, st)) return 1;
+        if (prof_begin(net, name, enc_planar ? (resid ? kEncPlanarFamilyRes : kEncPlanarFamily) : planar ? kPlanarFamily[net->planar_level & 3] : w4b ? (cerb_wino4b_packed(p) ? (resid ? "conv_wino4b<f4x4,16t,res>" : "conv_wino4b<f4x4,16t>") : (resid ? "conv_wino4b<f4x4,16x16,res>" : "conv_wino4b<f4x4,16x16>")) : (resid ? "conv_wino4<f4x4,16x16x2,res>" : "conv_wino4<f4x4,16x16x2>"), fl_done, st)) return 1;
         if (net->conv_bn_part && !planar && !resid && !(roi && roi[1] > roi[0] && roi[3] > roi[2])) {
             p.bn_part = net->conv_bn_part;
             net->conv_bn_bpg = w4b ? cerb_wino4b_bn_blocks(p) : N * ((p.Ho + 15) / 16) * ((p.Wo + 15) / 16);
@@ -706,15 +724,64 @@
         if (prof_begin(net, "stem", "stem_conv7x7", 2.0 * N * H * W * 64.0 * 147.0, st)) return 1;
         HIP_OK(cerb_launch_stem(sp, st));
         if (prof_end(net, st)) return 1;
-        if (prof_begin(net, "maxpool", "maxpool3x3s2", 0.0, st)) return 1;
-        HIP_OK(cerb_launch_maxpool(net->x0.p, net->pool.p, N, H, W, 64, st));
-        if (prof_end(net, st)) return 1;
+    }
+    const int enc_mask = [] {
+        const char* e = cerb_dev_getenv("CERB_ENC_PLANAR");
+        return e ? atoi(e) : kEncPlanarStages;
+    }();
+    auto encoder_stage_is_planar = [&](int li) {
+        if (dry || !net->planar || !net->fold_bn || net->conv_algo != 6 || !((enc_mask >> li) & 1)) return false;
+        const int hh = hs[li + 1], ww = ws[li + 1], planes = kFilters[li + 1];
+        if ((hh & 15) || (ww & 15) || hh < 16 || ww < 16 || planes % 64) return false;
+        for (int b = 0; b < kLayers[li]; ++b)
+            for (int j = 1; j <= 2; ++j) {
+                auto c = net->conv.find("backbone.layer" + std::to_string(li + 1) + "." + std::to_string(b) + ".conv" + std::to_string(j));
+                if (c == net->conv.end()) return false;
+                if (c->second.stride == 1 && (!c->second.wino || c->second.host_w.empty() || c->second.cin % 16)) return false;
+            }
+        return true;
+    };
+    if (!dry) {
+        if (encoder_stage_is_planar(0)) {
+            if (net->enc_a[0].ensure(1, N, hs[1], ws[1], 64, st)) return fail_alloc();
+            if (prof_begin(net, "maxpool", "maxpool3x3s2_planar", 0.0, st)) return 1;
+            HIP_OK(cerb_launch_maxpool_planar(net->x0.p, net->enc_a[0].b.p, N, H, W, 64, st));
+            if (prof_end(net, st)) return 1;
+        } else {
+            if (prof_begin(net, "maxpool", "maxpool3x3s2", 0.0, st)) return 1;
+            HIP_OK(cerb_launch_maxpool(net->x0.p, net->pool.p, N, H, W, 64, st));
+            if (prof_end(net, st)) return 1;
+        }
     }
     float* cur = dry ? nullptr : net->pool.p;
     int inpl = 64;
     for (int li = 0; li < 4; ++li) {
         const int planes = kFilters[li + 1];
         const int Hi = (li == 0) ? hs[1] : hs[li], Wi = (li == 0) ? ws[1] : ws[li];
+        if (encoder_stage_is_planar(li)) {
+            PlanarBuf &ba = net->enc_a[li], &bb = net->enc_b[li];
+            const int hh = hs[li + 1], ww = ws[li + 1];
+            if (ba.ensure(1, N, hh, ww, planes, st) || bb.ensure(1, N, hh, ww, planes, st)) return fail_alloc();
+            const int keep_level = net->planar_level;
+            net->planar_level = 4;
+            struct Restore { cerb_net* n; int v; ~Restore() { n->planar_level = v; } } restore{net, keep_level};
+            for (int b = 0; b < kLayers[li]; ++b) {
+                const std::string p = "backbone.layer" + std::to_string(li + 1) + "." + std::to_string(b);
+                if (b == 0 && li > 0) {
+                    if (run_conv(net, p + ".conv1", cur, nullptr, nullptr, bb.b.p, N, Hi, Wi, 1, 0, 0, 0, st, macs, nullptr, bb.gs())) return 1;
+                    if (run_conv(net, p + ".downsample", cur, nullptr, nullptr, ba.b.p, N, Hi, Wi, 0, 0, 0, 0, st, macs, nullptr, ba.gs())) return 1;
+                } else if (run_conv(net, p + ".conv1", ba.b.p, nullptr, nullptr, bb.b.p, N, hh, ww, 1, 0, ba.gs(), 0, st, macs, nullptr, bb.gs())) {
+                    return 1;
+                }
+                if (run_conv(net, p + ".conv2", bb.b.p, nullptr, ba.b.p, ba.b.p, N, hh, ww, 1, 0, bb.gs(), 0, st, macs, nullptr, ba.gs())) return 1;
+            }
+            if (prof_begin(net, "backbone.layer" + std::to_string(li + 1) + ".exit", "planar_to_nhwc", 0.0, st)) return 1;
+            HIP_OK(cerb_launch_planar_to_nhwc(ba.b.p, net->x[li + 1].p, N, hh, ww, planes, st));
+            if (prof_end(net, st)) return 1;
+            cur = net->x[li + 1].p;
+            inpl = planes;
+            continue;
+        }
         for (int b = 0; b < kLayers[li]; ++b) {
             const std::string p = "backbone.layer" + std::to_string(li + 1) + "." + std::to_string(b);
             const int stride = (b == 0 && li > 0) ? 2 : 1;
diff --git a/cerberus_amd/csrc/cerb_net.h b/cerberus_amd/csrc/cerb_net.h
--- a/cerberus_amd/csrc/cerb_net.h
+++ b/cerberus_amd/csrc/cerb_net.h
@@ -108,6 +108,8 @@
                                  const float* dgamma, const float* dbeta, const float* w1, const float* w2, float* dprev, float* dw1, float* db1, long long rows, int out,
                                  int eval_mode, int assign, void* ws, hipStream_t st, const float* const* in_bn = nullptr, double* in_part = nullptr);
 hipError_t cerb_launch_maxpool(const float* in, float* out, int N, int H, int W, int C, hipStream_t st);
+hipError_t cerb_launch_maxpool_planar(const float* in, float* out, int N, int H, int W, int C, hipStream_t st);
+hipError_t cerb_launch_planar_to_nhwc(const float* in, float* out, int N, int H, int W, int C, hipStream_t st);
 hipError_t cerb_launch_head(const HeadParams& p, hipStream_t st);
 hipError_t cerb_launch_head_group(const HeadParams* heads, int n_heads, hipStream_t st, int w2_44);
 struct PatchClassParams {
@@ -263,6 +265,7 @@
     int planar_level = 3;
     PlanarBuf psum2, pmid2, pout2;
     PlanarBuf psum1, pmid1, pout1, psum0, pmid0, pout0;
+    PlanarBuf enc_a[4], enc_b[4];
     int packed_items = 1;
     int planar = 1;
     bool profiling = false;
@@ -289,6 +292,8 @@
         if (pack_tab) (void)hipFree(pack_tab);
         x0.release(); pool.release(); ta.release(); tb.release(); cm.release(); dmid.release(); dsum.release(); psum.release(); pmid.release(); pout.release(); psum2.release(); pmid2.release(); pout2.release(); psum1.release(); pmid1.release(); pout1.release(); psum0.release(); pmid0.release(); pout0.release();
         t_mean.release(); t_rstd.release(); t_ws.release(); t_hid.release(); t_gap.release(); t_pc1.release(); t_idn.release(); t_dil.release();
+        for (auto& b : enc_a) b.release();
+        for (auto& b : enc_b) b.release();
         for (auto& b : tape) b.release();
         for (auto& b : x) b.release();
         for (auto& b : dout) b.release();
@@ -298,6 +303,8 @@
 
 static const int kLayers[4] = {3, 4, 6, 3};
 static const int kFilters[5] = {64, 64, 128, 256, 512};
+void cerb_host_pack_conv(const float* w, int cout, int cin, int ks, int chunk, std::vector<float>* out);
+void cerb_host_pack_wino4(const float* w, int cout, int cin, int layout, std::vector<float>* out);
 int prof_begin(cerb_net* net, const std::string& name, const std::string& kernel, double flops, hipStream_t st);
 int prof_end(cerb_net* net, hipStream_t st);
 int train_wino2_fresh(cerb_net* net, const std::string& name, PackedConv& cm, int dgrad, hipStream_t st);
diff --git a/cerberus_amd/csrc/conv_igemm.hip b/cerberus_amd/csrc/conv_igemm.hip
--- a/cerberus_amd/csrc/conv_igemm.hip
+++ b/cerberus_amd/csrc/conv_igemm.hip
@@ -40,7 +40,7 @@
     int g, cb, n, oy0, ox0, tx, ty;
 };
 
-template <int KS, int STRIDE, int TH, int TW, int CB, int MODE>
+template <int KS, int STRIDE, int TH, int TW, int CB, int MODE, bool PL = false>
 __global__ __launch_bounds__(256, 2) void conv_igemm_kernel(ConvParams p) {
     using C = ConvCfg<KS, STRIDE, TH, TW, CB, MODE>;
     constexpr int WD = C::WD;
@@ -145,7 +145,10 @@
         const int pl = (wave * 2 + q) * 32 + j;
         const int py = pl / TW, px = pl % TW;
         ldsb[q] = ((py * C::LSTEP) * C::IW + px * C::LSTEP) * C::PS + 4 * h;
-        ooff[q] = (unsigned)(((py * p.Wo + px) * p.Cout + 4 * h) * 4);
+        if constexpr (PL)
+            ooff[q] = (unsigned)(((px >> 4) * (p.Cout >> 4) * 4096 + ((py & 3) * 4 + (px & 3)) * 256 + ((py >> 2) * 4 + ((px >> 2) & 3)) * 16 + 4 * h) * 4);
+        else
+            ooff[q] = (unsigned)(((py * p.Wo + px) * p.Cout + 4 * h) * 4);
     }
     float* aux = lds + C::MAIN_FLOATS;
     int aoffM = 0, aoffE[NE];
@@ -340,7 +343,8 @@
 
         {
             const float* bias = p.bias + w.g * p.bias_gs + w.cb * 64 + h * 4;
-            const long long origin = (((long long)w.n * p.Ho + w.oy0) * p.Wo + w.ox0) * p.Cout + w.cb * 64;
+            const long long origin = PL ? ((((long long)w.n * p.pl_byp + (w.oy0 >> 4) + 1) * p.pl_bxp + (w.ox0 >> 4) + 1) * (p.Cout >> 4) + w.cb * 4) * 4096 + ((w.oy0 >> 2) & 3) * 64
+                                        : (((long long)w.n * p.Ho + w.oy0) * p.Wo + w.ox0) * p.Cout + w.cb * 64;
             const __amdgpu_buffer_rsrc_t r_out = make_rsrc(p.out + w.g * p.out_gs + origin);
             const __amdgpu_buffer_rsrc_t r_res = make_rsrc(p.resid ? p.resid + w.g * p.resid_gs + origin : p.out);
             const bool has_res = p.resid != nullptr;
@@ -358,14 +362,14 @@
                         const int co = s * 32 + rq * 8;
                         f32x4 o = {acc[s][q][rq * 4 + 0], acc[s][q][rq * 4 + 1], acc[s][q][rq * 4 + 2], acc[s][q][rq * 4 + 3]};
                         o = o + *reinterpret_cast<const f32x4*>(bias + co);
-                        if (has_res) o = o + buf_load(r_res, ooff[q], co * 4);
+                        if (!PL && has_res) o = o + buf_load(r_res, ooff[q], co * 4);
                         if (p.relu) {
                             o[0] = fmaxf(o[0], 0.f);
                             o[1] = fmaxf(o[1], 0.f);
                             o[2] = fmaxf(o[2], 0.f);
                             o[3] = fmaxf(o[3], 0.f);
                         }
-                        buf_store(o, r_out, ooff[q], co * 4);
+                        buf_store(o, r_out, ooff[q], PL ? (co >> 4) * 16384 + (co & 15) * 4 : co * 4);
                     }
                 }
             }
@@ -377,13 +381,13 @@
     }
 }
 
-template <int KS, int STRIDE, int TH, int TW, int CB, int MODE>
+template <int KS, int STRIDE, int TH, int TW, int CB, int MODE, bool PL = false>
 static hipError_t launch_cfg(ConvParams p, hipStream_t st) {
     using C = ConvCfg<KS, STRIDE, TH, TW, CB, MODE>;
     p.tiles_x = (p.Wo + TW - 1) / TW;
     p.tiles_y = (p.Ho + TH - 1) / TH;
     const long long items = (long long)p.groups * p.N * p.tiles_x * p.tiles_y * (p.Cout / 64);
-    auto kern = conv_igemm_kernel<KS, STRIDE, TH, TW, CB, MODE>;
+    auto kern = conv_igemm_kernel<KS, STRIDE, TH, TW, CB, MODE, PL>;
     static bool attr_done[64] = {};
     if (cerb_attr_needed(attr_done)) {
         hipError_t e = hipFuncSetAttribute(reinterpret_cast<const void*>(kern), hipFuncAttributeMaxDynamicSharedMemorySize, C::LDS_BYTES);
@@ -402,6 +406,14 @@
 
 hipError_t cerb_launch_conv(const ConvParams& p, int ks, int stride, int mode, hipStream_t st) {
     const bool small = p.Wo < 32;
+    if (p.pl_byp > 0) {
+        if (stride != 2 || mode != 0 || p.resid || (p.Ho & 15) || (p.Wo & 15) || p.Ho < 16 || p.Wo < 16 || p.groups != 1 || p.pl_byp != cerb_planar_blocks(p.Ho) ||
+            p.pl_bxp != cerb_planar_blocks(p.Wo))
+            return hipErrorInvalidValue;
+        if (ks == 3) return small ? launch_cfg<3, 2, 16, 16, 16, 0, true>(p, st) : launch_cfg<3, 2, 8, 32, 16, 0, true>(p, st);
+        if (ks == 1) return small ? launch_cfg<1, 2, 16, 16, 16, 0, true>(p, st) : launch_cfg<1, 2, 8, 32, 16, 0, true>(p, st);
+        return hipErrorInvalidValue;
+    }
     if (ks == 3 && stride == 1 && mode == 0) return small ? launch_cfg<3, 1, 16, 16, 32, 0>(p, st) : launch_cfg<3, 1, 8, 32, 32, 0>(p, st);
     if (ks == 3 && stride == 1 && mode == 1) return small ? launch_cfg<3, 1, 16, 16, 32, 1>(p, st) : launch_cfg<3, 1, 8, 32, 32, 1>(p, st);
     if (ks == 3 && stride == 2 && mode == 0) return small ? launch_cfg<3, 2, 16, 16, 16, 0>(p, st) : launch_cfg<3, 2, 8, 32, 16, 0>(p, st);
diff --git a/cerberus_amd/csrc/conv_wino4p.hip b/cerberus_amd/csrc/conv_wino4p.hip
--- a/cerberus_amd/csrc/conv_wino4p.hip
+++ b/cerberus_amd/csrc/conv_wino4p.hip
@@ -138,6 +138,7 @@
 template <int LEVEL>
 __global__ __launch_bounds__(256) __attribute__((amdgpu_waves_per_eu(1, 1))) void conv_wino4p_kernel(ConvParams p) {
     extern __shared__ __attribute__((aligned(16))) float lds[];
+    constexpr bool RES = LEVEL == 4;
     const int tid = threadIdx.x;
     const int lane = tid & 63;
     const int a = __builtin_amdgcn_readfirstlane(tid >> 6);
@@ -509,6 +510,17 @@
                 const long long origin = p.out_gs * w.g + ((((long long)bo.n * p.pl_byp + by_abs + 1) * p.pl_bxp + bx_abs + 1) * nplane_o + w.cb * 4 + a) * (long long)(PLANE_BYTES / 4);
                 const __amdgpu_buffer_rsrc_t r_out = __builtin_amdgcn_make_buffer_rsrc(p.out + origin, 0, PLANE_BYTES, 0x00020000);
                 const bool partial = (by_abs * BLK + BLK > p.Ho) || (bx_abs * BLK + BLK > p.Wo);
+                f32x4 rs[RES ? 4 : 1][RES ? 4 : 1];
+                auto load_res = [&](int i) __attribute__((always_inline)) {
+                    if constexpr (RES) {
+                        const int res_y = p.Ho - by_abs * BLK - 4 * (m_o >> 2), res_x = p.Wo - bx_abs * BLK - 4 * (m_o & 3);
+                        const __amdgpu_buffer_rsrc_t r_res = __builtin_amdgcn_make_buffer_rsrc(const_cast<float*>(p.resid) + (origin - p.out_gs * w.g + p.resid_gs * w.g), 0, PLANE_BYTES, 0x00020000);
+#pragma unroll
+                        for (int j = 0; j < 4; ++j) rs[i][j] = buf_load<0>(r_res, (!partial || (i < res_y && j < res_x)) ? olane : 0x80000000u, (i * 4 + j) * 1024);
+                    }
+                };
+                load_res(0);
+                load_res(1);
                 f32x4 T[4][6];
 #pragma unroll
                 for (int b = 0; b < 6; ++b) {
@@ -536,6 +548,7 @@
 #pragma unroll
                     for (int j = 0; j < 4; ++j) {
                         f32x4 o = y[j];
+                        if constexpr (RES) o = o + rs[i][j];
                         o[0] = fmaxf(o[0], floor_);
                         o[1] = fmaxf(o[1], floor_);
                         o[2] = fmaxf(o[2], floor_);
@@ -550,6 +563,9 @@
 #else
                         if (o[0] == 1.2345e-30f) buf_store(o, r_out, vo, (i * 4 + j) * 1024);
 #endif
+                    }
+                    if constexpr (RES) {
+                        if (i + 2 < 4) load_res(i + 2);
                     }
                 }
             }
@@ -571,13 +587,13 @@
 }
 
 hipError_t cerb_launch_wino4p(ConvParams p, hipStream_t st) {
-    if (p.Cin % CB || p.Cout % 64 || p.resid || p.pl_byp < 3 || p.pl_bxp < 3 || p.H != p.Ho || p.W != p.Wo) return hipErrorInvalidValue;
+    if (p.Cin % CB || p.Cout % 64 || (p.resid != nullptr) != (p.level_tag == 4) || p.pl_byp < 3 || p.pl_bxp < 3 || p.H != p.Ho || p.W != p.Wo) return hipErrorInvalidValue;
     const long long nblk = wino4_block_grid(p);
     if (p.pl_byp != (p.Ho + BLK - 1) / BLK + 2 || p.pl_bxp != (p.Wo + BLK - 1) / BLK + 2) return hipErrorInvalidValue;
     const long long items = (long long)p.groups * ((nblk + 1) / 2) * (p.Cout / 64);
-    const int tag = p.level_tag == 2 ? 2 : p.level_tag ? 1 : 0;
-    auto kern = tag == 2 ? conv_wino4p_kernel<2> : tag ? conv_wino4p_kernel<1> : conv_wino4p_kernel<0>;
-    static bool attr_done[3][64] = {};
+    const int tag = p.level_tag >= 2 && p.level_tag <= 4 ? p.level_tag : p.level_tag ? 1 : 0;
+    auto kern = tag == 4 ? conv_wino4p_kernel<4> : tag == 3 ? conv_wino4p_kernel<3> : tag == 2 ? conv_wino4p_kernel<2> : tag ? conv_wino4p_kernel<1> : conv_wino4p_kernel<0>;
+    static bool attr_done[5][64] = {};
     return wino4_launch(kern, attr_done[tag], items, LDS_BYTES + PROF_BYTES, p, st);
 }
 
diff --git a/cerberus_amd/csrc/dev_entry.hip b/cerberus_amd/csrc/dev_entry.hip
--- a/cerberus_amd/csrc/dev_entry.hip
+++ b/cerberus_amd/csrc/dev_entry.hip
@@ -127,4 +127,61 @@
     return (int)cerb_launch_upsample2_add_planar(skip, prev, out, G, N, H, W, C, prev_gs, out_gs, nullptr, prev_planar, (hipStream_t)st);
 }
 
+static int devfwd_upload(const std::vector<float>& v, float** out) {
+    if (hipMalloc((void**)out, v.size() * 4) != hipSuccess) return 1;
+    return hipMemcpy(*out, v.data(), v.size() * 4, hipMemcpyHostToDevice) != hipSuccess;
 }
+int cerb_devfwd_conv3x3(const float* w_host, const float* bias, const float* in, const float* resid, float* out, int N, int H, int W, int Cin, int Cout, int relu,
+                        int planar, void* st) {
+    DEV_NEED(w_host && bias && in && out && N > 0 && H >= 16 && W >= 16 && H % 16 == 0 && W % 16 == 0 && Cin % 64 == 0 && Cout % 64 == 0);
+    std::vector<float> w4;
+    cerb_host_pack_wino4(w_host, Cout, Cin, planar ? 0 : 1, &w4);
+    float* dw = nullptr;
+    DEV_NEED(devfwd_upload(w4, &dw) == 0);
+    ConvParams p;
+    memset(&p, 0, sizeof(p));
+    p.in = in; p.wpack = dw; p.bias = bias; p.resid = resid; p.out = out;
+    p.N = N; p.H = p.Ho = H; p.W = p.Wo = W; p.Cin = Cin; p.Cout = Cout; p.relu = relu; p.groups = 1;
+    p.w_gs = (long long)Cout * Cin * 36; p.bias_gs = Cout; p.pk_off = 1;
+    p.out_gs = planar ? cerb_planar_elems(N, H, W, Cout) : (long long)N * H * W * Cout;
+    if (planar) {
+        p.level_tag = resid ? 4 : 3;
+        p.pl_byp = cerb_planar_blocks(H);
+        p.pl_bxp = cerb_planar_blocks(W);
+    }
+    hipError_t e = planar ? cerb_launch_wino4p(p, (hipStream_t)st) : cerb_launch_wino4b(p, (hipStream_t)st);
+    if (e == hipSuccess) e = hipStreamSynchronize((hipStream_t)st);
+    (void)hipFree(dw);
+    return (int)e;
+}
+int cerb_devfwd_conv_s2(const float* w_host, const float* bias, const float* in, float* out, int N, int H, int W, int Cin, int Cout, int ks, int relu, int planar, void* st) {
+    DEV_NEED(w_host && bias && in && out && N > 0 && H % 32 == 0 && W % 32 == 0 && Cin % 16 == 0 && Cout % 64 == 0 && (ks == 1 || ks == 3));
+    std::vector<float> wp;
+    cerb_host_pack_conv(w_host, Cout, Cin, ks, cerb_conv_chunk(ks, 2), &wp);
+    float* dw = nullptr;
+    DEV_NEED(devfwd_upload(wp, &dw) == 0);
+    ConvParams p;
+    memset(&p, 0, sizeof(p));
+    p.in = in; p.wpack = dw; p.bias = bias; p.out = out;
+    p.N = N; p.H = H; p.W = W; p.Ho = H / 2; p.Wo = W / 2; p.Cin = Cin; p.Cout = Cout; p.relu = relu; p.groups = 1;
+    p.w_gs = (long long)Cout * Cin * ks * ks; p.bias_gs = Cout;
+    p.out_gs = planar ? cerb_planar_elems(N, p.Ho, p.Wo, Cout) : (long long)N * p.Ho * p.Wo * Cout;
+    if (planar) {
+        p.pl_byp = cerb_planar_blocks(p.Ho);
+        p.pl_bxp = cerb_planar_blocks(p.Wo);
+    }
+    hipError_t e = cerb_launch_conv(p, ks, 2, 0, (hipStream_t)st);
+    if (e == hipSuccess) e = hipStreamSynchronize((hipStream_t)st);
+    (void)hipFree(dw);
+    return (int)e;
+}
+int cerb_devfwd_maxpool(const float* in, float* out, int N, int H, int W, int C, int planar, void* st) {
+    DEV_NEED(in && out && N > 0 && H > 0 && W > 0 && C % 4 == 0);
+    return (int)(planar ? cerb_launch_maxpool_planar(in, out, N, H, W, C, (hipStream_t)st) : cerb_launch_maxpool(in, out, N, H, W, C, (hipStream_t)st));
+}
+int cerb_devfwd_planar_to_nhwc(const float* in, float* out, int N, int H, int W, int C, void* st) {
+    DEV_NEED(in && out && N > 0);
+    return (int)cerb_launch_planar_to_nhwc(in, out, N, H, W, C, (hipStream_t)st);
+}
+
+}
diff --git a/cerberus_amd/csrc/net_kernels.hip b/cerberus_amd/csrc/net_kernels.hip
--- a/cerberus_amd/csrc/net_kernels.hip
+++ b/cerberus_amd/csrc/net_kernels.hip
@@ -179,6 +179,74 @@
     long long blocks = ((total + 255) / 256 + 7) / 8 * 8;
     if (blocks > 256 * 64) blocks = 256 * 64;
     hipLaunchKernelGGL(maxpool3x3s2_kernel, dim3((unsigned)blocks), dim3(256), 0, st, in, out, N, H, W, C, Ho, Wo);
+    return hipGetLastError();
+}
+
+__global__ void maxpool3x3s2_planar_kernel(const float* __restrict__ in, float* __restrict__ out, int N, int H, int W, int C, int Ho, int Wo) {
+    const long long total = (long long)N * Ho * Wo * (C / 4);
+    const int byp = cerb_planar_blocks(Ho), bxp = cerb_planar_blocks(Wo), ncc = C >> 4;
+    const long long per_xcd = gridDim.x / 8, vb = (long long)(blockIdx.x & 7) * per_xcd + (blockIdx.x >> 3);
+    for (long long i = vb * (long long)blockDim.x + threadIdx.x; i < total; i += (long long)gridDim.x * blockDim.x) {
+        const int c4 = (int)(i % (C / 4));
+        long long r = i / (C / 4);
+        const int ox = (int)(r % Wo);
+        r /= Wo;
+        const int oy = (int)(r % Ho);
+        const int n = (int)(r / Ho);
+        f32x4 m = {-INFINITY, -INFINITY, -INFINITY, -INFINITY};
+#pragma unroll
+        for (int ky = 0; ky < 3; ++ky) {
+            const int y = oy * 2 - 1 + ky;
+            if (y < 0 || y >= H) continue;
+#pragma unroll
+            for (int kx = 0; kx < 3; ++kx) {
+                const int x = ox * 2 - 1 + kx;
+                if (x < 0 || x >= W) continue;
+                const f32x4 v = *reinterpret_cast<const f32x4*>(in + (((long long)n * H + y) * W + x) * C + c4 * 4);
+                m[0] = fmaxf(m[0], v[0]);
+                m[1] = fmaxf(m[1], v[1]);
+                m[2] = fmaxf(m[2], v[2]);
+                m[3] = fmaxf(m[3], v[3]);
+            }
+        }
+        *reinterpret_cast<f32x4*>(out + cerb_planar_offset(n, oy, ox, c4 >> 2, byp, bxp, ncc) + (c4 & 3) * 4) = m;
+    }
+}
+
+hipError_t cerb_launch_maxpool_planar(const float* in, float* out, int N, int H, int W, int C, hipStream_t st) {
+    const int Ho = (H + 2 - 3) / 2 + 1, Wo = (W + 2 - 3) / 2 + 1;
+    if (C % 64 || (Ho & 15) || (Wo & 15) || Ho < 16 || Wo < 16) return hipErrorInvalidValue;
+    const long long total = (long long)N * Ho * Wo * (C / 4);
+    long long blocks = ((total + 255) / 256 + 7) / 8 * 8;
+    if (blocks > 256 * 64) blocks = 256 * 64;
+    hipLaunchKernelGGL(maxpool3x3s2_planar_kernel, dim3((unsigned)blocks), dim3(256), 0, st, in, out, N, H, W, C, Ho, Wo);
+    return hipGetLastError();
+}
+
+__global__ __launch_bounds__(256) void planar_to_nhwc_kernel(const float* __restrict__ in, float* __restrict__ out, int N, int H, int W, int C) {
+    const int ncc = C >> 4, ncb = C >> 6, nby = H >> 4, nbx = W >> 4, byp = nby + 2, bxp = nbx + 2;
+    const int q = threadIdx.x & 15, pp = threadIdx.x >> 4;
+    const int nwork = N * nby * nbx * ncb;
+    for (int wk = blockIdx.x; wk < nwork; wk += gridDim.x) {
+        const int blk = wk / ncb, cb = wk % ncb;
+        const int bx = blk % nbx, r_ = blk / nbx, by = r_ % nby, n = r_ / nby;
+        const float* ib = in + ((((long long)n * byp + by + 1) * bxp + bx + 1) * ncc + cb * 4 + (q >> 2)) * 4096 + (q & 3) * 4;
+        float* ob = out + (((long long)n * H + 16 * by) * W + 16 * bx) * C + cb * 64 + q * 4;
+#pragma unroll
+        for (int k = 0; k < 16; ++k) {
+            const int y = k, x = pp;
+            const f32x4 v = *reinterpret_cast<const f32x4*>(ib + (((y & 3) * 4 + (x & 3)) * 16 + (y >> 2) * 4 + (x >> 2)) * 16);
+            *reinterpret_cast<f32x4*>(ob + ((long long)y * W + x) * C) = v;
+        }
+    }
+}
+
+hipError_t cerb_launch_planar_to_nhwc(const float* in, float* out, int N, int H, int W, int C, hipStream_t st) {
+    if (C % 64 || (H & 15) || (W & 15) || H < 16 || W < 16) return hipErrorInvalidValue;
+    const long long nwork = (long long)N * (H / 16) * (W / 16) * (C / 64);
+    if (nwork >= (1ll << 31)) return hipErrorInvalidValue;
+    const long long blocks = nwork < 256 * 16 ? nwork : 256 * 16;
+    hipLaunchKernelGGL(planar_to_nhwc_kernel, dim3((unsigned)blocks), dim3(256), 0, st, in, out, N, H, W, C);
     return hipGetLastError();
 }
 
```

Result: faster. 152.5, median of 6 (+1.0%).
